# jarcode-foss/glava

Hardware: AMD Instinct MI355X
Metric: stereo 4096-pt FFT+smooth frames/s; % HBM roofline -- `value`: the window+FFT+magnitude pass of BASELINE configs[1]; the FFT+smooth chains (gravity / average on f32 state, GLava's shipped GL_R16 chain, + its pre-smoothing pass) are in roofline.chains (higher is better)
Workload: dtype f32

## Files before the change

### glava_amd/build.py

```python
from __future__ import annotations

import argparse
import os
import subprocess
import sys
from concurrent.futures import ThreadPoolExecutor

HERE = os.path.dirname(os.path.abspath(__file__))
CSRC = os.path.join(HERE, "csrc")
OBJ = os.path.join(CSRC, "build")
TUNE_BIN = os.path.join(os.path.dirname(HERE), "tools", "bin")
ARCH = "gfx950"
HIPFLAGS = ["--offload-arch=" + ARCH, "-O3", "-std=c++17", "-ffp-contract=off", "-fPIC",
            "-fno-fast-math", "-Wall", "-Wno-unused-function"]
SIZES = (7, 8, 9, 10, 11, 12, 13, 14)
SMALL = ("glv_bars", "glv_misc")
HOST = ("glv_api", "glv_wisdom", "glv_device_state", "glv_bar_tables", "glv_chain", "glv_track", "glv_multi")
PARTS = (0, 1, 2, 3, 4, 5, 6)


def _inst_jobs(obj_dir: str, sizes, extra: list[str]):
    return [("glv_inst.hip", os.path.join(obj_dir, f"glv_inst_{k}_{p}.o"), [f"-DGLV_LOG_NN={k}", f"-DGLV_INST_PART={p}", *extra])
            for k in sorted(sizes, reverse=True) for p in PARTS]
HEADERS = ["glv_core.h", "glv_frame.h", "glv_kernel_tmpl.h", "glv_launch.h", "glv_launch_util.h", "glv_tables.h", "glv_winsplit.h", "glv_host.h",
           os.path.join("..", "..", "include", "glv_spectrum.h")]


def _newer(target: str, deps: list[str]) -> bool:
    if not os.path.exists(target):
        return True
    t = os.path.getmtime(target)
    return any(os.path.getmtime(d) > t for d in deps)


def _hipcc() -> str:
    for c in (os.environ.get("HIPCC"), "/opt/rocm/bin/hipcc", "hipcc"):
        if c and (os.path.isabs(c) and os.path.exists(c) or not os.path.isabs(c)):
            return c
    return "hipcc"


def _run(cmd: list[str]) -> None:
    r = subprocess.run(cmd, capture_output=True, text=True)
    if r.returncode != 0:
        sys.stderr.write(" ".join(cmd) + "\n" + r.stdout + r.stderr)
        raise RuntimeError("build step failed: " + os.path.basename(cmd[-1]))


def _compile(src: str, obj: str, extra: list[str]) -> str:
    deps = [os.path.join(CSRC, src)] + [os.path.join(CSRC, h) for h in HEADERS]
    if _newer(obj, deps):
        cmd = [_hipcc(), *HIPFLAGS, *extra, "-c", os.path.join(CSRC, src), "-o", obj]
        _run(cmd)
        open(obj + ".cmd", "w").write(" ".join(cmd) + "\n")
    return obj


def _refuse_experiment_flags(flags: list[str]) -> None:
    env = " ".join(os.environ.get(k, "") for k in ("HIPCC_COMPILE_FLAGS_APPEND", "HIPFLAGS", "CXXFLAGS", "CPPFLAGS"))
    bad = [f for f in flags if f.startswith("-D") and not f.startswith(("-DGLV_LOG_NN=", "-DGLV_INST_PART="))]
    if bad or "-DGLV_" in env:
        raise RuntimeError(f"product build refuses extra macro definitions: {bad or env!r} (use build_variant for A/B libraries)")


def build_tune_variant(name: str, extra_flags: list[str], variants: str | None = None) -> str:
    os.makedirs(OBJ, exist_ok=True)
    os.makedirs(TUNE_BIN, exist_ok=True)
    obj = os.path.join(OBJ, f"glv_tune_{name}.o")
    flags = ["-DGLV_TUNE_BUILD", *[f for f in extra_flags if f != "-DGLV_TUNE_BUILD"]]
    if variants:
        flags.append("-DGLV_TUNE_VARIANTS=" + variants)
    _run([_hipcc(), *HIPFLAGS, *flags, "-c", os.path.join(CSRC, "glv_tune.hip"), "-o", obj])
    lib = os.path.join(TUNE_BIN, f"libglvtune_{name}.so")
    _run([_hipcc(), "--offload-arch=" + ARCH, "-shared", "-fPIC", "-o", lib, obj])
    os.remove(obj)
    return lib


def build_variant(name: str, extra_flags: list[str], sizes=SIZES, kernels_only: bool = False, misc: bool = False) -> str:
    obj_dir = os.path.join(OBJ, name)
    os.makedirs(obj_dir, exist_ok=True)
    extra_flags = ["-DGLV_TUNE_BUILD", *[f for f in extra_flags if f != "-DGLV_TUNE_BUILD"]]
    jobs = _inst_jobs(obj_dir, sizes, extra_flags)
    reused = []
    if kernels_only:
        reused = [os.path.join(OBJ, f"glv_inst_{k}_{p}.o") for k in SIZES if k not in sizes for p in PARTS]
        reused += [os.path.join(OBJ, f"{u}.o") for u in HOST]
        if misc:
            jobs += [(f"{m}.hip", os.path.join(obj_dir, f"{m}.o"), list(extra_flags)) for m in SMALL]
        else:
            reused += [os.path.join(OBJ, f"{m}.o") for m in SMALL]
    else:
        jobs += [(f"{m}.hip", os.path.join(obj_dir, f"{m}.o"), list(extra_flags)) for m in SMALL]
        jobs += [(f"{u}.cpp", os.path.join(obj_dir, f"{u}.o"), ["-x", "hip", *extra_flags]) for u in HOST]
    with ThreadPoolExecutor(max_workers=min(8, os.cpu_count() or 2)) as ex:
        objs = list(ex.map(lambda j: _compile(*j), jobs))
    lib = os.path.join(CSRC, f"libglvspectrum_{name}.so")
    _run([_hipcc(), "--offload-arch=" + ARCH, "-shared", "-fPIC", "-o", lib, *objs, *reused])
    return lib


def build(tune: bool = False, verbose: bool = False) -> str:
    lib = os.path.join(CSRC, "libglvspectrum.so")
    srcs = [os.path.join(CSRC, f) for f in ("glv_inst.hip", *(f"{m}.hip" for m in SMALL), *(f"{u}.cpp" for u in HOST))] + [os.path.join(CSRC, h) for h in HEADERS]
    stamp_path = lib + ".stamp"
    stamp = repr(max(os.path.getmtime(f) for f in srcs))
    if not tune and os.path.exists(lib) and os.path.exists(stamp_path) and open(stamp_path).read() == stamp:
        if verbose:
            print("up to date", lib)
        return lib
    os.makedirs(OBJ, exist_ok=True)
    jobs = _inst_jobs(OBJ, SIZES, [])
    jobs += [(f"{m}.hip", os.path.join(OBJ, f"{m}.o"), []) for m in SMALL]
    jobs += [(f"{u}.cpp", os.path.join(OBJ, f"{u}.o"), ["-x", "hip"]) for u in HOST]
    for _, _, extra in jobs:
        _refuse_experiment_flags(extra)
    if tune:
        jobs.append(("glv_tune.hip", os.path.join(OBJ, "glv_tune.o"), ["-DGLV_TUNE_BUILD"]))
    with ThreadPoolExecutor(max_workers=min(8, os.cpu_count() or 2)) as ex:
        objs = list(ex.map(lambda j: _compile(*j), jobs))
    prod = [o for o in objs if not o.endswith("glv_tune.o")]
    if _newer(lib, prod) or not os.path.exists(stamp_path) or open(stamp_path).read() != stamp:
        _run([_hipcc(), "--offload-arch=" + ARCH, "-shared", "-fPIC", "-o", lib, *prod])
    if repr(max(os.path.getmtime(f) for f in srcs)) == stamp:
        open(stamp_path, "w").write(stamp)
    else:
        for o in prod:
            os.remove(o)
        if os.path.exists(stamp_path): os.remove(stamp_path)
    if tune:
        tlib = os.path.join(CSRC, "libglvtune.so")
        tobj = os.path.join(OBJ, "glv_tune.o")
        if _newer(tlib, [tobj]):
            _run([_hipcc(), "--offload-arch=" + ARCH, "-shared", "-fPIC", "-o", tlib, tobj])
    if verbose:
        print("built", lib)
    return lib


if __name__ == "__main__":
    ap = argparse.ArgumentParser()
    ap.add_argument("--tune", action="store_true")
    ap.add_argument("--variant", nargs="+", metavar=("NAME", "FLAG"), help="build libglvspectrum_NAME.so with extra flags; write them without the leading dash (DGLV_X=1)")
    a = ap.parse_args()
    if a.variant:
        print("built", build_variant(a.variant[0], ["-" + f.lstrip("-") for f in a.variant[1:]]))
    else:
        build(tune=a.tune, verbose=True)
```

### glava_amd/csrc/glv_api.cpp

```cpp
#include <cstdarg>
#include <cstdio>
#include <cstdlib>
#include <new>

#include "glv_host.h"
#include "glv_tables.h"

namespace glvh __attribute__((visibility("hidden"))) {
thread_local std::string g_err = "";
int fail(int code, const char* fmt, ...) {
    char buf[512];
    va_list ap;
    va_start(ap, fmt);
    vsnprintf(buf, sizeof(buf), fmt, ap);
    va_end(ap);
    g_err = buf;
    return code;
}
}
namespace {
int validate(const glv_params* p) {
    if (!p) return fail(GLV_ERR_INVALID, "params is NULL");
    const int l = log2_exact(p->n);
    if (l < 8 || l > 15) return fail(GLV_ERR_INVALID, "n=%u: must be a power of two in [256, 32768]", p->n);
    if (p->channels != 1 && p->channels != 2) return fail(GLV_ERR_INVALID, "channels=%u: must be 1 or 2", p->channels);
    if (p->avg_frames < 1 || p->avg_frames > GLV_MAX_AVG_FRAMES)
        return fail(GLV_ERR_INVALID, "avg_frames=%u: must be in [1, %d]", p->avg_frames, GLV_MAX_AVG_FRAMES);
    if (p->avg_window_kind > 1) return fail(GLV_ERR_INVALID, "avg_window_kind=%u: must be 0 or 1", p->avg_window_kind);
    if (p->log_mode > 2) return fail(GLV_ERR_INVALID, "log_mode=%u: must be 0, 1 or 2", p->log_mode);
    if (p->gl_storage > 2) return fail(GLV_ERR_INVALID, "gl_storage=%u: must be 0, 1 (GL_R16 state, one launch) or 2 (pass by pass, f32 state)", p->gl_storage);
    if (p->ur != p->ur) return fail(GLV_ERR_INVALID, "ur is NaN");
    if (p->round_formula > GLV_ROUND_LINEAR) return fail(GLV_ERR_INVALID, "round_formula=%u: 0 sinusoidal, 1 circular, 2 linear", p->round_formula);
    if (p->sample_mode > GLV_SAMPLE_HYBRID) return fail(GLV_ERR_INVALID, "sample_mode=%u: 0 average, 1 maximum, 2 hybrid", p->sample_mode);
    return GLV_OK;
}

int ensure_device(int device) {
    int count = 0;
    hipError_t e = hipGetDeviceCount(&count);
    if (e != hipSuccess || count <= 0)
        return fail(GLV_ERR_NO_DEVICE, "no usable HIP device (%s); this library has no CPU path",
                    e == hipSuccess ? "device count is 0" : hipGetErrorString(e));
    if (device < 0 || device >= count) return fail(GLV_ERR_INVALID, "device %d out of range [0, %d)", device, count);
    HIP_TRY(hipSetDevice(device));
    return GLV_OK;
}

bool same_params(const glv_params& a, const glv_params& b) {
    return a.n == b.n && a.channels == b.channels && same_bits(a.fft_scale, b.fft_scale) && same_bits(a.fft_cutoff, b.fft_cutoff)
           && same_bits(a.gravity_step, b.gravity_step) && same_bits(a.ur, b.ur) && a.avg_frames == b.avg_frames && a.avg_window == b.avg_window
           && a.avg_window_kind == b.avg_window_kind && a.log_mode == b.log_mode && a.bars == b.bars && same_bits(a.smooth_factor, b.smooth_factor)
           && same_bits(a.smooth_distance, b.smooth_distance) && same_bits(a.smooth_ratio, b.smooth_ratio) && a.gl_storage == b.gl_storage
           && same_bits(a.bar_phase, b.bar_phase) && same_shape(a, b);
}

int batch_create_rows(const glv_params* p, uint32_t streams, unsigned ops_mask, int device, bool single_row, glv_batch** out) {
    if (!out) return fail(GLV_ERR_INVALID, "out is NULL");
    *out = nullptr;
    if (int rc = validate(p)) return rc;
    if (streams == 0) return fail(GLV_ERR_INVALID, "streams must be > 0");
    if (streams > (1u << 30)) return fail(GLV_ERR_INVALID, "streams=%u: at most 2^30 (row indices are 32-bit)", streams);
    if (int rc = ensure_device(device)) return rc;
    wisdom_load_env();
    glv_batch* b = new (std::nothrow) glv_batch();
    if (!b) return fail(GLV_ERR_NOMEM, "out of host memory");
    b->p = *p; b->streams = streams; b->ops_mask = ops_mask; b->device = device;
    b->rows = single_row ? 1u : streams * 2u; b->single_row = single_row;
    b->unfused_bars = std::getenv("GLV_UNFUSED_BARS") != nullptr;
    b->unfused_wave = std::getenv("GLV_UNFUSED_WAVE") != nullptr;
    if (const char* o = std::getenv("GLV_TRACK_WAVE_ORDER")) b->track_wave_by_steps = std::strcmp(o, "steps") == 0;
    b->bar_i8_off = std::getenv("GLV_NO_BARS_I8") != nullptr;
    b->log_nn = log2_exact(p->n) - 1;
    hipDeviceProp_t prop;
    if (hipGetDeviceProperties(&prop, device) == hipSuccess) {
        b->num_cus = prop.multiProcessorCount;
        std::snprintf(b->device_name, sizeof(b->device_name), "%s", prop.gcnArchName[0] ? prop.gcnArchName : prop.name);
    }
    int rc = b->tab.create(p->n, device);
    if (rc == GLV_OK) rc = batch_alloc(b);
    if (rc == GLV_OK) rc = batch_prepare(b);
    if (rc != GLV_OK) { glv_batch_destroy(b); return rc; }
    *out = b;
    return GLV_OK;
}

int sync_params(glv_batch* b, const glv_params* p) {
    if (same_params(b->p, *p)) return GLV_OK;
    glv_params rest = *p;
    rest.ur = b->p.ur; rest.gravity_step = b->p.gravity_step;
    if (!same_params(b->p, rest)) return glv_batch_set_params(b, p);
    b->p.ur = p->ur; b->p.gravity_step = p->gravity_step;
    update_gravity_step(b);
    return GLV_OK;
}

int round_trip(glv_state* s, const void* in, size_t in_bytes, void* out, size_t out_bytes, unsigned ops, bool texels) {
    glv_batch* b = s->b;
    HIP_TRY(hipSetDevice(b->device));
    const bool via_seq = s->mapped && (ops & GLV_OP_SMOOTH);
    if (via_seq && !s->seq) HIP_TRY(s->seq.alloc(b->p.n, false));
    if (texels && !s->d_tex) {
        if (s->mapped) {
            HIP_TRY(hipHostMalloc(reinterpret_cast<void**>(&s->h_tex), out_bytes, hipHostMallocMapped));
            HIP_TRY(hipHostGetDevicePointer(reinterpret_cast<void**>(&s->d_tex), s->h_tex, 0));
        } else {
            HIP_TRY(s->tex_copy.alloc(b->p.n, false));
            s->d_tex = s->tex_copy;
        }
    }
    float* d_in = via_seq ? s->seq.get() : s->d_io;
    float* d_out = texels ? reinterpret_cast<float*>(s->d_tex) : d_in;
    if (s->mapped && !via_seq) {
        std::memcpy(s->h_io, in, in_bytes);
        const int rc = process(b, d_in, glv::IN_F32_PLANAR, d_out, ops, 1, 0, nullptr);
        HIP_TRY(hipStreamSynchronize(nullptr));
        if (rc) return rc;
        std::memcpy(out, texels ? static_cast<const void*>(s->h_tex) : s->h_io, out_bytes);
        return GLV_OK;
    }
    HIP_TRY(hipMemcpyAsync(d_in, in, in_bytes, hipMemcpyHostToDevice, nullptr));
    if (int rc = process(b, d_in, glv::IN_F32_PLANAR, d_out, ops, 1, 0, nullptr)) return rc;
    HIP_TRY(hipMemcpyAsync(out, d_out, out_bytes, hipMemcpyDeviceToHost, nullptr));
    HIP_TRY(hipStreamSynchronize(nullptr));
    return GLV_OK;
}
}

extern "C" {
void glv_params_default(glv_params* p) {
    if (!p) return;
    std::memset(p, 0, sizeof(*p));
    p->n = 4096;
    p->channels = 2;
    p->fft_scale = 10.2F;
    p->fft_cutoff = 0.3F;
    p->gravity_step = 4.2F;
    p->ur = 22050.0F / 256.0F;
    p->avg_frames = 5;
    p->avg_window = 1;
    p->avg_window_kind = 0;
    p->log_mode = 1;
    p->bars = 80;
    p->smooth_factor = 0.025F;
    p->smooth_distance = 0.01F;
    p->smooth_ratio = 4.0F;
    p->gl_storage = 0;
    p->bar_phase = 0.0F;
}

int glv_set_last_error(int code, const char* msg) { g_err = msg ? msg : ""; return code; }
int glv_abi_version(void) { return GLV_ABI_VERSION; }
const char* glv_last_error(void) { return g_err.c_str(); }
int glv_device_count(void) {
    int count = 0;
    if (hipGetDeviceCount(&count) != hipSuccess) return 0;
    return count;
}

int glv_batch_create(const glv_params* p, uint32_t streams, unsigned ops_mask, int device, glv_batch** out) {
    return batch_create_rows(p, streams, ops_mask, device, false, out);
}

int glv_batch_set_params(glv_batch* b, const glv_params* p) {
    if (!b) return fail(GLV_ERR_INVALID, "batch is NULL");
    if (int rc = validate(p)) return rc;
    if (p->n != b->p.n || p->avg_frames != b->p.avg_frames)
        return fail(GLV_ERR_STATE, "params (n=%u, F=%u) do not match the batch (n=%u, F=%u): fixed at creation", p->n, p->avg_frames, b->p.n, b->p.avg_frames);
    if ((p->gl_storage == 1) != b->state16)
        return fail(GLV_ERR_STATE, "gl_storage=%u: the state of this batch was created as %s", p->gl_storage, b->state16 ? "GL_R16 texels (gl_storage 1)" : "floats (gl_storage 0 / 2)");
    if (b->snapped() && (p->bars != b->p.bars || p->gl_storage == 0))
        return fail(GLV_ERR_STATE, "bar texels are set (glv_batch_set_bar_texels): bars (%u -> %u) must keep the table's length and gl_storage must stay non-zero "
                                   "(a float chain has no pre-smoothed texture); clear the table first", b->p.bars, p->bars);
    HIP_TRY(hipSetDevice(b->device));
    HIP_TRY(hipDeviceSynchronize());
    const glv_params old = b->p;
    b->p = *p;
    int rc = batch_prepare(b);
    if (rc == GLV_OK && b->ran_live && b->live_bins() == 0)
        rc = fail(GLV_ERR_STATE, "this GLV_OP_BARS_ONLY batch has run its live kernel class: the state beyond the live bins was not kept, and these parameters "
                                 "(smooth_factor=%g bars=%u log_mode=%u) need the full chain -- glv_batch_reset first, or a new batch", (double) p->smooth_factor, p->bars, p->log_mode);
    if (rc != GLV_OK) { const std::string said = g_err; b->p = old; (void) batch_prepare(b); g_err = said; }
    for (auto& row : b->plan_cache) for (auto& pc : row) pc.gen = 0;
    return rc;
}

int glv_batch_reset(glv_batch* b) {
    if (!b) return fail(GLV_ERR_INVALID, "batch is NULL");
    HIP_TRY(hipSetDevice(b->device));
    const size_t n = b->p.n;
    if (b->d_hist) HIP_TRY(hipMemset(b->d_hist, 0, b->hist_bytes()));
    if (b->d_grav) HIP_TRY(hipMemset(b->d_grav, 0, b->grav_bytes()));
    if (b->d_ring) HIP_TRY(hipMemset(b->d_ring, 0, sizeof(int16_t) * 2 * n * b->streams));
    if (b->d_ring_f32) HIP_TRY(hipMemset(b->d_ring_f32, 0, sizeof(float) * 2 * n * b->streams));
    b->ring_pos = 0; b->ring_pos_f32 = 0; b->rewind_state();
    return GLV_OK;
}

int glv_batch_destroy(glv_batch* b) {
    if (!b) return GLV_OK;
    (void) hipSetDevice(b->device);
    b->tab.destroy();
    state_free(b->d_grav);
    state_free(b->d_hist);
    for (hipEvent_t e : b->ev) (void) hipEventDestroy(e);
    delete b;
    return GLV_OK;
}

int glv_batch_process_s16(glv_batch* b, const int16_t* d_pcm, float* d_out, unsigned ops, void* hip_stream) {
    if (!b) return fail(GLV_ERR_INVALID, "batch is NULL");
    if (!(ops & (GLV_OP_FFT | GLV_OP_WAVE))) return fail(GLV_ERR_INVALID, "s16 input requires GLV_OP_FFT or GLV_OP_WAVE");
    return process(b, d_pcm, glv::IN_S16_STEREO, d_out, ops, b->streams * 2, 0, (hipStream_t) hip_stream);
}

int glv_batch_process_f32(glv_batch* b, const float* d_f32, float* d_out, unsigned ops, void* hip_stream) {
    if (!b) return fail(GLV_ERR_INVALID, "batch is NULL");
    return process(b, d_f32, glv::IN_F32_PLANAR, d_out, ops, b->streams * 2, 0, (hipStream_t) hip_stream);
}

int glv_batch_process_f32_stereo(glv_batch* b, const float* d_pcm, float* d_out, unsigned ops, void* hip_stream) {
    if (!b) return fail(GLV_ERR_INVALID, "batch is NULL");
    if (!(ops & (GLV_OP_FFT | GLV_OP_WAVE))) return fail(GLV_ERR_INVALID, "interleaved input requires GLV_OP_FFT or GLV_OP_WAVE");
    return process(b, d_pcm, glv::IN_F32_STEREO, d_out, ops, b->streams * 2, 0, (hipStream_t) hip_stream);
}
// ... 339 lines not shown
```

### glava_amd/csrc/glv_chain.cpp

```cpp
#include <cstring>

#include "glv_host.h"
#include "glv_tables.h"

namespace glvh __attribute__((visibility("hidden"))) {
bool gl_fused_chain(const glv_batch* b, unsigned ops) {
    return b->p.gl_storage == 1 && (ops & GLV_OP_FFT) && (ops & (GLV_OP_GRAVITY | GLV_OP_AVERAGE)) && !(ops & (GLV_OP_RAW | GLV_OP_SMOOTH)) && b->p.log_mode != 2;
}
}
namespace {
bool gl_passes_chain(const glv_batch* b, unsigned ops) {
    return b->p.gl_storage != 0 && (ops & (GLV_OP_GRAVITY | GLV_OP_AVERAGE)) && !gl_fused_chain(b, ops);
}
}
namespace glvh __attribute__((visibility("hidden"))) {
unsigned frame_ops(const glv_batch* b, unsigned ops) { return gl_passes_chain(b, ops) ? GLV_OP_FFT | (ops & GLV_OP_RAW) : ops; }

void fill_common(glv::FrameArgs& a, const glv_params& p, const Tables& t) {
    std::memset(&a, 0, sizeof(a));
    a.tw = t.d_tw; a.win = t.d_win; a.win_split = t.d_win_split; a.logtab = t.d_log; a.tilt = t.d_tilt;
    a.F = p.avg_frames; a.mono = p.channels == 1; a.avg_window = p.avg_window != 0;
    a.inv_n = 1.0f / (float) p.n;
    a.fft_scale = p.fft_scale;
    a.one_minus_cutoff = 1.0F - p.fft_cutoff;
// ... 8 lines not shown
    if (!b->timing) return GLV_OK;
    if (b->ev_used + 2 > b->ev.size()) {
        hipEvent_t e0, e1;
        HIP_TRY(hipEventCreate(&e0));
        HIP_TRY(hipEventCreate(&e1));
        b->ev.push_back(e0); b->ev.push_back(e1);
    }
    HIP_TRY(hipEventRecord(b->ev[b->ev_used], st));
    return GLV_OK;
}
int timed_launch_end(glv_batch* b, hipStream_t st) {
    if (!b->timing) return GLV_OK;
    HIP_TRY(hipEventRecord(b->ev[b->ev_used + 1], st));
    b->ev_used += 2;
    b->launches += 1;
    return GLV_OK;
}

void update_gravity_step(glv_batch* b) {
    const float g = b->p.gravity_step * (1.0F / b->p.ur);
    if (b->state16 && (!b->grav_known || std::memcmp(&g, &b->grav_g, sizeof(g)) != 0)) {
        b->grav_int = glv::gravity_r16_integer_step(g, &b->grav_sub);
        b->grav_g = g; b->grav_known = true;
    }
}

int batch_prepare(glv_batch* b) {
    if (int rc = b->tab.set_tilt(b->p.fft_scale, b->p.fft_cutoff, b->p.log_mode == 1)) return rc;
    update_gravity_step(b);
    {
        const std::string said = g_err;
        const int rc = ensure_smooth_tables(b);
        if (rc != GLV_OK) { if (b->ops_mask & GLV_OP_SMOOTH) return rc; g_err = said; }
    }
    {
        const std::string said = g_err;
        const int rc = ensure_bar_tables(b);
        if (rc != GLV_OK) { if (b->ops_mask & GLV_OP_BARS) return rc; g_err = said; }
    }
    if (b->ops_mask & GLV_OP_BARS) {
        if (bars_need_rows(b, b->bar) || (b->ops_mask & GLV_OP_WAVE)) if (int rc = ensure_scratch(b)) return rc;
        if (int rc = ensure_snap_tables(b)) return rc;
        b->update_live_bins();
    }
    if (b->attr_log_mode != (int) b->p.log_mode) {
        b->attr_log_mode = (int) b->p.log_mode;
        glv::FrameArgs a;
        std::memset(&a, 0, sizeof(a));
        for (int in_mode = 0; in_mode < glv::kFrameKinds; ++in_mode)
            for (int v = 0; v < glv::frame_variants(b->log_nn); ++v)
                for (int c = 0; c < glv::kFrameClasses; ++c)
                    (void) glv::launch_frame(b->log_nn, in_mode, (int) b->p.log_mode, v, (glv::FrameClass) c, a, 0, nullptr);
        (void) hipGetLastError();
    }
    if (b->p.gl_storage == 2 && (b->ops_mask & (GLV_OP_GRAVITY | GLV_OP_AVERAGE)) && !b->single_row) return ensure_scratch(b);
    return GLV_OK;
}

int check_ops(const glv_batch* b, unsigned ops, const float* d_out) {
    const bool state_is_output = (ops & GLV_OP_GRAVITY) && !(ops & (GLV_OP_AVERAGE | GLV_OP_SMOOTH | GLV_OP_RAW));
    if (!d_out && !(state_is_output && !(ops & GLV_OP_BARS) && !b->state16))
        return fail(GLV_ERR_INVALID, "NULL output pointer (allowed only for f32-state chains ending in gravity, see glv_batch_gravity_state)");
    if (ops & GLV_OP_WAVE) {
        if (ops & (GLV_OP_FFT | GLV_OP_GRAVITY | GLV_OP_AVERAGE | GLV_OP_RAW | GLV_OP_WRANGE | GLV_OP_MAGNITUDE | GLV_OP_SMOOTH | GLV_OP_OUTPUT_IS_STATE))
            return fail(GLV_ERR_INVALID, "GLV_OP_WAVE combines with GLV_OP_BARS and GLV_OP_R16 only (it includes wrange and is stateless; ops 0x%x)", ops);
        if (ops & GLV_OP_BARS) {
            if (b->p.gl_storage == 0)
                return fail(GLV_ERR_STATE, "GLV_OP_WAVE | GLV_OP_BARS: gl_storage 0 -- a float chain has no texel rows for the pre-smoothing pass to sample");
            if ((b->ops_mask & (GLV_OP_WAVE | GLV_OP_BARS)) != (unsigned) (GLV_OP_WAVE | GLV_OP_BARS))
                return fail(GLV_ERR_STATE, "GLV_OP_WAVE | GLV_OP_BARS needs both bits in glv_batch_create's ops_mask (0x%x): the rows between its two launches are made at creation", b->ops_mask);
        }
        if (b->columns())
            return fail(GLV_ERR_STATE, "GLV_OP_WAVE with column texels set (glv_batch_set_column_texels): the wave shader does not average three texels (wave/1.frag:17-23)");
    }
    const unsigned stateful = ops & (GLV_OP_GRAVITY | GLV_OP_AVERAGE);
    if (stateful & ~b->ops_mask)
        return fail(GLV_ERR_STATE, "ops 0x%x need state the batch was not created with (ops_mask 0x%x)", ops, b->ops_mask);
    if (stateful && b->state16 != (b->p.gl_storage == 1))
        return fail(GLV_ERR_STATE, "gl_storage=%u: the state of this batch was created as %s", b->p.gl_storage, b->state16 ? "GL_R16 texels (gl_storage 1)" : "floats (gl_storage 0 / 2)");
    if ((b->ops_mask & GLV_OP_BARS_ONLY) && stateful && !(ops & GLV_OP_BARS))
        return fail(GLV_ERR_STATE, "the batch was created with GLV_OP_BARS_ONLY: its state lives only below the bins the bars sample, a stateful call must ask for GLV_OP_BARS (ops 0x%x)", ops);
    if ((ops & GLV_OP_WRANGE) && (ops & GLV_OP_FFT)) return fail(GLV_ERR_INVALID, "GLV_OP_WRANGE excludes GLV_OP_FFT");
    if ((ops & GLV_OP_RAW) && !(ops & GLV_OP_FFT)) return fail(GLV_ERR_INVALID, "GLV_OP_RAW needs GLV_OP_FFT");
    if ((ops & GLV_OP_MAGNITUDE) && (ops & (GLV_OP_FFT | GLV_OP_WRANGE))) return fail(GLV_ERR_INVALID, "GLV_OP_MAGNITUDE excludes GLV_OP_FFT and GLV_OP_WRANGE");
    if (!(ops & (GLV_OP_FFT | GLV_OP_GRAVITY | GLV_OP_AVERAGE | GLV_OP_WRANGE | GLV_OP_SMOOTH | GLV_OP_MAGNITUDE | GLV_OP_R16 | GLV_OP_WAVE))) return fail(GLV_ERR_INVALID, "empty ops");
    if ((ops & GLV_OP_R16) && (ops & (GLV_OP_RAW | GLV_OP_SMOOTH))) return fail(GLV_ERR_INVALID, "GLV_OP_R16 excludes GLV_OP_RAW and GLV_OP_SMOOTH");
    if ((ops & GLV_OP_R16) && !d_out) return fail(GLV_ERR_INVALID, "GLV_OP_R16 needs an output buffer");
    if ((ops & GLV_OP_OUTPUT_IS_STATE) && (!state_is_output || !d_out || (ops & (GLV_OP_BARS | GLV_OP_R16)) || b->p.gl_storage))
        return fail(GLV_ERR_INVALID, "GLV_OP_OUTPUT_IS_STATE needs a chain that ends in gravity with f32 rows out (no AVERAGE / SMOOTH / RAW / BARS / R16, gl_storage 0)");
    if ((ops & GLV_OP_BARS) && !b->bar.desc)
        return fail(GLV_ERR_STATE, "GLV_OP_BARS: the batch has no bar tables (bars / smooth_factor / bar_phase were unusable when it was created; tables are built at creation and by glv_batch_set_params, process calls never allocate)");
    if ((ops & GLV_OP_BARS) && (b->bar_x.count != b->p.bars || b->bar_x.factor != b->p.smooth_factor || b->bar_x.phase != b->p.bar_phase || !same_shape(b->bar_x.shape_of, b->p)))
        return fail(GLV_ERR_STATE, "GLV_OP_BARS: bar parameters changed without glv_batch_set_params");
    if ((ops & GLV_OP_BARS) && b->snapped()) {
        if (!(ops & GLV_OP_WAVE) && (!(ops & GLV_OP_FFT) || !(gl_fused_chain(b, ops) || gl_passes_chain(b, ops)) || (ops & GLV_OP_SMOOTH)))
            return fail(GLV_ERR_STATE, "GLV_OP_BARS with bar texels set (glv_batch_set_bar_texels) needs a GL chain's texel rows: GLV_OP_FFT with gravity / average on "
                                       "gl_storage 1 or 2, without GLV_OP_SMOOTH (ops 0x%x)", ops);
        if (!snap_current(b)) return fail(GLV_ERR_STATE, "GLV_OP_BARS: bar parameters changed without glv_batch_set_params");
        if (b->columns() && (ops & GLV_OP_R16))
            return fail(GLV_ERR_STATE, "GLV_OP_R16 with column texels set (glv_batch_set_column_texels): a mean of three texels is not a texel, the columns are floats");
    }
    if ((ops & GLV_OP_SMOOTH) && (!b->d_smin || b->smooth_d != b->p.smooth_distance || b->smooth_r != b->p.smooth_ratio))
        return fail(GLV_ERR_STATE, "GLV_OP_SMOOTH: the batch has no window bounds for these parameters (unusable smooth_ratio at creation, or changed without glv_batch_set_params)");
    return GLV_OK;
}

int plan_wave(const glv_batch* b, int in_mode, unsigned ops, uint32_t rot, float* d_out, ChainPlan& pl, bool whole_groups = true) {
    pl.route = ChainPlan::WAVE; pl.ops = ops; pl.out = d_out; pl.bars = ChainPlan::NO_BARS;
    pl.wave_r16 = (ops & GLV_OP_R16) != 0; pl.wave_limit = b->p.n;
    if (!(ops & GLV_OP_BARS)) return GLV_OK;
    const bool averaging = b->p.sample_mode == GLV_SAMPLE_AVERAGE;
    if (b->snapped()) pl.bars = averaging ? ChainPlan::BARS_SNAP : ChainPlan::BARS_SNAP_MODE;
    else if (averaging && b->p.bars >= glv::kBarSeqMin && b->bar_x.i8()) pl.bars = ChainPlan::BARS_I8;
    else pl.bars = ChainPlan::BARS_F32;
    pl.wave_fused = pl.bars == ChainPlan::BARS_I8 && (in_mode == glv::IN_S16_STEREO || in_mode == glv::IN_S16_RING) && (rot & 7u) == 0u && whole_groups && !b->unfused_wave && !b->single_row;
    if (pl.wave_fused) return GLV_OK;
    if (!b->d_scratch) return fail(GLV_ERR_STATE, "GLV_OP_WAVE | GLV_OP_BARS needs the internal rows: announce both bits in glv_batch_create's ops_mask");
    pl.out = pl.rows = b->d_scratch;
    pl.wave_r16 = pl.bars == ChainPlan::BARS_I8 || pl.bars == ChainPlan::BARS_SNAP;
    const uint32_t bins = b->snapped() ? b->snap.bins : b->bar_x.bins_needed;
    if ((pl.bars != ChainPlan::BARS_F32 || !averaging) && bins != 0 && bins < b->p.n) pl.wave_limit = bins;
    return GLV_OK;
}

int launch_bars_pass(glv_batch* b, const ChainPlan& pl, float* d_bars, size_t units, bool r16, hipStream_t st) {
    hipError_t e;
    if (pl.bars == ChainPlan::NO_BARS) return GLV_OK;
    if (pl.bars == ChainPlan::BARS_F32) {
        const glv::BarRowsTables rt = rows_tables(b->p, b->bar_x, b->bar);
        e = glv::launch_bars(pl.rows, d_bars, units, b->p.n, b->p.bars, b->bar_x.nsteps, b->bar_x.items, b->bar.desc, b->bar.w, st, r16, &rt);
    } else if (pl.bars == ChainPlan::BARS_SNAP || pl.bars == ChainPlan::BARS_SNAP_FLOATS) {
        e = glv::launch_bars_snap(pl.rows, pl.bars == ChainPlan::BARS_SNAP_FLOATS, d_bars, units, b->p.n, b->p.bars, b->snap.desc, reinterpret_cast<const uint32_t*>(b->snap.w.get()), st, r16);
    } else if (pl.bars == ChainPlan::BARS_COLUMNS) {
        e = glv::launch_columns(pl.rows, d_bars, units, b->p.n, (uint32_t) b->snap_x.tex.size(), b->p.bars, b->snap_x.col_nsteps, b->snap_x.col_items, b->snap.desc,
                                b->snap.w, b->snap_x.col_map, b->p.sample_mode, shape_hybrid(b->p), st);
    } else if (pl.bars == ChainPlan::BARS_SNAP_MODE) {
        const glv::BarRowsTables rt = rows_tables(b->p, b->bar_x, b->snap);
        e = glv::launch_bars(pl.rows, d_bars, units, b->p.n, b->p.bars, 0, nullptr, b->snap.desc, nullptr, st, r16, &rt);
    } else {
        const glv::BarIRowsTables irt = b->bar_x.irows_tables();
        e = glv::launch_bars_i8(pl.rows, pl.bars == ChainPlan::BARS_I8_FLOATS, d_bars, units, b->p.n, b->p.bars, &irt, st, r16);
    }
    ++b->last_launches;
    return e == hipSuccess ? GLV_OK : fail(GLV_ERR_HIP, "bars launch failed: %s", hipGetErrorString(e));
}
}
namespace {
int plan_chain(glv_batch* b, int in_mode, unsigned ops, uint32_t units, uint32_t rot, float* d_out, ChainPlan& pl) {
    if (ops & GLV_OP_WAVE) return plan_wave(b, in_mode, ops, rot, d_out, pl);
    const bool gl_passes = gl_passes_chain(b, ops);
    if (gl_fused_chain(b, ops)) pl.route = ChainPlan::GL_FUSED;
    else if (ops & GLV_OP_FFT) pl.route = gl_passes ? ChainPlan::GL_PASSES : ChainPlan::FRAME;
    else pl.route = (ops & (GLV_OP_GRAVITY | GLV_OP_AVERAGE | GLV_OP_WRANGE | GLV_OP_MAGNITUDE | GLV_OP_R16)) ? ChainPlan::POST : ChainPlan::COPY;
    if (ops & GLV_OP_FFT) launch_plan(b, units, in_mode, ops, &pl.variant, &pl.grid);
    const bool snap = (ops & GLV_OP_BARS) && b->snapped();
    pl.fused_bars = (ops & GLV_OP_BARS) && (ops & GLV_OP_FFT) && !gl_passes && bars_fusable(b, ops) && pl.variant < kMaxVariants
                    && (snap ? b->snap : b->bar).fusable[pl.variant];
    pl.out = d_out;
    if (ops & GLV_OP_BARS) {
        const bool state_is_output = (ops & GLV_OP_GRAVITY) && !(ops & (GLV_OP_AVERAGE | GLV_OP_SMOOTH | GLV_OP_RAW));
        if (pl.fused_bars || (state_is_output && !b->p.gl_storage)) pl.out = nullptr;
        else {
            if (!b->d_scratch) return fail(GLV_ERR_STATE, "this GLV_OP_BARS chain needs the internal spectra rows: announce it in glv_batch_create's ops_mask (GLV_OP_BARS together with the chain's other operators; GLV_OP_R16 too when a float chain's bars are wanted as texels)");
            pl.out = b->d_scratch;
        }
    }
    if (pl.route == ChainPlan::GL_PASSES) {
        pl.out = d_out && !(ops & (GLV_OP_BARS | GLV_OP_R16)) ? d_out : b->d_scratch;
        pl.rows = (ops & GLV_OP_BARS) ? pl.out : d_out;
    } else pl.rows = pl.out ? pl.out : b->d_grav;
    if (!(ops & GLV_OP_BARS) || pl.fused_bars) pl.bars = ChainPlan::NO_BARS;
    else if (snap && b->columns()) pl.bars = ChainPlan::BARS_COLUMNS;
    else if (snap) pl.bars = b->p.sample_mode != GLV_SAMPLE_AVERAGE ? ChainPlan::BARS_SNAP_MODE : pl.route == ChainPlan::GL_FUSED ? ChainPlan::BARS_SNAP : ChainPlan::BARS_SNAP_FLOATS;
    else if (b->p.bars >= glv::kBarSeqMin && b->bar_x.i8() && (pl.route == ChainPlan::GL_FUSED || (gl_passes && !(ops & GLV_OP_SMOOTH))))
        pl.bars = pl.route == ChainPlan::GL_FUSED ? ChainPlan::BARS_I8 : ChainPlan::BARS_I8_FLOATS;
    else pl.bars = ChainPlan::BARS_F32;
    if (pl.route == ChainPlan::GL_PASSES) pl.ops = frame_ops(b, ops);
    else {
        pl.ops = ops & ~(unsigned) (GLV_OP_PRIVATE_STATE | GLV_OP_OUTPUT_IS_STATE);
        if (ops & GLV_OP_BARS) pl.ops &= ~(unsigned) GLV_OP_R16;
        if (pl.bars == ChainPlan::BARS_I8 || pl.bars == ChainPlan::BARS_SNAP) pl.ops |= glv::OP_R16;
    }
    const uint32_t bins_needed = snap ? b->snap.bins : b->bar_x.bins_needed;
    if (pl.route == ChainPlan::GL_FUSED && pl.bars != ChainPlan::NO_BARS && bins_needed != 0 && bins_needed < b->p.n)
        pl.out_limit = bins_needed * 4u;
    if (b->live_bins() != 0 && (pl.route == ChainPlan::GL_FUSED || pl.fused_bars)) pl.live_points = b->live_bins() / 2u;
    pl.cls = glv::frame_class(pl.route == ChainPlan::GL_FUSED, pl.fused_bars, pl.live_points != 0, pl.ops, snap, snap && b->columns());
    return GLV_OK;
}

int run_wave(glv_batch* b, const ChainPlan& pl, const void* d_in, int in_mode, float* d_out, unsigned ops, uint32_t units, uint32_t rot, hipStream_t st) {
    const bool mono = b->p.channels == 1;
    if (int rc = timed_launch_begin(b, st)) return rc;
    hipError_t e;
    if (pl.wave_fused) {
        const glv::BarIRowsTables irt = b->bar_x.irows_tables();
        e = glv::launch_bars_i8_pcm(d_in, rot, mono, d_out, units, b->p.n, b->p.bars, &irt, st, (ops & GLV_OP_R16) != 0);
        b->kernel_name = "glv_bars_rows_i8_kernel";
    } else {
        e = glv::launch_wave(d_in, in_mode, mono, b->p.n, rot, units, pl.out, pl.wave_r16, pl.wave_limit, st);
        b->kernel_name = "glv_wave_kernel";
    }
    ++b->last_launches;
    if (e != hipSuccess) return fail(GLV_ERR_HIP, "kernel launch failed: %s", hipGetErrorString(e));
    if (!pl.wave_fused) if (int rc = launch_bars_pass(b, pl, d_out, units, (ops & GLV_OP_R16) != 0, st)) return rc;
    return timed_launch_end(b, st);
}

int run_chain(glv_batch* b, const ChainPlan& pl, const void* d_in, int in_mode, float* d_out, unsigned ops, uint32_t units, uint32_t rot,
              hipStream_t st) {
    glv::FrameArgs a;
    fill_common(a, b->p, b->tab);
    a.in = d_in; a.out = pl.out; a.grav = b->grav_cur; a.grav_w = b->d_grav; a.hist = b->d_hist;
    a.units = units; a.ops = pl.ops; a.head = b->head; a.rot = rot; a.log_mode = b->p.log_mode;
    a.grav_sub = b->grav_sub; a.grav_int = b->grav_int ? 1u : 0u;
    a.bars_r16 = (ops & GLV_OP_BARS) && (ops & GLV_OP_R16) ? 1u : 0u;
    a.out_limit = pl.out_limit;
    const bool gravity_only = (ops & GLV_OP_GRAVITY) && !(ops & GLV_OP_AVERAGE);
    const bool out_is_state = (ops & GLV_OP_OUTPUT_IS_STATE) != 0;
    if (out_is_state) {
        if ((const void*) d_out == d_in) return fail(GLV_ERR_INVALID, "GLV_OP_OUTPUT_IS_STATE: the output buffer must not be the input");
        a.grav_w = d_out; a.out = nullptr;
    }
    const float* grav_next = gravity_only ? (out_is_state ? d_out : b->d_grav) : b->grav_cur;
    if (pl.fused_bars) {
        const BarTableSet& t = b->snapped() ? b->snap : b->bar;
        a.bar_desc = t.desc; a.bar_items = t.fitems[pl.variant]; a.bar_nsteps = t.fnsteps[pl.variant]; a.bar_w = t.w;
        a.bars = b->p.bars; a.bars_out = d_out; a.col_map = b->snap_x.col_map;
    }
    if (pl.route == ChainPlan::GL_FUSED) a.gl_storage = 1;
    if (pl.route == ChainPlan::POST && (ops & (GLV_OP_GRAVITY | GLV_OP_AVERAGE))) a.gl_storage = b->p.gl_storage;
    if (pl.route == ChainPlan::GL_PASSES && !pl.out)
        return fail(GLV_ERR_STATE, "this gl_storage chain needs the internal spectra rows (created for gl_storage 2 batches with state, and with GLV_OP_BARS in the ops_mask)");
    if (pl.live_points != 0) { a.live_points = pl.live_points; b->ran_live = true; }

    if (int rc = timed_launch_begin(b, st)) return rc;
    hipError_t e = hipSuccess;
    if (pl.route == ChainPlan::POST || pl.route == ChainPlan::COPY) {
        if (in_mode != glv::IN_F32_PLANAR) return fail(GLV_ERR_INVALID, "operators without GLV_OP_FFT take planar f32 input");
        if (pl.route == ChainPlan::POST) { e = glv::launch_post(a, b->p.n, st); ++b->last_launches; }
        else if ((const void*) pl.out != d_in) e = hipMemcpyAsync(pl.out, d_in, sizeof(float) * (size_t) units * b->p.n, hipMemcpyDeviceToDevice, st);
        b->kernel_name = pl.route == ChainPlan::POST ? "glv_post_kernel" : "glv_smooth_kernel";
    } else {
        b->last_grid = pl.grid; b->last_variant = pl.variant;
        e = glv::launch_frame(b->log_nn, in_mode, (int) b->p.log_mode, pl.variant, pl.cls, a, pl.grid, st); ++b->last_launches;
        if (pl.route == ChainPlan::FRAME) b->kernel_name = "glv_frame_kernel";
    }
    if (e != hipSuccess) return fail(GLV_ERR_HIP, "kernel launch failed: %s", hipGetErrorString(e));
    if (pl.route == ChainPlan::GL_PASSES) {
        glv::FrameArgs a2 = a;
        a2.in = pl.out; a2.ops = ops & (GLV_OP_GRAVITY | GLV_OP_AVERAGE | ((ops & GLV_OP_BARS) ? 0u : (unsigned) GLV_OP_R16)); a2.gl_storage = b->p.gl_storage;
        a2.out = pl.rows;
        e = glv::launch_post(a2, b->p.n, st); ++b->last_launches;
        if (e != hipSuccess) return fail(GLV_ERR_HIP, "GL-storage pass launch failed: %s", hipGetErrorString(e));
    }
    if (pl.route == ChainPlan::GL_FUSED || pl.route == ChainPlan::GL_PASSES) b->kernel_name = "glv_frame_kernel";
    if (ops & GLV_OP_AVERAGE) b->head = (b->head + 1) % b->p.avg_frames;
    b->grav_cur = grav_next;
    if (ops & GLV_OP_SMOOTH) {
        e = glv::launch_smooth(pl.rows, units, b->p.n, b->d_smin, b->d_smax, b->smooth_asz, b->smooth_reach, b->smooth_window, st); ++b->last_launches;
        if (e != hipSuccess) return fail(GLV_ERR_HIP, "smooth launch failed: %s", hipGetErrorString(e));
    }
    if (int rc = launch_bars_pass(b, pl, d_out, units, (ops & GLV_OP_R16) != 0, st)) return rc;
    return timed_launch_end(b, st);
}

int gravity_form(unsigned ops) { return !(ops & GLV_OP_GRAVITY) ? 0 : (ops & GLV_OP_AVERAGE) ? 2 : 1; }
}
namespace glvh __attribute__((visibility("hidden"))) {
int refuse_gravity_mix(const glv_batch* b, unsigned ops) {
    const int mode = gravity_form(ops);
    if (mode == 0 || b->grav_mode == 0 || b->grav_mode == mode) return GLV_OK;
    return fail(GLV_ERR_STATE, "gravity was last applied %s average on this batch and is now requested %s it: the two forms keep "
                               "their state in different buffers (glv_batch_reset, or one batch per chain)",
                b->grav_mode == 2 ? "fused with" : "without", mode == 2 ? "fused with" : "without");
}
void commit_gravity_form(glv_batch* b, unsigned ops) {
    if (ops & GLV_OP_GRAVITY) b->grav_mode = gravity_form(ops);
}
int refuse_stale_tilt(const glv_batch* b) {
    if (b->tab.tilt_scale == b->p.fft_scale && b->tab.tilt_cutoff == b->p.fft_cutoff && b->tab.tilt_fold == (b->p.log_mode == 1)) return GLV_OK;
    return fail(GLV_ERR_STATE, "fft_scale / fft_cutoff / log_mode changed without glv_batch_set_params");
}

int process(glv_batch* b, const void* d_in, int in_mode, float* d_out, unsigned ops, uint32_t units,
            uint32_t rot, hipStream_t st) {
    if (!d_in) return fail(GLV_ERR_INVALID, "NULL device pointer");
    if (int rc = check_ops(b, ops, d_out)) return rc;
    if (int rc = refuse_gravity_mix(b, ops)) return rc;
    b->last_launches = 0;
    HIP_TRY(hipSetDevice(b->device));
    ChainPlan pl;
    if (int rc = plan_chain(b, in_mode, ops, units, rot, d_out, pl)) return rc;
    if (int rc = refuse_stale_tilt(b)) return rc;
    commit_gravity_form(b, ops);
    if (pl.route == ChainPlan::WAVE) return run_wave(b, pl, d_in, in_mode, d_out, ops, units, rot, st);
    return run_chain(b, pl, d_in, in_mode, d_out, ops, units, rot, st);
}
}
```

### glava_amd/csrc/glv_core.h

```cpp
#pragma once

#include <math.h>
#include <stdint.h>

#if !defined(GLV_TUNE_BUILD)
#if defined(GLV_ROWS_RB) || defined(GLV_BAR_BATCH_BIG) || defined(GLV_STATE_PAIR_MAX)
#error "tuning macros are for tools/tune.py A/B builds: compile with -DGLV_TUNE_BUILD (glava_amd.build.build_variant does); the product never defines them"
#endif
#endif

#if defined(__HIPCC__)
#define GLV_HD __host__ __device__ __forceinline__
#else
#define GLV_HD inline
#endif

#if defined(__HIP_DEVICE_COMPILE__)
#define GLV_SCHED_FENCE() __builtin_amdgcn_sched_barrier(0)
#else
#define GLV_SCHED_FENCE() ((void) 0)
#endif

namespace glv {

struct alignas(8) cf { float x, y; };
struct alignas(8) u32x2 { uint32_t x, y; };
struct alignas(16) d2 { double x, y; };
struct alignas(16) cf2 { cf a, b; };

GLV_HD constexpr int tw_offset(int L) { return L; }

#if defined(__HIP_DEVICE_COMPILE__)
typedef float glv_f2 __attribute__((ext_vector_type(2)));
template <bool SCALAR_W>
__device__ __forceinline__ void bf_mul(glv_f2& p02, glv_f2& p13, const cf& b, const cf& w) {
    const glv_f2 B = { b.x, b.y }, W = { w.x, w.y };
    if constexpr (SCALAR_W) {
        asm("v_pk_mul_f32 %0, %1, %2 op_sel:[0,0] op_sel_hi:[0,1]" : "=v"(p02) : "s"(W), "v"(B));
        asm("v_pk_mul_f32 %0, %1, %2 op_sel:[1,1] op_sel_hi:[1,0]" : "=v"(p13) : "s"(W), "v"(B));
    } else {
        asm("v_pk_mul_f32 %0, %1, %2 op_sel:[0,0] op_sel_hi:[0,1]" : "=v"(p02) : "v"(W), "v"(B));
        asm("v_pk_mul_f32 %0, %1, %2 op_sel:[1,1] op_sel_hi:[1,0]" : "=v"(p13) : "v"(W), "v"(B));
    }
}
__device__ __forceinline__ void bf_t(glv_f2& t, const glv_f2& p02, const glv_f2& p13) {
    asm("v_pk_add_f32 %0, %1, %2 neg_lo:[0,1]" : "=v"(t) : "v"(p02), "v"(p13));
}
__device__ __forceinline__ void bf_out(cf& a, cf& b, const glv_f2& t) {
    const glv_f2 A = { a.x, a.y };
    glv_f2 hi, lo;
    asm("v_pk_add_f32 %0, %1, %2 neg_lo:[0,1] neg_hi:[0,1]" : "=v"(hi) : "v"(A), "v"(t));
    asm("v_pk_add_f32 %0, %1, %2" : "=v"(lo) : "v"(A), "v"(t));
    a.x = lo.x; a.y = lo.y; b.x = hi.x; b.y = hi.y;
}
#endif
template <bool SCALAR_W = false>
GLV_HD void butterfly(cf& a, cf& b, const cf w) {
#if defined(__HIP_DEVICE_COMPILE__)
    glv_f2 p02, p13, t;
    bf_mul<SCALAR_W>(p02, p13, b, w);
    bf_t(t, p02, p13);
    bf_out(a, b, t);
#else
    const float p0 = w.x * b.x, p1 = w.y * b.y;
    const float p2 = w.x * b.y, p3 = w.y * b.x;
    const float tr = p0 - p1;
    const float ti = p2 + p3;
    const cf hi = { a.x - tr, a.y - ti };
    const cf lo = { a.x + tr, a.y + ti };
    a = lo; b = hi;
#endif
}

GLV_HD void butterfly_unit(cf& a, cf& b) {
#if defined(__HIP_DEVICE_COMPILE__)
    const glv_f2 A = { a.x, a.y }, B = { b.x, b.y };
    glv_f2 hi, lo;
    asm("v_pk_add_f32 %0, %1, %2 neg_lo:[0,1] neg_hi:[0,1]" : "=v"(hi) : "v"(A), "v"(B));
    asm("v_pk_add_f32 %0, %1, %2" : "=v"(lo) : "v"(A), "v"(B));
    a.x = lo.x; a.y = lo.y; b.x = hi.x; b.y = hi.y;
#else
    const cf hi = { a.x - b.x, a.y - b.y };
    const cf lo = { a.x + b.x, a.y + b.y };
    a = lo; b = hi;
#endif
}

GLV_HD constexpr int bitrev(int v, int bits) {
    int r = 0;
    for (int i = 0; i < bits; ++i) r |= ((v >> i) & 1) << (bits - 1 - i);
    return r;
}

template <int RB>
struct SubPass {
    static constexpr int R = 1 << RB;

    GLV_HD static constexpr int ksub_of(int r0, int s) {
        int k = 0;
        for (int t = 0; t < s; ++t) k |= ((r0 >> (RB - 1 - t)) & 1) << t;
        return k;
    }

    template <bool FIRST, bool UNIT_SHORTCUT = true>
    GLV_HD static void run(cf (&v)[R], const cf (&tw)[R > 1 ? R - 1 : 1]) {
        constexpr bool SC = FIRST && UNIT_SHORTCUT;
#pragma unroll
        for (int s = 0; s < RB; ++s) {
            const int bit = 1 << (RB - 1 - s);
#if defined(__HIP_DEVICE_COMPILE__)
            constexpr int NB = R / 2, GRP = NB < 4 ? NB : 4;
#pragma unroll
            for (int g0 = 0; g0 < NB; g0 += GRP) {
                glv_f2 p02[GRP], p13[GRP], t[GRP];
#pragma unroll
                for (int j = 0; j < GRP; ++j) {
                    const int r0 = lo_slot(g0 + j, bit);
                    if (!(SC && ksub_of(r0, s) == 0)) bf_mul<FIRST>(p02[j], p13[j], v[r0 | bit], tw[(1 << s) - 1 + ksub_of(r0, s)]);
                }
#pragma unroll
                for (int j = 0; j < GRP; ++j) {
                    const int r0 = lo_slot(g0 + j, bit);
                    if (!(SC && ksub_of(r0, s) == 0)) bf_t(t[j], p02[j], p13[j]);
                }
#pragma unroll
                for (int j = 0; j < GRP; ++j) {
                    const int r0 = lo_slot(g0 + j, bit);
                    if (SC && ksub_of(r0, s) == 0) butterfly_unit(v[r0], v[r0 | bit]);
                    else bf_out(v[r0], v[r0 | bit], t[j]);
                }
            }
#else
#pragma unroll
            for (int r0 = 0; r0 < R; ++r0) {
                if (r0 & bit) continue;
                if (SC && ksub_of(r0, s) == 0) butterfly_unit(v[r0], v[r0 | bit]);
                else butterfly<FIRST>(v[r0], v[r0 | bit], tw[(1 << s) - 1 + ksub_of(r0, s)]);
            }
#endif
        }
    }
    GLV_HD static constexpr int lo_slot(int idx, int bit) { return ((idx & ~(bit - 1)) << 1) | (idx & (bit - 1)); }

    GLV_HD static constexpr int tw_index(int L0, int k0, int s, int ksub) {
        return tw_offset(L0 << s) + k0 + L0 * ksub;
    }
};

template <int LOG_NN, int LOG_E = 4>
struct Plan {
    static constexpr int NN = 1 << LOG_NN;
    static constexpr int E = 1 << LOG_E;
    static constexpr int T = NN / E;
    static constexpr int P = (LOG_NN + LOG_E - 1) / LOG_E;
    GLV_HD static constexpr int rb(int pass) { return pass < P - 1 ? LOG_E : LOG_NN - LOG_E * (P - 1); }
    GLV_HD static constexpr int log_l0(int pass) { return LOG_E * pass; }
};

GLV_HD constexpr int lds_index(int pass, int q, int log_e = 4) { return pass == 0 ? q + (q >> log_e) : q; }
// ... 174 lines not shown
```

### glava_amd/csrc/glv_frame.h

```cpp
#pragma once

#include "glv_core.h"

namespace glv {

enum InMode { IN_S16_STEREO = 0, IN_F32_PLANAR = 1, IN_S16_RING = 2, IN_F32_STEREO = 3, IN_F32_RING = 4,
              IN_S16_TRACK = 5,
              IN_F32_TRACK = 6 };
constexpr int IN_S16_TRACK_AT = 7, IN_F32_TRACK_AT = 8;
constexpr int kFrameKinds = 9;
GLV_HD constexpr bool in_track_table(int in_mode) { return in_mode == IN_S16_TRACK_AT || in_mode == IN_F32_TRACK_AT; }
enum Epi { EPI_RAW = 0, EPI_MAG = 1, EPI_MAG_STATE = 2, EPI_RAW_STATE = 3 };

enum : uint32_t { OP_FFT = 1u, OP_GRAVITY = 2u, OP_AVERAGE = 4u, OP_RAW = 8u, OP_WRANGE = 16u, OP_BARS = 32u, OP_SMOOTH = 64u, OP_MAGNITUDE = 128u, OP_R16 = 256u, OP_PRIVATE_STATE = 512u, OP_WAVE = 16384u };

struct BarDesc { uint32_t first_bin, count, tap_offset; float weight_sum; };
struct BarModeBlock { uint32_t w_off, maxcount; };
constexpr uint32_t kBarModeUnroll = 4;
struct alignas(16) BarItem { uint32_t w_byte, tex_byte, res; float keep; };
struct alignas(8) ColumnMap { uint16_t l, m, r, pad; };
struct alignas(16) BarTile { uint32_t k0, k1, origin, end; };
struct alignas(16) BarMTile { uint32_t k0, origin, steps, w_off; };
struct alignas(8) BarIFin { uint32_t c, s; };
constexpr uint32_t kBarIFinNone = 16;
constexpr uint32_t kBarILookAhead = 4;

enum FrameClass : int {
    FC_PLAIN = 0,
    FC_STATE = 1,
    FC_STATE_BARS = 2,
    FC_R16 = 3,
    FC_STATE_R16 = 4,
    FC_GL16 = 5,
    FC_GL16_BARS = 6,
    FC_GL16_LIVE = 7,
    FC_STATE_BARS_LIVE = 8,
    FC_GL16_BARS_LIVE = 9,
    FC_GL16_SNAP = 10,
    FC_GL16_SNAP_LIVE = 11,
    FC_GL16_COLS = 12,
    FC_GL16_COLS_LIVE = 13,
};
constexpr int kFrameClasses = 14;
GLV_HD constexpr bool fc_cols(int c) { return c == FC_GL16_COLS || c == FC_GL16_COLS_LIVE; }
GLV_HD constexpr bool fc_snap(int c) { return c == FC_GL16_SNAP || c == FC_GL16_SNAP_LIVE || fc_cols(c); }
GLV_HD constexpr bool fc_fused_bars(int c) { return c == FC_STATE_BARS || c == FC_GL16_BARS || c == FC_STATE_BARS_LIVE || c == FC_GL16_BARS_LIVE || fc_snap(c); }
GLV_HD constexpr bool fc_gl16(int c) { return c == FC_GL16 || c == FC_GL16_BARS || c == FC_GL16_LIVE || c == FC_GL16_BARS_LIVE || fc_snap(c); }
GLV_HD constexpr bool fc_live(int c) { return c == FC_GL16_LIVE || c == FC_STATE_BARS_LIVE || c == FC_GL16_BARS_LIVE || c == FC_GL16_SNAP_LIVE || c == FC_GL16_COLS_LIVE; }
GLV_HD constexpr bool fc_has_state(int c) { return c != FC_PLAIN && c != FC_R16; }
GLV_HD constexpr bool fc_texel_out(int c) { return c == FC_R16 || c == FC_STATE_R16; }
GLV_HD constexpr FrameClass frame_class(bool gl16, bool fused_bars, bool live, uint32_t ops, bool snap = false, bool cols = false) {
    if (gl16 && fused_bars && snap && cols) return live ? FC_GL16_COLS_LIVE : FC_GL16_COLS;
    if (gl16 && fused_bars && snap) return live ? FC_GL16_SNAP_LIVE : FC_GL16_SNAP;
    if (gl16) return fused_bars ? (live ? FC_GL16_BARS_LIVE : FC_GL16_BARS) : (live ? FC_GL16_LIVE : FC_GL16);
    if (fused_bars) return live ? FC_STATE_BARS_LIVE : FC_STATE_BARS;
    if (ops & (OP_GRAVITY | OP_AVERAGE)) return (ops & OP_R16) ? FC_STATE_R16 : FC_STATE;
    return (ops & OP_R16) ? FC_R16 : FC_PLAIN;
}

struct TrackWindows {
    uint64_t pitch_frames, hop;
    uint32_t steps, streams;
    uint32_t step_major, pad;
    const uint32_t* starts;
    uint32_t start_max, pad2;
};
GLV_HD constexpr uint64_t track_window_start(const TrackWindows& w, uint32_t s, uint32_t t, uint32_t entry = 0) {
    return (uint64_t) s * w.pitch_frames + (w.starts ? (uint64_t) (entry < w.start_max ? entry : w.start_max) : (uint64_t) t * w.hop);
}
GLV_HD constexpr uint64_t track_window_row(const TrackWindows& w, uint32_t s, uint32_t t) {
    return w.step_major ? ((uint64_t) t * w.streams + s) * 2u : ((uint64_t) s * w.steps + t) * 2u;
}

struct FrameArgs {
    const void* in;
    float* out;
    const float* grav;
    float* grav_w;
    float* hist;
    const cf* tw;
    const double* win;
    const void* win_split;
    const LogEntry* logtab;
    const float* tilt;
    uint32_t units;
    uint32_t ops;
    uint32_t F, head;
    uint32_t mono;
    uint32_t avg_window;
    uint32_t gl_storage;
    uint32_t grav_sub;
    uint32_t grav_int;
    uint32_t bars_r16;
    uint32_t log_mode;
    uint32_t rot;
    float inv_n, fft_scale, one_minus_cutoff, g, F_as_float;
    float F_rcp;
    uint32_t out_limit;
    uint32_t live_points;
    double wts[64];
    float wts32[64];
    const BarDesc* bar_desc;
    const BarItem* bar_items;
    const float* bar_w;
    float* bars_out;
    uint32_t bars;
    uint32_t bar_nsteps;
    const ColumnMap* col_map;
    TrackWindows trk;
};

constexpr int kBarTaps = 8;
GLV_HD constexpr int bar_lanes_of(uint32_t n) { return n <= 1024u ? 2 : (n == 2048u ? 4 : 8); }
GLV_HD constexpr uint32_t bar_chunk_of(uint32_t n) { return (uint32_t) (bar_lanes_of(n) * kBarTaps); }
GLV_HD constexpr bool win_split_of(int log_nn, int cls) { return !(log_nn == 13 && cls == FC_PLAIN); }
constexpr int kBarBatch = 2;
#if !defined(GLV_BAR_BATCH_BIG)
#define GLV_BAR_BATCH_BIG 6
#endif
GLV_HD constexpr int bar_batch_of(int log_nn) { return log_nn >= 13 ? GLV_BAR_BATCH_BIG : kBarBatch; }
struct BarTaps { float t[kBarTaps], w[kBarTaps]; };
struct alignas(16) BarW4 { float w[4]; };
struct __attribute__((packed, aligned(4))) BarT4 { float t[4]; };
template <bool VEC = true>
GLV_HD BarTaps bar_item_load(const float* tex_row, const float* tap_w, const BarItem& it, int sub) {
    BarTaps s;
    const uint32_t lane_byte = 4u * (uint32_t) kBarTaps * (uint32_t) sub;
#pragma unroll
    for (int h = 0; h < kBarTaps / 4; ++h) {
        const BarW4 w4 = ld<BarW4>(tap_w, it.w_byte + lane_byte + 16u * (uint32_t) h);
#pragma unroll
        for (int i = 0; i < 4; ++i) s.w[4 * h + i] = w4.w[i];
    }
    const uint32_t base = it.tex_byte + lane_byte;
    if constexpr (VEC) {
#pragma unroll
        for (int h = 0; h < kBarTaps / 4; ++h) {
            const BarT4 t4 = *reinterpret_cast<const BarT4*>(reinterpret_cast<const char*>(tex_row) + base + 16u * (uint32_t) h);
#pragma unroll
            for (int i = 0; i < 4; ++i) s.t[4 * h + i] = t4.t[i];
        }
    } else {
#pragma unroll
        for (int i = 0; i < kBarTaps; ++i) s.t[i] = ld<float>(tex_row, base + 4u * (uint32_t) i);
    }
    return s;
}
GLV_HD float bar_item_lane_sum(const BarTaps& s) {
#if defined(__HIP_DEVICE_COMPILE__)
    const glv_f2 ones = {1.0f, 1.0f};
    glv_f2 acc = {0.0f, 0.0f};
#pragma unroll
    for (int i = 0; i < kBarTaps; i += 2) {
        glv_f2 t = {s.t[i], s.t[i + 1]};
        const glv_f2 w = {s.w[i], s.w[i + 1]};
        asm("v_pk_mul_f32 %0, %1, %2 clamp" : "=v"(t) : "v"(t), "s"(ones));
        asm("v_pk_fma_f32 %0, %1, %2, %3" : "=v"(acc) : "v"(t), "v"(w), "v"(acc));
    }
    return acc.x + acc.y;
#else
    float e = 0.0f, o = 0.0f;
    auto clamp01 = [](float x) { return x > 0.0f ? (x < 1.0f ? x : 1.0f) : 0.0f; };
    for (int i = 0; i < kBarTaps; i += 2) {
        e = __builtin_fmaf(clamp01(s.t[i]), s.w[i], e);
        o = __builtin_fmaf(clamp01(s.t[i + 1]), s.w[i + 1], o);
    }
    return e + o;
#endif
}
GLV_HD uint64_t bar_snap_lane_sum(const BarTaps& s) {
    uint64_t acc = 0;
#pragma unroll
    for (int i = 0; i < kBarTaps; i += 2) {
        const uint32_t c2 = pack_unorm16(s.t[i], s.t[i + 1]);
        acc += (uint64_t) __builtin_bit_cast(uint32_t, s.w[i]) * (c2 & 0xffffu);
        acc += (uint64_t) __builtin_bit_cast(uint32_t, s.w[i + 1]) * (c2 >> 16);
    }
    return acc;
}
GLV_HD uint64_t bar_item_texel_sum(const uint16_t* tex_row, const float* tap_w, const BarItem& it, int sub) {
    const uint32_t lane_byte = 4u * (uint32_t) kBarTaps * (uint32_t) sub;
    const uint32_t first = it.tex_byte / 4u + (uint32_t) kBarTaps * (uint32_t) sub;
    uint32_t c[kBarTaps];
#pragma unroll
    for (int i = 0; i < kBarTaps; ++i) c[i] = (uint32_t) tex_row[first + (uint32_t) i];
    uint64_t acc = 0;
#pragma unroll
    for (int h = 0; h < kBarTaps / 4; ++h) {
        const BarW4 w4 = ld<BarW4>(tap_w, it.w_byte + lane_byte + 16u * (uint32_t) h);
#pragma unroll
        for (int i = 0; i < 4; ++i) acc += (uint64_t) __builtin_bit_cast(uint32_t, w4.w[i]) * c[4 * h + i];
    }
    return acc;
}
GLV_HD uint32_t bar_snap_texel(uint64_t total) { return (uint32_t) ((total + (1ull << 30)) >> 31); }
GLV_HD float bar_snap_float(uint64_t total) { return (float) (__builtin_ldexp((double) total, -31) / 65535.0); }
GLV_HD float column_mean(uint32_t cl, uint32_t cm, uint32_t cr) {
    const float lm = unorm16_to_float(cl) + unorm16_to_float(cm);
    const float lmr = lm + unorm16_to_float(cr);
    return lmr / 3.0f;
}

#if defined(__HIPCC__)
template <int CTRL> __device__ __forceinline__ float dpp_move(float v) {
    return __builtin_bit_cast(float, __builtin_amdgcn_update_dpp(0, __builtin_bit_cast(int, v), CTRL, 0xF, 0xF, false));
}
template <int GL> __device__ __forceinline__ float group_sum(float v) {
    static_assert(GL == 2 || GL == 4 || GL == 8, "lanes per group");
    v = v + dpp_move<0xB1>(v);
    if constexpr (GL >= 4) v = v + dpp_move<0x4E>(v);
    if constexpr (GL >= 8) v = v + dpp_move<0x141>(v);
    return v;
}
template <int CTRL> __device__ __forceinline__ uint64_t dpp_move64(uint64_t v) {
    const uint32_t lo = (uint32_t) __builtin_amdgcn_update_dpp(0, (int) (uint32_t) v, CTRL, 0xF, 0xF, false);
    const uint32_t hi = (uint32_t) __builtin_amdgcn_update_dpp(0, (int) (uint32_t) (v >> 32), CTRL, 0xF, 0xF, false);
    return ((uint64_t) hi << 32) | lo;
}
template <int GL> __device__ __forceinline__ uint64_t group_sum64(uint64_t v) {
    static_assert(GL == 2 || GL == 4 || GL == 8, "lanes per group");
    v = v + dpp_move64<0xB1>(v);
    if constexpr (GL >= 4) v = v + dpp_move64<0x4E>(v);
    if constexpr (GL >= 8) v = v + dpp_move64<0x141>(v);
    return v;
}
#endif


GLV_HD uint32_t ring_slot(uint32_t head, uint32_t f, uint32_t F) {
    uint32_t s = head + 1 + f;
    return s >= F ? s - F : s;
}

GLV_HD void weighted_add(cf& acc, cf f, float w, bool windowed) {
#if defined(__HIP_DEVICE_COMPILE__)
    const glv_f2 T = {f.x, f.y}, A = {acc.x, acc.y};
    glv_f2 s;
    if (windowed) {
        const glv_f2 W = {w, w};
        glv_f2 p;
        asm("v_pk_mul_f32 %0, %1, %2" : "=v"(p) : "v"(T), "s"(W));
        asm("v_pk_add_f32 %0, %1, %2" : "=v"(s) : "v"(A), "v"(p));
    } else asm("v_pk_add_f32 %0, %1, %2" : "=v"(s) : "v"(A), "v"(T));
    acc.x = s.x; acc.y = s.y;
#else
    if (windowed) { const float p0 = w * f.x, p1 = w * f.y; acc.x = acc.x + p0; acc.y = acc.y + p1; }
    else { acc.x = acc.x + f.x; acc.y = acc.y + f.y; }
#endif
}
GLV_HD void weighted_texels(cf& acc, uint32_t p, float w, bool windowed) { weighted_add(acc, texels_to_float(p), w, windowed); }
GLV_HD uint32_t apply_state_r16(uint32_t tex, uint32_t off, size_t row, uint32_t n, const FrameArgs& a) {
    const uint32_t F = a.F, o = off / 2u;
    const bool ring = (a.ops & OP_AVERAGE) != 0;
    uint16_t* h = ring ? reinterpret_cast<uint16_t*>(a.hist) + row * (size_t) F * n : nullptr;
    if (a.ops & OP_GRAVITY) {
        const uint16_t* gs = ring ? h + (size_t) (F == 1 ? a.head : ring_slot(a.head, F - 2, F)) * n
                                  : reinterpret_cast<const uint16_t*>(a.grav) + row * (size_t) n;
        tex = gravity_r16(tex, ld<uint32_t>(gs, o), a.g, a.grav_sub, a.grav_int);
        if (!ring) st<uint32_t>(reinterpret_cast<uint16_t*>(a.grav_w) + row * (size_t) n, o, tex);
    }
    if (ring) {
        cf acc = { 0.0f, 0.0f };
// ... 851 lines not shown
```

### glava_amd/csrc/glv_host.h

```cpp
#pragma once

#include <hip/hip_runtime.h>

#include <cstring>
#include <string>
#include <vector>

#include "../../include/glv_spectrum.h"
#include "glv_launch.h"

namespace glvh __attribute__((visibility("hidden"))) {
extern thread_local std::string g_err;
int fail(int code, const char* fmt, ...) __attribute__((format(printf, 2, 3)));

#define HIP_TRY(expr)                                                                              \
    do {                                                                                           \
        hipError_t e_ = (expr);                                                                    \
        if (e_ != hipSuccess) return fail(GLV_ERR_HIP, "%s failed: %s", #expr, hipGetErrorString(e_)); \
    } while (0)

inline int log2_exact(uint32_t v) {
    int l = 0;
    while ((1u << l) < v) ++l;
    return (1u << l) == v ? l : -1;
}

inline float shape_scale(const glv_params& p) { return p.sample_scale != 0.0f ? p.sample_scale : 8.0f; }
inline float shape_range(const glv_params& p) { return p.sample_range != 0.0f ? p.sample_range : 0.9f; }
inline float shape_hybrid(const glv_params& p) { return p.sample_hybrid_weight != 0.0f ? p.sample_hybrid_weight : 0.65f; }
inline bool same_bits(float a, float b) { return std::memcmp(&a, &b, sizeof(a)) == 0; }
inline bool same_shape(const glv_params& a, const glv_params& b) {
    return a.round_formula == b.round_formula && a.sample_mode == b.sample_mode && same_bits(a.sample_hybrid_weight, b.sample_hybrid_weight)
           && same_bits(a.sample_scale, b.sample_scale) && same_bits(a.sample_range, b.sample_range);
}

constexpr int kOpsClasses = 7, kInKinds = 7;
constexpr int kMaxVariants = 4;
constexpr bool kTrackWaveBySteps = false;

template <class T> class DeviceArray {
    T* p_ = nullptr;
    hipError_t renew(const T* src, size_t count, bool zeroed) {
        T* q = nullptr;
        hipError_t e = hipMalloc(&q, sizeof(T) * count);
        if (e == hipSuccess && src) e = hipMemcpy(q, src, sizeof(T) * count, hipMemcpyHostToDevice);
        if (e == hipSuccess && zeroed) e = hipMemset(q, 0, sizeof(T) * count);
        if (e != hipSuccess) { if (q) (void) hipFree(q); return e; }
        reset();
        p_ = q;
        return hipSuccess;
    }
public:
    DeviceArray() = default;
    DeviceArray(DeviceArray&& o) noexcept : p_(o.p_) { o.p_ = nullptr; }
    DeviceArray& operator=(DeviceArray&& o) noexcept { if (this != &o) { reset(); p_ = o.p_; o.p_ = nullptr; } return *this; }
    ~DeviceArray() { reset(); }
    hipError_t upload(const T* src, size_t count) { return renew(src, count, false); }
    hipError_t upload(const std::vector<T>& v) { return renew(v.data(), v.size(), false); }
    hipError_t alloc(size_t count, bool zeroed) { return renew(nullptr, count, zeroed); }
    void reset() { if (p_) (void) hipFree(p_); p_ = nullptr; }
    T* get() const { return p_; }
    operator T*() const { return p_; }
};

struct SharedTables;
struct Tables {
    SharedTables* shared = nullptr;
    glv::cf* d_tw = nullptr;
    double* d_win = nullptr;
    float* d_win_split = nullptr;
    int win_shifted = 0;
    glv::LogEntry* d_log = nullptr;
    DeviceArray<float> d_tilt;
    float tilt_scale = 0.f, tilt_cutoff = 0.f;
    bool tilt_fold = false;
    uint32_t n_ = 0;
    int set_tilt(float fft_scale, float fft_cutoff, bool fold);
    static int make_shared(SharedTables* t);
    int create(uint32_t n, int device);
    void destroy();
};

struct BarTableSet {
    DeviceArray<glv::BarDesc> desc;
    DeviceArray<float> w;
    DeviceArray<glv::BarItem> fitems[kMaxVariants];
    uint32_t fnsteps[kMaxVariants] = {}; bool fusable[kMaxVariants] = {};
    DeviceArray<glv::BarModeBlock> mblocks; DeviceArray<float> mw; uint32_t nmblocks = 0;
    uint32_t bins = 0;
};
struct BarExtras {
    DeviceArray<glv::BarItem> items; uint32_t nsteps = 0;
    DeviceArray<glv::BarMTile> mtiles; DeviceArray<float> wt, wsum; DeviceArray<glv::BarTile> rounds;
    uint32_t ntiles = 0, nrounds = 0, ring_bins = 0, bins_needed = 0;
    uint32_t chunk_reach = 0;
    DeviceArray<glv::BarMTile> itiles; DeviceArray<int8_t> wq; DeviceArray<glv::BarIFin> fin; DeviceArray<glv::BarTile> irounds;
    uint32_t intiles = 0, inrounds = 0, iring_bins = 0;
    bool i8_none = false;
    uint32_t count = 0; float factor = -1.f, phase = 0.f;
    glv_params shape_of{};
    glv::BarIRowsTables irows_tables() const { return glv::BarIRowsTables{itiles, intiles, wq, fin, irounds, inrounds, iring_bins}; }
    bool i8() const { return irounds.get() != nullptr && inrounds != 0; }
};
struct SnapExtras {
    std::vector<uint32_t> tex;
    std::vector<uint32_t> col_tex;
    DeviceArray<glv::ColumnMap> col_map;
    DeviceArray<glv::BarItem> col_items; uint32_t col_nsteps = 0;
    glv_params of{};
};

struct EventPair {
    hipEvent_t e0 = nullptr, e1 = nullptr;
    EventPair() = default; EventPair(const EventPair&) = delete; EventPair& operator=(const EventPair&) = delete;
    ~EventPair() { if (e0) (void) hipEventDestroy(e0); if (e1) (void) hipEventDestroy(e1); }
    hipError_t create() { const hipError_t e = hipEventCreate(&e0); return e != hipSuccess ? e : hipEventCreate(&e1); }
};
}
using namespace glvh;

struct glv_batch {
    glv_params p;
    uint32_t streams = 0;
    unsigned ops_mask = 0;
    int device = 0;
    int log_nn = 0;
    int num_cus = 256;
    Tables tab;
    float* d_grav = nullptr;
    const float* grav_cur = nullptr;
    float* d_hist = nullptr;
    DeviceArray<int16_t> d_ring;
    int grav_mode = 0;
    uint32_t head = 0;
    uint32_t ring_pos = 0;
    int grid_override = 0;
    int variant_override = -1;
    int attr_log_mode = -1;
    int last_launches = 0;
    int last_grid = 0;
    int last_variant = 0;
    char device_name[48] = "unknown";
    struct PlanCache { uint64_t gen = 0; int variant = 0, grid = 0; bool hit = false; } plan_cache[kInKinds][kOpsClasses];
    uint32_t rows = 0;
    bool single_row = false;
    bool unfused_bars = false;
    bool unfused_wave = false;
    bool track_wave_by_steps = kTrackWaveBySteps;
    bool state16 = false;
    float grav_g = 0.f; uint32_t grav_sub = 0; bool grav_int = false, grav_known = false;
    DeviceArray<float> d_scratch;
    DeviceArray<float> d_ring_f32;
    uint32_t ring_pos_f32 = 0;
    DeviceArray<int> d_smin, d_smax;
    uint32_t smooth_asz = 0;
    uint32_t smooth_reach = 0;
    uint32_t smooth_window = 0;
    float smooth_d = -1.f, smooth_r = -1.f;
    BarTableSet bar; BarExtras bar_x;
    BarTableSet snap; SnapExtras snap_x;
    bool bar_i8_off = false;
    size_t grav_bytes() const { return (state16 ? sizeof(uint16_t) : sizeof(float)) * rows * p.n; }
    size_t hist_bytes() const { return grav_bytes() * p.avg_frames; }
    void rewind_state() { head = 0; grav_mode = 0; grav_cur = d_grav; ran_live = false; }
    bool snapped() const { return !snap_x.tex.empty(); }
    bool columns() const { return !snap_x.col_tex.empty(); }
    uint32_t live_bins_now = 0;
    uint32_t live_bins() const { return live_bins_now; }
    bool ran_live = false;
    uint32_t live_bins_with(uint32_t snap_bins) const {
        const uint32_t sampled = snap_bins > bar.bins ? snap_bins : bar.bins;
        if (!(ops_mask & GLV_OP_BARS_ONLY) || sampled == 0 || sampled >= p.n || p.gl_storage > 1u || p.log_mode == 2u) return 0u;
        for (int v = 0; v < glv::frame_variants(log_nn); ++v)
            if ((uint32_t) glv::frame_geometry(log_nn, v).live_points * 2u < sampled) return 0u;
        if (p.gl_storage == 0u && (!bar.fusable[0] || unfused_bars)) return 0u;
        return sampled;
    }
    void update_live_bins() { live_bins_now = live_bins_with(snapped() ? snap.bins : 0u); }
    bool timing = false;
    std::vector<hipEvent_t> ev;
    size_t ev_used = 0;
    uint64_t launches = 0;
    const char* kernel_name = "glv_frame_kernel";
};

struct glv_state {
    glv_batch* b = nullptr;
    float* h_io = nullptr;
    float* d_io = nullptr;
    uint16_t* h_tex = nullptr;
    uint16_t* d_tex = nullptr;
    DeviceArray<uint16_t> tex_copy;
    DeviceArray<float> seq;
    bool mapped = true;
};

namespace glvh __attribute__((visibility("hidden"))) {
struct ChainPlan {
    enum Route {
        GL_FUSED,
        GL_PASSES,
        FRAME,
        POST,
        COPY,
        WAVE,
    } route = FRAME;
    enum Bars { NO_BARS, BARS_F32, BARS_I8, BARS_I8_FLOATS,
                BARS_SNAP, BARS_SNAP_FLOATS, BARS_SNAP_MODE,
                BARS_COLUMNS,
                BARS_COLUMNS_TEXELS } bars = NO_BARS;
    int variant = 0, grid = 0;
    glv::FrameClass cls = glv::FC_PLAIN;
    unsigned ops = 0;
    bool fused_bars = false;
    float* out = nullptr;
    float* rows = nullptr;
    uint32_t out_limit = 0, live_points = 0;
    bool wave_fused = false;
    bool wave_r16 = false;
    uint32_t wave_limit = 0;
};

    void launch_plan(glv_batch* b, uint32_t units, int in_mode, unsigned ops, int* variant, int* grid);
    void wisdom_load_env();
    void state_free(void* p);
    int batch_alloc(glv_batch* b);
    glv::BarRowsTables rows_tables(const glv_params& p, const BarExtras& x, const BarTableSet& s);
    int ensure_smooth_tables(glv_batch* b); int ensure_bar_tables(glv_batch* b); int ensure_scratch(glv_batch* b); int ensure_snap_tables(glv_batch* b);
    bool snap_current(const glv_batch* b);
    bool bars_fusable(const glv_batch* b, unsigned ops);
    bool bars_need_rows(const glv_batch* b, const BarTableSet& s);
    bool gl_fused_chain(const glv_batch* b, unsigned ops);
    unsigned frame_ops(const glv_batch* b, unsigned ops);
    void fill_common(glv::FrameArgs& a, const glv_params& p, const Tables& t);
    int timed_launch_begin(glv_batch* b, hipStream_t st); int timed_launch_end(glv_batch* b, hipStream_t st);
    void update_gravity_step(glv_batch* b);
    int batch_prepare(glv_batch* b);
    int check_ops(const glv_batch* b, unsigned ops, const float* d_out);
    int plan_wave(const glv_batch* b, int in_mode, unsigned ops, uint32_t rot, float* d_out, ChainPlan& pl, bool whole_groups);
    int launch_bars_pass(glv_batch* b, const ChainPlan& pl, float* d_bars, size_t units, bool r16, hipStream_t st);
    int refuse_gravity_mix(const glv_batch* b, unsigned ops); void commit_gravity_form(glv_batch* b, unsigned ops); int refuse_stale_tilt(const glv_batch* b);
    int process(glv_batch* b, const void* d_in, int in_mode, float* d_out, unsigned ops, uint32_t units, uint32_t rot, hipStream_t st);
}
```

### glava_amd/csrc/glv_kernel_tmpl.h

```cpp
#pragma once

#include <hip/hip_runtime.h>

#include <atomic>
#include <type_traits>

#include "glv_frame.h"

namespace glv {

template <int T, int SLOTS>
struct SlotSync {
    static constexpr bool WAVE_LOCAL = T <= 64 && (64 % T) == 0;
    static constexpr bool WORKGROUP = !WAVE_LOCAL && SLOTS == 1;
    static constexpr bool COUNTER = !WAVE_LOCAL && !WORKGROUP;
    static constexpr uint32_t WAVES = T / 64 > 0 ? T / 64 : 1;
    uint32_t* counter = nullptr;
    uint32_t expected = 0;
    __device__ __forceinline__ void sync() {
        if constexpr (WAVE_LOCAL) {
            __builtin_amdgcn_fence(__ATOMIC_ACQ_REL, "wavefront");
            __builtin_amdgcn_wave_barrier();
        } else if constexpr (WORKGROUP) {
            __syncthreads();
        } else {
            expected += WAVES;
            __builtin_amdgcn_fence(__ATOMIC_RELEASE, "workgroup");
            if ((threadIdx.x & 63) == 0) __hip_atomic_fetch_add(counter, 1u, __ATOMIC_RELAXED, __HIP_MEMORY_SCOPE_WORKGROUP);
            while (__hip_atomic_load(counter, __ATOMIC_RELAXED, __HIP_MEMORY_SCOPE_WORKGROUP) < expected) __builtin_amdgcn_s_sleep(1);
            __builtin_amdgcn_fence(__ATOMIC_ACQUIRE, "workgroup");
        }
    }
};

template <int LOG_NN, int LOG_E, int NBUF, int TWREG, bool UNIT_SHORTCUT = true>
struct Body {
    using FR = Frame<LOG_NN, LOG_E>;
    static constexpr int P = FR::P, NN = FR::NN, N = FR::N, T = FR::T;

    static constexpr bool TW_LDS_MODE = (TWREG == 4 && P >= 2) || (TWREG >= 2 && P >= 3);
    static constexpr bool is_mid(int q) { return q >= 1 && q < P - 1; }
    static constexpr bool from_lds(int q) { return TW_LDS_MODE && (is_mid(q) || (TWREG == 4 && q >= 1)); }
    static constexpr bool resident(int q) { return q >= 1 && (TWREG == 1 || (TWREG >= 2 && !TW_LDS_MODE) || (TWREG == 3 && q == P - 1)); }
    static constexpr int LDS_BIAS = tw_offset(FR::E);
    static constexpr int LDS_ENTRIES = !TW_LDS_MODE ? 0 : TWREG == 4 ? NN - FR::E : (1 << FR::PL::log_l0(P - 1)) - FR::E;

    template <int PASS>
    static constexpr int tw_off() {
        if constexpr (PASS == 0) return 0;
        else return tw_off<PASS - 1>() + FR::template PassInfo<PASS - 1>::NTW;
    }
    static constexpr int TW_TOTAL = tw_off<P>();

    template <int PASS>
    static __device__ __forceinline__ cf (&tw_ref(cf* all))[FR::template PassInfo<PASS>::NTW] {
        return *reinterpret_cast<cf(*)[FR::template PassInfo<PASS>::NTW]>(all + tw_off<PASS>());
    }

    static __device__ __forceinline__ void gather_uniform_tw0(cf* all, const cf* __restrict__ table) {
        cf (&t0)[FR::template PassInfo<0>::NTW] = tw_ref<0>(all);
        FR::template gather_tw<0>(t0, table, 0);
#pragma unroll
        for (int i = 0; i < FR::template PassInfo<0>::NTW; ++i) {
            t0[i].x = __builtin_bit_cast(float, __builtin_amdgcn_readfirstlane(__builtin_bit_cast(int, t0[i].x)));
            t0[i].y = __builtin_bit_cast(float, __builtin_amdgcn_readfirstlane(__builtin_bit_cast(int, t0[i].y)));
        }
    }

    template <int PASS>
    static __device__ __forceinline__ void gather_resident(cf* all, const cf* __restrict__ table, int tid) {
        if constexpr (resident(PASS)) FR::template gather_tw<PASS>(tw_ref<PASS>(all), table, tid);
        if constexpr (PASS + 1 < P) gather_resident<PASS + 1>(all, table, tid);
    }
    template <int PASS>
    static __device__ __forceinline__ void gather_transient(cf* all, const cf* __restrict__ table, const cf* lds_tw, int tid) {
        if constexpr (from_lds(PASS)) FR::template gather_tw<PASS, LDS_BIAS>(tw_ref<PASS>(all), lds_tw, tid);
        else if constexpr (!resident(PASS)) FR::template gather_tw<PASS>(tw_ref<PASS>(all), table, tid);
    }

    template <int PASS, typename SYNC>
    static __device__ __forceinline__ void run(cf (&v)[FR::E], cf* tw_all, const cf* __restrict__ table,
                                               char* xslot, int tid, unsigned& xcount, const cf* lds_tw, SYNC& sy) {
        FR::template compute<PASS, UNIT_SHORTCUT>(v, tw_ref<PASS>(tw_all));
        if constexpr (PASS + 1 < P) {
            char* xb = xslot + (NBUF == 2 ? (size_t) (xcount & 1u) * FR::XREGION * sizeof(cf) : 0);
            GLV_SCHED_FENCE();
            if constexpr (NBUF == 0) {
                sy.sync();
                FR::template exchange_write_half<PASS, 0>(xb, v, tid);
                gather_transient<PASS + 1>(tw_all, table, lds_tw, tid);
                sy.sync();
                FR::template exchange_read_half<PASS + 1, 0>(v, xb, tid);
                GLV_SCHED_FENCE();
                sy.sync();
                FR::template exchange_write_half<PASS, 1>(xb, v, tid);
                sy.sync();
                FR::template exchange_read_half<PASS + 1, 1>(v, xb, tid);
            } else {
            if constexpr (NBUF == 1) sy.sync();
            FR::template exchange_write<PASS>(xb, v, tid);
            gather_transient<PASS + 1>(tw_all, table, lds_tw, tid);
            sy.sync();
            FR::template exchange_read<PASS + 1>(v, xb, tid);
            }
            GLV_SCHED_FENCE();
            ++xcount;
            run<PASS + 1>(v, tw_all, table, xslot, tid, xcount, lds_tw, sy);
        }
    }
};

template <int LOG_NN, int LOG_E, int SLOTS, int NBUF, bool WINLDS, int TWREG = 0>
constexpr size_t frame_lds_bytes() {
    return (size_t) SLOTS * (NBUF == 0 ? sizeof(float) : NBUF * sizeof(cf)) * Frame<LOG_NN, LOG_E>::XREGION + (WINLDS ? (size_t) Frame<LOG_NN, LOG_E>::N * sizeof(double) : 0)
           + ((size_t) sizeof(LogEntry) << log_tab_bits_of(LOG_NN)) + (size_t) Body<LOG_NN, LOG_E, NBUF, TWREG>::LDS_ENTRIES * sizeof(cf) + (size_t) 16 * SLOTS;
}

template <bool UNIFORM>
static __device__ __forceinline__ uint32_t maybe_scalar(uint32_t v) {
    if constexpr (UNIFORM) return (uint32_t) __builtin_amdgcn_readfirstlane((int) v);
    else return v;
}

template <int LOG_NN, int IN_MODE, int LOG_MODE, int SLOTS, int NBUF, int TWREG, bool WINLDS, int OCC, int PREFETCH, int TILTREG,
          int LOG_E, int STATEFUL, int WPRE = 0>
__global__ void __launch_bounds__((Frame<LOG_NN, LOG_E>::T * SLOTS), OCC)
glv_frame_kernel(const FrameArgs a) {
    using FR = Frame<LOG_NN, LOG_E>;
    constexpr int E = FR::E;
    constexpr int T = FR::T, N = FR::N;
    constexpr bool RING = IN_MODE == IN_S16_RING;
    constexpr bool TRACK_TABLE = in_track_table(IN_MODE);
    constexpr bool TRACK = IN_MODE == IN_S16_TRACK || IN_MODE == IN_S16_TRACK_AT;
    constexpr bool TRACKF = IN_MODE == IN_F32_TRACK || IN_MODE == IN_F32_TRACK_AT;
    constexpr bool S16 = IN_MODE == IN_S16_STEREO || RING || TRACK;
    constexpr bool WSPLIT = S16 && win_split_of(LOG_NN, STATEFUL);
    constexpr bool NF = !S16;
    using BD = Body<LOG_NN, LOG_E, NBUF, TWREG, S16>;
    constexpr bool WAVE_SLOT = (T % 64) == 0;
    constexpr size_t XBYTES = (size_t) FR::XREGION * (NBUF == 0 ? sizeof(float) : sizeof(cf));
    constexpr int NREG = NBUF == 0 ? 1 : NBUF;

    extern __shared__ __attribute__((aligned(16))) char smem[];
    constexpr int NTHREADS = T * SLOTS;
    const uint32_t slot = maybe_scalar<WAVE_SLOT>(threadIdx.x / T);
    const int tid = (int) (threadIdx.x % T);
    char* xslot = smem + (size_t) slot * NREG * XBYTES;

    const void* gwin = WSPLIT ? a.win_split : static_cast<const void*>(a.win);
    const void* win = gwin;
    if constexpr (WINLDS) {
        char* lwin = smem + (size_t) SLOTS * NREG * XBYTES;
        for (int i = threadIdx.x; i < N / 2; i += NTHREADS) st<d2>(lwin, (uint32_t) i * 16u, ld<d2>(gwin, (uint32_t) i * 16u));
        __syncthreads();
        win = lwin;
    }

    const LogEntry* logtab = a.logtab;
    if constexpr (LOG_MODE == 0) {
        char* llog = smem + (size_t) SLOTS * NREG * XBYTES + (WINLDS ? (size_t) N * sizeof(double) : 0);
        constexpr int LB = log_tab_bits_of(LOG_NN);
        for (int i = threadIdx.x; i < (1 << LB); i += NTHREADS) st<d2>(llog, (uint32_t) i * 16u, ld<d2>(a.logtab, (uint32_t) (i << (kLogTabMaxBits - LB)) * 16u));
        __syncthreads();
        logtab = reinterpret_cast<const LogEntry*>(llog);
    }

    const cf* lds_tw = nullptr;
    if constexpr (BD::TW_LDS_MODE) {
        char* ltw = smem + (size_t) SLOTS * NREG * XBYTES + (WINLDS ? (size_t) N * sizeof(double) : 0) + ((size_t) sizeof(LogEntry) << log_tab_bits_of(LOG_NN));
        for (int i = threadIdx.x; i < BD::LDS_ENTRIES; i += NTHREADS) st<cf>(ltw, (uint32_t) i * 8u, ld<cf>(a.tw, (uint32_t) (BD::LDS_BIAS + i) * 8u));
        __syncthreads();
        lds_tw = reinterpret_cast<const cf*>(ltw);
    }

    SlotSync<T, SLOTS> sy;
    if constexpr (SlotSync<T, SLOTS>::COUNTER) {
        uint32_t* ctr = reinterpret_cast<uint32_t*>(smem + frame_lds_bytes<LOG_NN, LOG_E, SLOTS, NBUF, WINLDS, TWREG>() - 16 * SLOTS) + 4 * slot;
        if (tid == 0) { ctr[0] = 0; ctr[1] = 0; ctr[2] = 0; }
        __syncthreads();
        sy.counter = ctr;
    }

    cf tw_all[BD::TW_TOTAL];
    BD::gather_uniform_tw0(tw_all, a.tw);
    if constexpr (FR::P > 1) BD::template gather_resident<1>(tw_all, a.tw, tid);
    cf tilt_reg[TILTREG == 1 ? E : 1];
    if constexpr (TILTREG == 1) FR::gather_tilt(tilt_reg, a.tilt, tid);
    if constexpr (TILTREG == 3) {
        const int lane_q = FR::template out_index<FR::P - 1>(tid, 0, 0) - FR::template out_index<FR::P - 1>(0, 0, 0);
        tilt_reg[0].x = tilt_lin_base(tilt_lin(a.inv_n, a.fft_scale, a.one_minus_cutoff), 2 * lane_q);
        tilt_reg[0].y = 0.0f;
    }

    const bool raw_out = (a.ops & OP_RAW) != 0;
    constexpr bool FUSED_BARS = fc_fused_bars(STATEFUL);
    constexpr bool GL16 = fc_gl16(STATEFUL);
    constexpr bool GL16_LIVE = GL16 && fc_live(STATEFUL);
    constexpr bool F32_LIVE = !GL16 && fc_live(STATEFUL);
    constexpr bool HAS_STATE = fc_has_state(STATEFUL);
    constexpr bool TEXELS = fc_texel_out(STATEFUL);
    static_assert(!FUSED_BARS || WAVE_SLOT, "fused bars need whole waves per row");
    static_assert(!GL16 || LOG_MODE != 2, "the GL_R16 chain is built for log modes 0 and 1");
    static_assert(!FUSED_BARS || NBUF == 1, "fused bars park the finished row in exchange region 0: needs the full-size, two-barrier region");
    constexpr bool LIVE_PRE = GL16_LIVE && FR::LIVE_PREFETCH && S16 && PREFETCH == 1;
    typename FR::LivePre live_pre;
    const typename FR::LivePre* live_pre_ptr = nullptr;
    auto finish = [&](const cf (&v)[E], size_t row, int tid) {
        float* out_row = FUSED_BARS ? reinterpret_cast<float*>(xslot)
                                               : (HAS_STATE && a.out == nullptr ? nullptr : a.out + row * N);
        if constexpr (GL16) {
            float* o = FUSED_BARS ? reinterpret_cast<float*>(xslot)
                                  : ((a.ops & OP_R16) ? reinterpret_cast<float*>(reinterpret_cast<uint16_t*>(a.out) + row * N) : a.out + row * N);
            FR::template epilogue_gl16<LOG_MODE, TILTREG, NF, FUSED_BARS, GL16_LIVE>(v, o, row, tid, a, logtab, tilt_reg, live_pre_ptr);
        } else if constexpr (TEXELS && HAS_STATE) {
            float* out16 = reinterpret_cast<float*>(reinterpret_cast<uint16_t*>(a.out) + row * N);
            if (raw_out) FR::template epilogue<LOG_MODE, EPI_RAW_STATE, 0, true, NF>(v, out16, row, tid, a, logtab);
            else FR::template epilogue<LOG_MODE, EPI_MAG_STATE, TILTREG, true, NF>(v, out16, row, tid, a, logtab, tilt_reg);
        } else if constexpr (F32_LIVE) {
            FR::template epilogue<LOG_MODE, EPI_MAG_STATE, TILTREG, false, NF, true>(v, out_row, row, tid, a, logtab, tilt_reg);
        } else if constexpr (HAS_STATE) {
            if (raw_out) FR::template epilogue<LOG_MODE, EPI_RAW_STATE, 0, false, NF>(v, out_row, row, tid, a, logtab);
            else FR::template epilogue<LOG_MODE, EPI_MAG_STATE, TILTREG, false, NF>(v, out_row, row, tid, a, logtab, tilt_reg);
        } else if constexpr (TEXELS) {
            float* out16 = reinterpret_cast<float*>(reinterpret_cast<uint16_t*>(a.out) + row * N);
            if (raw_out) FR::template epilogue<LOG_MODE, EPI_RAW, 0, true, NF>(v, out16, row, tid, a, logtab);
            else FR::template epilogue<LOG_MODE, EPI_MAG, TILTREG, true, NF>(v, out16, row, tid, a, logtab, tilt_reg);
        } else {
            if (raw_out) FR::template epilogue<LOG_MODE, EPI_RAW, 0, false, NF>(v, out_row, row, tid, a, logtab);
            else FR::template epilogue<LOG_MODE, EPI_MAG, TILTREG, false, NF>(v, out_row, row, tid, a, logtab, tilt_reg);
        }
    };
    float bar_wsum = 1.0f;
    if constexpr (FUSED_BARS && !fc_cols(STATEFUL)) { if ((uint32_t) tid < a.bars) bar_wsum = a.bar_desc[tid].weight_sum; }
    auto finish_row = [&](const cf (&v)[E], size_t row, int tid, bool active) {
        if constexpr (FUSED_BARS) {
            sy.sync();
            if (active) finish(v, row, tid);
            sy.sync();
            constexpr int GL = bar_lanes_of((uint32_t) N);
            constexpr uint32_t G = T / GL;
            constexpr int BB = bar_batch_of(LOG_NN);
            float* lrow = reinterpret_cast<float*>(xslot);
            float* lres = lrow + N;
            static_assert(2 * T >= 64, "the chunk reads of bar_item_load stay inside the slot's region");
            constexpr bool snap = fc_snap(STATEFUL);
            constexpr bool cols = fc_cols(STATEFUL);
            if (active && snap) {
                const int sub = tid & (GL - 1);
                const uint32_t g = (uint32_t) tid / GL;
                const BarItem* items = a.bar_items + g;
                uint32_t* lout = reinterpret_cast<uint32_t*>(lres);
                const bool r16 = a.bars_r16 != 0;
                BarItem it[BB];
#pragma unroll
                for (int b = 0; b < BB; ++b) it[b] = items[(size_t) b * G];
                uint64_t total = 0;
                for (uint32_t s0 = 0; s0 < a.bar_nsteps; s0 += BB) {
                    BarTaps tp[BB];
                    BarItem nx[BB];
#pragma unroll
                    for (int b = 0; b < BB; ++b) tp[b] = bar_item_load<false>(lrow, a.bar_w, it[b], sub);
#pragma unroll
                    for (int b = 0; b < BB; ++b) nx[b] = items[(size_t) (s0 + BB + b) * G];
                    if constexpr (BB <= kBarBatch) GLV_SCHED_FENCE();
#pragma unroll
                    for (int b = 0; b < BB; ++b) {
                        const uint64_t chunk_sum = group_sum64<GL>(bar_snap_lane_sum(tp[b]));
                        total = it[b].keep != 0.0f ? total + chunk_sum : chunk_sum;
                        if constexpr (cols) { if (sub == 0) reinterpret_cast<uint16_t*>(lres)[it[b].res] = (uint16_t) bar_snap_texel(total); }
                        else if (sub == 0) lout[it[b].res] = r16 ? bar_snap_texel(total) : __builtin_bit_cast(uint32_t, bar_snap_float(total));
                    }
#pragma unroll
                    for (int b = 0; b < BB; ++b) it[b] = nx[b];
                }
            } else if (active) {
                const int sub = tid & (GL - 1);
                const uint32_t g = (uint32_t) tid / GL;
                const BarItem* items = a.bar_items + g;
                BarItem it[BB];
#pragma unroll
                for (int b = 0; b < BB; ++b) it[b] = items[(size_t) b * G];
                float total = 0.0f;
                for (uint32_t s0 = 0; s0 < a.bar_nsteps; s0 += BB) {
                    BarTaps tp[BB];
                    BarItem nx[BB];
#pragma unroll
                    for (int b = 0; b < BB; ++b) tp[b] = bar_item_load<false>(lrow, a.bar_w, it[b], sub);
#pragma unroll
                    for (int b = 0; b < BB; ++b) nx[b] = items[(size_t) (s0 + BB + b) * G];
                    if constexpr (BB <= kBarBatch) GLV_SCHED_FENCE();
#pragma unroll
                    for (int b = 0; b < BB; ++b) {
                        total = __builtin_fmaf(total, it[b].keep, group_sum<GL>(bar_item_lane_sum(tp[b])));
                        if (sub == 0) lres[it[b].res] = total;
                    }
#pragma unroll
                    for (int b = 0; b < BB; ++b) it[b] = nx[b];
                }
            }
            sy.sync();
            if constexpr (cols) {
                if (active) {
                    const uint16_t* ltex = reinterpret_cast<const uint16_t*>(lres);
                    float* co = a.bars_out + row * a.bars;
                    for (uint32_t x = (uint32_t) tid; x < a.bars; x += T) {
                        const ColumnMap m = a.col_map[x];
                        co[x] = column_mean(ltex[m.l], ltex[m.m], ltex[m.r]);
                    }
                }
            } else
            if (active) {
                if (GL16 && a.bars_r16 && snap) {
                    uint16_t* bo = reinterpret_cast<uint16_t*>(a.bars_out) + row * a.bars;
                    const uint32_t* lout = reinterpret_cast<const uint32_t*>(lres);
                    for (uint32_t k = (uint32_t) tid; k < a.bars; k += T) bo[k] = (uint16_t) lout[k];
                } else if (GL16 && a.bars_r16) {
                    uint16_t* bo = reinterpret_cast<uint16_t*>(a.bars_out) + row * a.bars;
                    if ((uint32_t) tid < a.bars) bo[tid] = (uint16_t) unorm16(lres[tid] / bar_wsum);
                    for (uint32_t k = (uint32_t) tid + T; k < a.bars; k += T) bo[k] = (uint16_t) unorm16(lres[k] / a.bar_desc[k].weight_sum);
                } else {
                if ((uint32_t) tid < a.bars) a.bars_out[row * a.bars + (uint32_t) tid] = lres[tid] / bar_wsum;
                for (uint32_t k = (uint32_t) tid + T; k < a.bars; k += T) a.bars_out[row * a.bars + k] = lres[k] / a.bar_desc[k].weight_sum;
                }
            }
        } else {
            if (active) finish(v, row, tid);
        }
    };
    auto row_of = [&](uint32_t base) -> uint32_t {
        const uint32_t r = base + slot;
        return r < a.units ? r : a.units - 1;
    };

    struct TrackAt { const void* win; size_t row0; };
    auto track_entry = [&](uint32_t f) -> uint32_t { if constexpr (TRACK_TABLE) return a.trk.starts[f % a.trk.steps]; else return 0u; };
    auto track_at = [&](uint32_t f, uint32_t entry) -> TrackAt {
        const uint32_t s = f / a.trk.steps, t = f - s * a.trk.steps;
        uint64_t start;
        if constexpr (TRACK_TABLE) start = (uint64_t) s * a.trk.pitch_frames + (entry < a.trk.start_max ? entry : a.trk.start_max);
        else start = (uint64_t) s * a.trk.pitch_frames + (uint64_t) t * a.trk.hop;
        return { static_cast<const char*>(a.in) + start * (TRACKF ? 8u : 4u), a.trk.step_major ? ((size_t) t * a.trk.streams + s) * 2u : (size_t) f * 2u };
    };
    (void) track_at; (void) track_entry;

    unsigned xcount = 0;
    constexpr uint32_t SEQ = SLOTS == 1 ? 2 : 1, RPI = SLOTS * SEQ;
    const uint32_t stride = gridDim.x * RPI;
    const uint32_t nsteps = a.units == 0 ? 0 : ((a.units - 1) / RPI / gridDim.x + 1) * SEQ;
    auto step_base = [&](uint32_t step) -> uint32_t {
        return blockIdx.x * RPI + (step / SEQ) * stride + (step % SEQ) * SLOTS;
    };
    const int tid_outer = tid;
    if constexpr (S16 && PREFETCH == 1) {
        const uint32_t nframes = a.units / 2;
        const uint32_t fstride = gridDim.x * SLOTS;
        const uint32_t nfs = nframes == 0 ? 0 : (nframes - 1) / fstride + 1;
        auto frame_of = [&](uint32_t m) -> uint32_t {
            const uint32_t f = blockIdx.x * SLOTS + m * fstride + slot;
            return f < nframes ? f : nframes - 1;
        };
        auto frame_ptr = [&](uint32_t f) -> const void* { return static_cast<const char*>(a.in) + (size_t) f * ((size_t) N * 4); };
        cf v[E];
        typename FR::Raw raw;
        size_t trow = 0, trow_next = 0;
        uint32_t tent = 0;
        (void) trow; (void) trow_next; (void) frame_ptr; (void) tent;
        if (blockIdx.x * SLOTS < nframes) {
            int tid = tid_outer;
            asm volatile("" : "+v"(tid));
            if constexpr (TRACK) {
                const TrackAt w = track_at(frame_of(0), track_entry(frame_of(0))); FR::load_pcm_at(raw, w.win, tid); trow = w.row0;
                if constexpr (TRACK_TABLE) tent = track_entry(frame_of(1));
            } else
            FR::template load_pcm<RING>(raw, frame_ptr(frame_of(0)), tid, a.rot);
            FR::template unpack_window<0, WSPLIT>(v, raw, win, tid, 0u, a.mono != 0);
        }
        __builtin_amdgcn_s_waitcnt(0x0F70);
        for (uint32_t r = 0; r < 2 * nfs; ++r) {
            const uint32_t m = r >> 1, ch = r & 1u;
            if (blockIdx.x * SLOTS + m * fstride >= nframes) break;
            int tid = tid_outer;
            asm volatile("" : "+v"(tid));
            const uint32_t fraw = blockIdx.x * SLOTS + m * fstride + slot;
            const bool active = fraw < nframes;
            const uint32_t f = frame_of(m);
            if constexpr (TRACK) {
                if (ch) { const TrackAt w = track_at(frame_of(m + 1), tent); FR::load_pcm_at(raw, w.win, tid); trow_next = w.row0; if constexpr (TRACK_TABLE) tent = track_entry(frame_of(m + 2)); }
            } else
            if (ch) FR::template load_pcm<RING>(raw, frame_ptr(frame_of(m + 1)), tid, a.rot);
            if constexpr (LIVE_PRE) { FR::live_prefetch(live_pre, (size_t) f * 2 + ch, tid, a); live_pre_ptr = &live_pre; }
            GLV_SCHED_FENCE();
            BD::template run<0>(v, tw_all, a.tw, xslot, tid, xcount, lds_tw, sy);
            GLV_SCHED_FENCE();
            __builtin_amdgcn_s_waitcnt(0x0F70);
            typename FR::template WinPre<WPRE> wp;
            if constexpr (WPRE > 0) { FR::template window_prefetch<WPRE>(wp, win, tid); GLV_SCHED_FENCE(); }
            if constexpr (TRACK) { finish_row(v, trow + ch, tid, active); if (ch) trow = trow_next; }
            else
            finish_row(v, (size_t) f * 2 + ch, tid, active);
            GLV_SCHED_FENCE();
            FR::template unpack_window<WPRE, WSPLIT>(v, raw, win, tid, ch ^ 1u, a.mono != 0, wp.w);
        }
        return;
    }
    if constexpr (IN_MODE == IN_F32_PLANAR && PREFETCH == 1 && LOG_E <= 4) {
        auto row_ptr = [&](uint32_t row) -> const void* { return static_cast<const char*>(a.in) + (size_t) row * ((size_t) N * 4); };
        cf v[E];
        typename FR::RawF raw;
        if (step_base(0) < a.units) {
            int tid = tid_outer;
            asm volatile("" : "+v"(tid));
            FR::load_f32_raw(raw, row_ptr(row_of(step_base(0))), tid);
            FR::window_f32_raw(v, raw, win, tid);
        }
        __builtin_amdgcn_s_waitcnt(0x0F70);
        for (uint32_t step = 0; step < nsteps; ++step) {
            const uint32_t base = step_base(step);
            if (base >= a.units) break;
            int tid = tid_outer;
            asm volatile("" : "+v"(tid));
            const bool active = base + slot < a.units;
            const uint32_t row = row_of(base);
            const uint32_t nb = step_base(step + 1);
            const bool has_next = step + 1 < nsteps && nb < a.units;
            FR::load_f32_raw(raw, row_ptr(row_of(has_next ? nb : base)), tid);
            GLV_SCHED_FENCE();
            BD::template run<0>(v, tw_all, a.tw, xslot, tid, xcount, lds_tw, sy);
            GLV_SCHED_FENCE();
            __builtin_amdgcn_s_waitcnt(0x0F70);
            finish_row(v, (size_t) row, tid, active);
            GLV_SCHED_FENCE();
            FR::window_f32_raw(v, raw, win, tid);
        }
        return;
    }
    constexpr bool F32S = IN_MODE == IN_F32_STEREO || IN_MODE == IN_F32_RING || TRACKF;
    constexpr bool RINGF = IN_MODE == IN_F32_RING;
    if constexpr (F32S && PREFETCH == 1 && LOG_E <= 4) {
        if (a.mono == 0) {
            const uint32_t nframes = a.units / 2;
            const uint32_t fstride = gridDim.x * SLOTS;
            const uint32_t nfs = nframes == 0 ? 0 : (nframes - 1) / fstride + 1;
            auto frame_of = [&](uint32_t m) -> uint32_t {
                const uint32_t f = blockIdx.x * SLOTS + m * fstride + slot;
                return f < nframes ? f : nframes - 1;
            };
            auto frame_ptr = [&](uint32_t f) -> const void* { return static_cast<const char*>(a.in) + (size_t) f * ((size_t) N * 8); };
            cf v[E];
            typename FR::RawF raw;
            size_t trow = 0, trow_next = 0;
            uint32_t tent = 0, tent_next = 0;
            (void) trow; (void) trow_next; (void) frame_ptr; (void) tent; (void) tent_next;
            if (blockIdx.x * SLOTS < nframes) {
                int tid = tid_outer;
                asm volatile("" : "+v"(tid));
                if constexpr (TRACKF) {
                    if constexpr (TRACK_TABLE) tent = track_entry(frame_of(0));
                    const TrackAt w = track_at(frame_of(0), tent); FR::template load_f32s_raw<false>(raw, w.win, tid, 0u); trow = w.row0;
                    if constexpr (TRACK_TABLE) tent_next = track_entry(frame_of(1));
                } else
                FR::template load_f32s_raw<RINGF>(raw, frame_ptr(frame_of(0)), tid, 0u, a.rot);
                FR::window_f32_raw(v, raw, win, tid);
            }
            __builtin_amdgcn_s_waitcnt(0x0F70);
            for (uint32_t r = 0; r < 2 * nfs; ++r) {
                const uint32_t m = r >> 1, ch = r & 1u;
                if (blockIdx.x * SLOTS + m * fstride >= nframes) break;
                int tid = tid_outer;
                asm volatile("" : "+v"(tid));
                const bool active = blockIdx.x * SLOTS + m * fstride + slot < nframes;
                const uint32_t f = frame_of(m);
                if constexpr (TRACKF) {
                    const TrackAt w = track_at(frame_of(m + ch), ch ? tent_next : tent);
                    FR::template load_f32s_raw<false>(raw, w.win, tid, ch ^ 1u);
                    if (ch) { trow_next = w.row0; if constexpr (TRACK_TABLE) { tent = tent_next; tent_next = track_entry(frame_of(m + 2)); } }
                } else
                FR::template load_f32s_raw<RINGF>(raw, frame_ptr(frame_of(m + ch)), tid, ch ^ 1u, a.rot);
                GLV_SCHED_FENCE();
                BD::template run<0>(v, tw_all, a.tw, xslot, tid, xcount, lds_tw, sy);
                GLV_SCHED_FENCE();
                __builtin_amdgcn_s_waitcnt(0x0F70);
                if constexpr (TRACKF) { finish_row(v, trow + ch, tid, active); if (ch) trow = trow_next; }
                else
                finish_row(v, (size_t) f * 2 + ch, tid, active);
                GLV_SCHED_FENCE();
                FR::window_f32_raw(v, raw, win, tid);
            }
            return;
        }
    }
    for (uint32_t step = 0; step < nsteps; ++step) {
        const uint32_t base = step_base(step);
        if (base >= a.units) break;
        int tid = tid_outer;
        asm volatile("" : "+v"(tid));
        const bool active = base + slot < a.units;
        const uint32_t row = row_of(base);
        cf v[E];
        if constexpr (TRACK) {
            typename FR::Raw raw;
            const TrackAt w = track_at(row >> 1, track_entry(row >> 1));
            FR::load_pcm_at(raw, w.win, tid);
            GLV_SCHED_FENCE();
            FR::template unpack_window<0, WSPLIT>(v, raw, win, tid, row & 1u, a.mono != 0);
            BD::template run<0>(v, tw_all, a.tw, xslot, tid, xcount, lds_tw, sy);
            finish_row(v, w.row0 + (row & 1u), tid, active);
            continue;
        } else
        if constexpr (TRACKF) {
            const TrackAt w = track_at(row >> 1, track_entry(row >> 1));
            FR::load_f32_stereo_window_at(v, w.win, win, tid, row & 1u, a.mono != 0);
            BD::template run<0>(v, tw_all, a.tw, xslot, tid, xcount, lds_tw, sy);
            finish_row(v, w.row0 + (row & 1u), tid, active);
            continue;
        } else
        if constexpr (S16) {
            typename FR::Raw raw;
            FR::template load_pcm<RING>(raw, static_cast<const char*>(a.in) + (size_t) (row >> 1) * ((size_t) N * 4), tid, a.rot);
            GLV_SCHED_FENCE();
            FR::template unpack_window<0, WSPLIT>(v, raw, win, tid, row & 1u, a.mono != 0);
        } else if constexpr (F32S) {
            FR::template load_f32_stereo_window<RINGF>(v, static_cast<const char*>(a.in) + (size_t) (row >> 1) * ((size_t) N * 8), win, tid,
                                                       row & 1u, a.mono != 0, a.rot);
        } else {
            FR::load_f32_window(v, static_cast<const char*>(a.in) + (size_t) row * ((size_t) N * 4), win, tid);
        }
        BD::template run<0>(v, tw_all, a.tw, xslot, tid, xcount, lds_tw, sy);
        finish_row(v, (size_t) row, tid, active);
    }
}



template <int LOG_NN, int IN_MODE, int LOG_MODE, int SLOTS, int NBUF, int TWREG, bool WINLDS, int OCC, int PREFETCH, int TILTREG,
          int LOG_E = 4, int WPRE = 0, int WPRE_S = 0>
hipError_t launch_variant(FrameClass cls, const FrameArgs& a, int grid, hipStream_t st) {
    using FR = Frame<LOG_NN, LOG_E>;
    constexpr size_t lds = frame_lds_bytes<LOG_NN, LOG_E, SLOTS, NBUF, WINLDS, TWREG>();
    static_assert(lds <= 160 * 1024, "exchange regions + window exceed the 160 KiB LDS of a gfx950 CU");
    struct AttrDone { std::atomic<bool> dev[64] = {}; };
    auto launch = [&](auto k, AttrDone& done, int threads = FR::T * SLOTS) -> hipError_t {
        if (lds > 64 * 1024) {
            int dev = 0;
            (void) hipGetDevice(&dev);
            if (dev < 0 || dev >= 64 || !done.dev[dev].load(std::memory_order_acquire)) {
                hipError_t e = hipFuncSetAttribute(reinterpret_cast<const void*>(k),
                                                   hipFuncAttributeMaxDynamicSharedMemorySize, (int) lds);
                if (e != hipSuccess) return e;
                if (dev >= 0 && dev < 64) done.dev[dev].store(true, std::memory_order_release);
            }
        }
        if (grid <= 0) return hipSuccess;
        hipLaunchKernelGGL(k, dim3(grid), dim3(threads), lds, st, a);
        return hipGetLastError();
    };
    static AttrDone done[kFrameClasses];
    constexpr int TW_STATEFUL = TWREG == 3 ? 2 : TWREG;
    auto launch_class = [&](auto c) -> hipError_t {
        constexpr int C = decltype(c)::value;
        if constexpr ((fc_fused_bars(C) && !(FR::T % 64 == 0 && NBUF == 1)) || (fc_gl16(C) && LOG_MODE == 2) || ((IN_MODE == IN_S16_TRACK || IN_MODE == IN_F32_TRACK || in_track_table(IN_MODE)) && fc_has_state(C))) return hipErrorInvalidValue;
        else if constexpr (fc_has_state(C))
            return launch(glv_frame_kernel<LOG_NN, IN_MODE, LOG_MODE, SLOTS, NBUF, TW_STATEFUL, WINLDS, OCC, PREFETCH, TILTREG, LOG_E, C, WPRE_S>, done[C]);
        else return launch(glv_frame_kernel<LOG_NN, IN_MODE, LOG_MODE, SLOTS, NBUF, TWREG, WINLDS, OCC, PREFETCH, TILTREG, LOG_E, C, WPRE>, done[C]);
    };
    switch (cls) {
        case FC_GL16_LIVE:       return launch_class(std::integral_constant<int, FC_GL16_LIVE>{});
        case FC_GL16_COLS_LIVE:  return launch_class(std::integral_constant<int, FC_GL16_COLS_LIVE>{});
        case FC_GL16_COLS:       return launch_class(std::integral_constant<int, FC_GL16_COLS>{});
        case FC_GL16_SNAP_LIVE:  return launch_class(std::integral_constant<int, FC_GL16_SNAP_LIVE>{});
        case FC_GL16_SNAP:       return launch_class(std::integral_constant<int, FC_GL16_SNAP>{});
        case FC_GL16_BARS_LIVE:  return launch_class(std::integral_constant<int, FC_GL16_BARS_LIVE>{});
        case FC_GL16_BARS:       return launch_class(std::integral_constant<int, FC_GL16_BARS>{});
        case FC_GL16:            return launch_class(std::integral_constant<int, FC_GL16>{});
        case FC_STATE_BARS_LIVE: return launch_class(std::integral_constant<int, FC_STATE_BARS_LIVE>{});
        case FC_STATE_BARS:      return launch_class(std::integral_constant<int, FC_STATE_BARS>{});
        case FC_STATE_R16:       return launch_class(std::integral_constant<int, FC_STATE_R16>{});
        case FC_STATE:           return launch_class(std::integral_constant<int, FC_STATE>{});
        case FC_R16:             return launch_class(std::integral_constant<int, FC_R16>{});
        case FC_PLAIN:           return launch_class(std::integral_constant<int, FC_PLAIN>{});
    }
    return hipErrorInvalidValue;
}

}
```

### glava_amd/csrc/glv_track.cpp

```cpp
#include "glv_host.h"
#include "glv_tables.h"

namespace {
struct TrackPlan {
    uint32_t q = 0, log_q = 0;
    uint64_t frames = 0;
    uint64_t k0 = 0;
    bool windows = false;
    bool f32 = false;
    bool to_out = false;
    bool scan = false;
    uint32_t hops_per_pitch = 0, residue_rows = 0;
    bool state = false;
    bool in16 = false;
    bool out16 = false;
    ChainPlan::Bars bars = ChainPlan::NO_BARS;
    uint64_t rows_bytes = 0, work_bytes = 0;
    uint64_t out_rows = 0;
    bool at = false;
    const uint32_t* starts = nullptr;
    bool live = false;
    uint32_t kept = 0;
};
int track_args(unsigned ops, uint32_t steps, bool live = false) {
    if (!(ops & GLV_OP_FFT)) return fail(GLV_ERR_INVALID, "a track call transforms: GLV_OP_FFT is required (ops 0x%x)", ops);
    if (live && (!(ops & GLV_OP_BARS) || !(ops & (GLV_OP_GRAVITY | GLV_OP_AVERAGE))))
        return fail(GLV_ERR_INVALID, "a live track call takes GLV_OP_FFT | GLV_OP_BARS with GLV_OP_GRAVITY and / or GLV_OP_AVERAGE (ops 0x%x)", ops);
    const unsigned allowed = GLV_OP_FFT | GLV_OP_GRAVITY | GLV_OP_AVERAGE | GLV_OP_BARS | GLV_OP_R16 | GLV_OP_PRIVATE_STATE;
    if (ops & ~allowed)
        return fail(GLV_ERR_INVALID, "a track call takes GLV_OP_FFT with GLV_OP_GRAVITY / AVERAGE / BARS / R16 only (no RAW, SMOOTH, WAVE, WRANGE, MAGNITUDE, OUTPUT_IS_STATE; ops 0x%x)", ops);
    if (steps == 0) return fail(GLV_ERR_INVALID, "steps must be > 0");
    return GLV_OK;
}
uint32_t kept_bins(const glv_batch* b, const TrackPlan& tp) {
    const uint32_t L = b->live_bins();
    if (L == 0) return 0;
    uint32_t reach = L;
    if (!tp.out16) {
        if (tp.bars != ChainPlan::BARS_F32 || b->p.sample_mode != GLV_SAMPLE_AVERAGE || b->p.bars >= glv::kBarSeqMin) return 0;
        reach = b->bar_x.chunk_reach;
    }
    const uint32_t K = glv::track_kept_bins(L, reach);
    if (K >= b->p.n) return 0;
    for (int v = 0; v < glv::frame_variants(b->log_nn); ++v)
        if (K > 2u * (uint32_t) glv::frame_geometry(b->log_nn, v).live_points) return 0;
    return K;
}
int track_chain(const glv_batch* b, uint32_t pitch_frames, uint32_t steps, unsigned ops, TrackPlan& tp, bool columns = false, bool live = false) {
    static const float some_output = 0.0f;
    if (b->p.gl_storage == 2) return fail(GLV_ERR_STATE, "gl_storage 2 is the pass-by-pass checker form: a track call runs on gl_storage 0 and 1");
    if (live) {
        if (!(b->ops_mask & GLV_OP_BARS_ONLY))
            return fail(GLV_ERR_STATE, "the batch was not created with GLV_OP_BARS_ONLY: its track entries are glv_batch_track_windows_* / glv_batch_track_columns_*");
        columns = b->columns();
    } else if (b->ops_mask & GLV_OP_BARS_ONLY)
        return fail(GLV_ERR_STATE, "the batch was created with GLV_OP_BARS_ONLY: its state beyond the live bins does not exist, which the scan over time would read");
    if (b->columns() && !columns) return fail(GLV_ERR_STATE, "column texels are set (glv_batch_set_column_texels): a track call has no columns form");
    if (columns && !b->columns())
        return fail(GLV_ERR_STATE, "no column texels are set (glv_batch_set_column_texels): bars and bar texels are tracked by glv_batch_track_windows_s16 / _f32");
    if (b->single_row) return fail(GLV_ERR_STATE, "a track call needs a batch of stereo streams");
    if (int rc = check_ops(b, ops, &some_output)) return rc;
    tp.out_rows = (uint64_t) steps * b->streams * 2u;
    if (tp.out_rows > 0xffffffffull)
        return fail(GLV_ERR_INVALID, "steps=%u of %u streams at pitch_frames=%u: more than 2^32 rows in one call, cut the track into chunks", steps, b->streams, pitch_frames);
    tp.state = (ops & (GLV_OP_GRAVITY | GLV_OP_AVERAGE)) != 0;
    tp.live = live;
    if (columns) {
        tp.bars = ChainPlan::BARS_COLUMNS_TEXELS; tp.in16 = tp.out16 = true;
        if (live) tp.kept = kept_bins(b, tp);
        return GLV_OK;
    }
    const bool gl = tp.state && b->state16;
    const bool snap = (ops & GLV_OP_BARS) && b->snapped();
    if (!(ops & GLV_OP_BARS)) tp.bars = ChainPlan::NO_BARS;
    else if (snap) tp.bars = b->p.sample_mode != GLV_SAMPLE_AVERAGE ? ChainPlan::BARS_SNAP_MODE : b->p.log_mode != 2 ? ChainPlan::BARS_SNAP : ChainPlan::BARS_SNAP_FLOATS;
    else if (gl && b->p.bars >= glv::kBarSeqMin && b->bar_x.i8()) tp.bars = b->p.log_mode != 2 ? ChainPlan::BARS_I8 : ChainPlan::BARS_I8_FLOATS;
    else tp.bars = ChainPlan::BARS_F32;
    tp.in16 = tp.state ? gl : ((ops & GLV_OP_R16) && !(ops & GLV_OP_BARS));
    tp.out16 = (ops & GLV_OP_BARS) ? (tp.bars == ChainPlan::BARS_I8 || tp.bars == ChainPlan::BARS_SNAP) : (ops & GLV_OP_R16) != 0;
    if (live) tp.kept = kept_bins(b, tp);
    return GLV_OK;
}
uint64_t up256(uint64_t v) { return (v + 255u) & ~(uint64_t) 255u; }
bool pitch_too_short(uint32_t n, uint32_t pitch_frames, uint32_t hop, uint32_t steps) {
    if ((uint64_t) pitch_frames >= (uint64_t) n + (uint64_t) (steps - 1) * hop) return false;
    (void) fail(GLV_ERR_INVALID, "pitch_frames=%u holds fewer than steps=%u windows of n=%u frames every hop=%u", pitch_frames, steps, n, hop);
    return true;
}
int plan_track(const glv_batch* b, uint32_t pitch_frames, uint32_t hop, uint32_t steps, unsigned ops, TrackPlan& tp) {
    const uint32_t n = b->p.n;
    if (int rc = track_args(ops, steps)) return rc;
    const int lh = log2_exact(hop);
    if (lh < 2 || hop > n) return fail(GLV_ERR_INVALID, "hop=%u: must be a power of two in [4, n=%u]", hop, n);
    if (pitch_frames % hop != 0) return fail(GLV_ERR_INVALID, "pitch_frames=%u is not a multiple of hop=%u", pitch_frames, hop);
    if (pitch_too_short(n, pitch_frames, hop, steps)) return GLV_ERR_INVALID;
    if (int rc = track_chain(b, pitch_frames, steps, ops, tp)) return rc;
    tp.q = n / hop; tp.log_q = (uint32_t) log2_exact(tp.q);
    tp.frames = (uint64_t) (b->streams - 1) * pitch_frames + (uint64_t) (steps - 1) * hop + n;
    tp.k0 = tp.frames / n;
    if (2u * tp.k0 > 0xffffffffull || (uint64_t) b->streams * (pitch_frames / hop) + steps > 0xffffffffull)
        return fail(GLV_ERR_INVALID, "steps=%u of %u streams at pitch_frames=%u: more than 2^32 rows in one call, cut the track into chunks", steps, b->streams, pitch_frames);
    tp.scan = true; tp.hops_per_pitch = pitch_frames / hop; tp.residue_rows = (uint32_t) (2u * tp.k0);
    tp.rows_bytes = up256((uint64_t) tp.q * 2u * tp.k0 * n * (tp.in16 ? 2u : 4u));
    tp.work_bytes = tp.rows_bytes + ((ops & GLV_OP_BARS) ? up256(tp.out_rows * n * (tp.out16 ? 2u : 4u)) : 0u);
    return GLV_OK;
}
int windows_args(uint32_t n, uint32_t pitch_frames, uint32_t hop, uint32_t steps, bool at) {
    if (at) return pitch_frames >= n ? GLV_OK : fail(GLV_ERR_INVALID, "pitch_frames=%u holds no window of n=%u frames", pitch_frames, n);
    if (hop == 0) return fail(GLV_ERR_INVALID, "hop must be > 0");
    return pitch_too_short(n, pitch_frames, hop, steps) ? GLV_ERR_INVALID : GLV_OK;
}
void windows_geometry(const glv_batch* b, uint32_t steps, unsigned ops, TrackPlan& tp) {
    const uint32_t n = b->p.n;
    tp.windows = true; tp.scan = tp.state; tp.hops_per_pitch = steps;
    tp.to_out = !tp.state && !(ops & GLV_OP_BARS);
    if (tp.to_out) { tp.rows_bytes = 0; tp.work_bytes = 256; return; }
    tp.rows_bytes = up256(tp.out_rows * n * (tp.in16 ? 2u : 4u));
    tp.work_bytes = tp.rows_bytes + (tp.state && (ops & GLV_OP_BARS) ? up256(tp.out_rows * n * (tp.out16 ? 2u : 4u)) : 0u);
}
int plan_track_windows(const glv_batch* b, uint32_t pitch_frames, uint32_t hop, uint32_t steps, unsigned ops, TrackPlan& tp) {
    if (int rc = track_args(ops, steps)) return rc;
    if (int rc = windows_args(b->p.n, pitch_frames, hop, steps, tp.at)) return rc;
    if (int rc = track_chain(b, pitch_frames, steps, ops, tp)) return rc;
    windows_geometry(b, steps, ops, tp);
    return GLV_OK;
}
int plan_track_columns(const glv_batch* b, uint32_t pitch_frames, uint32_t hop, uint32_t steps, unsigned ops, TrackPlan& tp) {
    if (int rc = track_args(ops, steps)) return rc;
    if (!(ops & GLV_OP_BARS)) return fail(GLV_ERR_INVALID, "a columns track call samples: GLV_OP_BARS is required (ops 0x%x)", ops);
    if (int rc = windows_args(b->p.n, pitch_frames, hop, steps, tp.at)) return rc;
    if (int rc = track_chain(b, pitch_frames, steps, ops, tp, true)) return rc;
    windows_geometry(b, steps, ops, tp);
    return GLV_OK;
}
int plan_track_live(const glv_batch* b, uint32_t pitch_frames, uint32_t hop, uint32_t steps, unsigned ops, TrackPlan& tp) {
    if (int rc = track_args(ops, steps, true)) return rc;
    if (int rc = windows_args(b->p.n, pitch_frames, hop, steps, tp.at)) return rc;
    if (int rc = track_chain(b, pitch_frames, steps, ops, tp, false, true)) return rc;
    windows_geometry(b, steps, ops, tp);
    return GLV_OK;
}
int plan_track_at(const glv_batch* b, uint32_t pitch_frames, uint32_t hop, uint32_t steps, unsigned ops, TrackPlan& tp) {
    tp.at = true;
    if (b->ops_mask & GLV_OP_BARS_ONLY) return plan_track_live(b, pitch_frames, hop, steps, ops, tp);
    if (b->columns()) return plan_track_columns(b, pitch_frames, hop, steps, ops, tp);
    return plan_track_windows(b, pitch_frames, hop, steps, ops, tp);
}

int refuse_track_pointers(const void* d_pcm, bool f32, const void* d_out, const void* d_work) {
    if (!d_pcm || !d_out || !d_work) return fail(GLV_ERR_INVALID, "NULL device pointer");
    if (f32 && (reinterpret_cast<uintptr_t>(d_pcm) & 7u)) return fail(GLV_ERR_INVALID, "d_pcm must be aligned like a float frame: 8 bytes");
    if (reinterpret_cast<uintptr_t>(d_work) & 255u) return fail(GLV_ERR_INVALID, "d_work must be 256-byte aligned");
    return GLV_OK;
}
int track_residues(glv_batch* b, const TrackPlan& tp, glv::FrameArgs& a, glv::FrameClass cls, const int16_t* d_pcm, uint32_t hop, char* work, hipStream_t st) {
    const uint32_t n = b->p.n;
    for (uint32_t r = 0; r < tp.q; ++r) {
        const uint64_t k_r = (tp.frames - (uint64_t) r * hop) / n;
        if (k_r == 0) continue;
        a.in = d_pcm + (size_t) r * hop * 2u;
        a.out = reinterpret_cast<float*>(work + (size_t) r * 2u * tp.k0 * n * (tp.in16 ? 2u : 4u));
        a.units = (uint32_t) (2u * k_r);
        int variant = 0, grid = 0;
        launch_plan(b, a.units, glv::IN_S16_STEREO, a.ops, &variant, &grid);
        b->last_grid = grid; b->last_variant = variant;
        const hipError_t e = glv::launch_frame(b->log_nn, glv::IN_S16_STEREO, (int) b->p.log_mode, variant, cls, a, grid, st);
        if (e != hipSuccess) return fail(GLV_ERR_HIP, "kernel launch failed: %s", hipGetErrorString(e));
    }
    b->last_launches += (int) tp.q;
    return GLV_OK;
}
int track_windows(glv_batch* b, const TrackPlan& tp, glv::FrameArgs& a, glv::FrameClass cls, const void* d_pcm, uint32_t pitch_frames, uint32_t hop, uint32_t steps,
                        float* rows, hipStream_t st) {
    a.in = d_pcm; a.out = rows; a.units = (uint32_t) tp.out_rows;
    a.trk.pitch_frames = pitch_frames; a.trk.hop = hop; a.trk.steps = steps; a.trk.streams = b->streams; a.trk.step_major = tp.state ? 0u : 1u;
    a.trk.pad = 0; a.trk.starts = tp.starts; a.trk.start_max = pitch_frames - b->p.n; a.trk.pad2 = 0;
    const int hop_mode = tp.f32 ? glv::IN_F32_TRACK : glv::IN_S16_TRACK;
    const int mode = !tp.starts ? hop_mode : tp.f32 ? glv::IN_F32_TRACK_AT : glv::IN_S16_TRACK_AT;
    int variant = 0, grid = 0;
    launch_plan(b, a.units, hop_mode, a.ops, &variant, &grid);
    b->last_grid = grid; b->last_variant = variant;
    const hipError_t e = glv::launch_frame(b->log_nn, mode, (int) b->p.log_mode, variant, cls, a, grid, st); ++b->last_launches;
    if (e != hipSuccess) return fail(GLV_ERR_HIP, "kernel launch failed: %s", hipGetErrorString(e));
    b->kernel_name = "glv_frame_kernel";
    return GLV_OK;
}
int track_scan(glv_batch* b, const TrackPlan& tp, glv::FrameArgs& a, uint32_t steps, const char* work, float* out, unsigned ops, hipStream_t st) {
    a.in = work; a.out = out;
    a.units = b->streams * 2u; a.ops = ops & (GLV_OP_GRAVITY | GLV_OP_AVERAGE);
    a.grav = b->grav_cur; a.grav_w = b->d_grav; a.hist = b->d_hist; a.head = b->head;
    a.grav_sub = b->grav_sub; a.grav_int = b->grav_int ? 1u : 0u; a.gl_storage = tp.in16 && tp.state ? 1u : 0u;
    glv::TrackGeometry g;
    g.n = b->p.n; g.steps = steps; g.hops_per_pitch = tp.hops_per_pitch; g.log_q = tp.log_q; g.residue_rows = tp.residue_rows; g.out_texels = tp.out16 ? 1u : 0u;
    g.kept = tp.kept != 0 ? tp.kept : b->p.n;
    const hipError_t e = glv::launch_track_scan(a, g, tp.in16, st); ++b->last_launches;
    if (e != hipSuccess) return fail(GLV_ERR_HIP, "scan launch failed: %s", hipGetErrorString(e));
    b->kernel_name = "glv_track_scan_kernel";
    if (ops & GLV_OP_AVERAGE) b->head = (uint32_t) (((uint64_t) b->head + steps) % b->p.avg_frames);
    if ((ops & GLV_OP_GRAVITY) && !(ops & GLV_OP_AVERAGE)) b->grav_cur = b->d_grav;
    return GLV_OK;
}
int track_columns(glv_batch* b, const TrackPlan& tp, const float* rows, float* out, hipStream_t st) {
    const hipError_t e = glv::launch_columns_texels(reinterpret_cast<const uint16_t*>(rows), out, (size_t) tp.out_rows, b->p.n,
                                                    (uint32_t) b->snap_x.tex.size(), b->p.bars, b->snap_x.col_nsteps, b->snap_x.col_items, b->snap.desc, b->snap.w,
                                                    b->snap_x.col_map, b->p.sample_mode, shape_hybrid(b->p), st);
    ++b->last_launches;
    if (e != hipSuccess) return fail(GLV_ERR_HIP, "columns launch failed: %s", hipGetErrorString(e));
    b->kernel_name = "glv_columns_kernel";
    return GLV_OK;
}
const char* bars_kernel_name(const glv_batch* b, ChainPlan::Bars bars) {
    switch (bars) {
        case ChainPlan::BARS_I8: case ChainPlan::BARS_I8_FLOATS: return "glv_bars_rows_i8_kernel";
        case ChainPlan::BARS_SNAP: case ChainPlan::BARS_SNAP_FLOATS: return "glv_bars_snap_kernel";
        case ChainPlan::BARS_SNAP_MODE: return "glv_bars_mode_kernel";
        default: return b->p.sample_mode != GLV_SAMPLE_AVERAGE ? "glv_bars_mode_kernel" : b->p.bars >= glv::kBarSeqMin ? "glv_bars_rows_kernel" : "glv_bars_kernel";
    }
}
int track(glv_batch* b, const TrackPlan& tp, const void* d_pcm, uint32_t pitch_frames, uint32_t hop, uint32_t steps, void* d_out, void* d_work, unsigned ops, hipStream_t st) {
    if (int rc = refuse_track_pointers(d_pcm, tp.f32, d_out, d_work)) return rc;
    if (int rc = refuse_gravity_mix(b, ops)) return rc;
    if (int rc = refuse_stale_tilt(b)) return rc;
    b->last_launches = 0;
    HIP_TRY(hipSetDevice(b->device));
    commit_gravity_form(b, ops);
    char* const work = static_cast<char*>(d_work);
    float* const out = static_cast<float*>(d_out);
    if (int rc = timed_launch_begin(b, st)) return rc;
    glv::FrameArgs a;
    fill_common(a, b->p, b->tab);
    a.ops = GLV_OP_FFT | (tp.in16 ? (unsigned) GLV_OP_R16 : 0u); a.log_mode = b->p.log_mode;
    const glv::FrameClass cls = glv::frame_class(false, false, false, a.ops);
    if (tp.kept != 0) b->ran_live = true;
    if (int rc = tp.windows ? track_windows(b, tp, a, cls, d_pcm, pitch_frames, hop, steps, tp.to_out ? out : reinterpret_cast<float*>(work), st)
                            : track_residues(b, tp, a, cls, static_cast<const int16_t*>(d_pcm), hop, work, st)) return rc;
    ChainPlan pl;
    pl.bars = tp.bars;
    pl.rows = reinterpret_cast<float*>(work + (tp.scan ? tp.rows_bytes : 0u));
    if (tp.scan) if (int rc = track_scan(b, tp, a, steps, work, (ops & GLV_OP_BARS) ? pl.rows : out, ops, st)) return rc;
    if (tp.bars == ChainPlan::BARS_COLUMNS_TEXELS) { if (int rc = track_columns(b, tp, pl.rows, out, st)) return rc; }
    else if (int rc = launch_bars_pass(b, pl, out, (size_t) steps * b->streams * 2u, (ops & GLV_OP_R16) != 0, st)) return rc;
    else if (tp.live) b->kernel_name = bars_kernel_name(b, tp.bars);
    return timed_launch_end(b, st);
}

struct TrackWavePlan {
    bool f32 = false;
    bool at = false;
    ChainPlan pl;
    bool one_launch = false;
    uint64_t rows = 0;
    uint64_t work_bytes = 256;
};
int plan_track_wave(const glv_batch* b, uint32_t pitch_frames, uint32_t hop, uint32_t steps, unsigned ops, TrackWavePlan& tp) {
    static const float some_output = 0.0f;
    const uint32_t n = b->p.n;
    if (!(ops & GLV_OP_WAVE)) return fail(GLV_ERR_INVALID, "a wave track call needs GLV_OP_WAVE (ops 0x%x; GLV_OP_FFT chains: glv_batch_track_s16)", ops);
    if (ops & ~(unsigned) (GLV_OP_WAVE | GLV_OP_BARS | GLV_OP_R16))
        return fail(GLV_ERR_INVALID, "a wave track call takes GLV_OP_WAVE with GLV_OP_BARS / GLV_OP_R16 only (ops 0x%x)", ops);
    if (steps == 0) return fail(GLV_ERR_INVALID, "steps must be > 0");
    if (int rc = windows_args(n, pitch_frames, hop, steps, tp.at)) return rc;
    if (b->single_row) return fail(GLV_ERR_STATE, "a track call needs a batch of stereo streams");
    tp.rows = (uint64_t) steps * b->streams * 2u;
    if (tp.rows > 0x100000000ull)
        return fail(GLV_ERR_INVALID, "steps=%u of %u streams: more than 2^32 rows in one call, cut the track into chunks", steps, b->streams);
    if (int rc = check_ops(b, ops, &some_output)) return rc;
    const int in_mode = tp.f32 ? glv::IN_F32_STEREO : glv::IN_S16_STEREO;
    if (int rc = plan_wave(b, in_mode, ops, 0, nullptr, tp.pl, false)) return rc;
    if (ops & GLV_OP_BARS) {
        ChainPlan grouped;
        if (int rc = plan_wave(b, in_mode, ops, 0, nullptr, grouped, !tp.at && hop % 8u == 0u && pitch_frames % 8u == 0u)) return rc;
        tp.one_launch = grouped.wave_fused;
        tp.work_bytes = up256(tp.rows * n * (tp.pl.wave_r16 ? 2u : 4u));
    }
    return GLV_OK;
}

int track_wave(glv_batch* b, const void* d_pcm, bool f32, uint32_t pitch_frames, uint32_t hop, uint32_t steps, void* d_out, void* d_work, unsigned ops, hipStream_t st,
               const uint32_t* d_starts = nullptr) {
    if (int rc = refuse_track_pointers(d_pcm, f32, d_out, d_work)) return rc;
    TrackWavePlan tp;
    tp.f32 = f32; tp.at = d_starts != nullptr;
    if (int rc = plan_track_wave(b, pitch_frames, hop, steps, ops, tp)) return rc;
    ChainPlan& pl = tp.pl;
    const bool fused = tp.one_launch && (reinterpret_cast<uintptr_t>(d_pcm) & 31u) == 0u;
    b->last_launches = 0;
    HIP_TRY(hipSetDevice(b->device));
    const bool mono = b->p.channels == 1, r16 = (ops & GLV_OP_R16) != 0;
    glv::WaveWindows w;
    w.units = b->streams * 2u; w.steps = steps; w.hop = hop; w.pitch_frames = pitch_frames;
    w.starts = d_starts; w.start_max = pitch_frames - b->p.n;
    w.by_steps = b->track_wave_by_steps && (4ull * w.units + 2u) * b->p.bars * 4u <= 0xffffffffull ? 1u : 0u;
    if (int rc = timed_launch_begin(b, st)) return rc;
    hipError_t e;
    if (fused) {
        const glv::BarIRowsTables irt = b->bar_x.irows_tables();
        e = glv::launch_bars_i8_pcm_track(d_pcm, w, mono, d_out, b->p.n, b->p.bars, &irt, st, r16);
        b->kernel_name = "glv_bars_rows_i8_kernel";
    } else {
        if (ops & GLV_OP_BARS) pl.out = pl.rows = static_cast<float*>(d_work);
        else pl.out = static_cast<float*>(d_out);
        e = glv::launch_wave_track(d_pcm, f32, w, mono, b->p.n, pl.out, pl.wave_r16, pl.wave_limit, st);
        b->kernel_name = "glv_wave_kernel";
    }
    ++b->last_launches;
    if (e != hipSuccess) return fail(GLV_ERR_HIP, "kernel launch failed: %s", hipGetErrorString(e));
    if (!fused) if (int rc = launch_bars_pass(b, pl, static_cast<float*>(d_out), (size_t) tp.rows, r16, st)) return rc;
    return timed_launch_end(b, st);
}

template <class Plan>
uint64_t planned_work_bytes(const glv_batch* b, int (*plan)(const glv_batch*, uint32_t, uint32_t, uint32_t, unsigned, Plan&), uint32_t pitch_frames, uint32_t hop, uint32_t steps,
                            unsigned ops, bool at = false) {
    if (!b) { (void) fail(GLV_ERR_INVALID, "batch is NULL"); return 0; }
    Plan tp;
    tp.at = at;
    if (const int rc = plan(b, pitch_frames, hop, steps, ops, tp)) {
        g_err = std::string(rc == GLV_ERR_STATE ? "GLV_ERR_STATE: " : "GLV_ERR_INVALID: ") + g_err;
        return 0;
    }
    return tp.work_bytes;
}
int track_at(glv_batch* b, const void* d_pcm, bool f32, uint32_t pitch_frames, const uint32_t* d_starts, uint32_t steps, void* d_out, void* d_work, unsigned ops, hipStream_t st) {
    if (!b) return fail(GLV_ERR_INVALID, "batch is NULL");
    if (!d_starts) return fail(GLV_ERR_INVALID, "NULL device pointer");
    if (reinterpret_cast<uintptr_t>(d_starts) & 3u) return fail(GLV_ERR_INVALID, "d_starts must be 4-byte aligned");
    if (ops & GLV_OP_WAVE) return track_wave(b, d_pcm, f32, pitch_frames, 0u, steps, d_out, d_work, ops, st, d_starts);
    TrackPlan tp;
    if (int rc = plan_track_at(b, pitch_frames, 0u, steps, ops, tp)) return rc;
    tp.f32 = f32; tp.starts = d_starts;
    return track(b, tp, d_pcm, pitch_frames, 0u, steps, d_out, d_work, ops, st);
}
}
// ... 110 lines not shown
```

### glava_amd/csrc/glv_tune.hip

```cpp
#include <cstring>
#include <vector>

#include "glv_kernel_tmpl.h"
#include "glv_winsplit.h"
#include "glv_tables.h"

#ifndef GLV_TUNE_LOG_NN
#define GLV_TUNE_LOG_NN 11
#endif
#ifndef GLV_TUNE_IN_MODE
#define GLV_TUNE_IN_MODE IN_S16_STEREO
#endif

namespace glv {
namespace {

struct Variant {
    const char* desc;
    hipError_t (*launch)(int in_mode, int log_mode, const FrameArgs& a, int grid, hipStream_t st);
    int slots;
};

template <int SLOTS, int NBUF, int TWREG, bool WINLDS, int OCC, int PF = 0, int TL = 0, int LE = 4, int WP = 0, int WPS = 0>
hipError_t launch_v(int in_mode, int log_mode, const FrameArgs& a, int grid, hipStream_t st) {
    constexpr int K = GLV_TUNE_LOG_NN;
    if (in_mode != IN_S16_STEREO) return hipErrorInvalidValue;
    const FrameClass cls = frame_class(false, false, false, a.ops);
#if !defined(GLV_TUNE_NO_LOG0)
    if (log_mode == 0) return launch_variant<K, GLV_TUNE_IN_MODE, 0, SLOTS, NBUF, TWREG, WINLDS, OCC, PF, TL, LE, WP, WPS>(cls, a, grid, st);
#endif
    return launch_variant<K, GLV_TUNE_IN_MODE, 1, SLOTS, NBUF, TWREG, WINLDS, OCC, PF, TL, LE, WP, WPS>(cls, a, grid, st);
}

#define V(S, NB, TR, WL, OC) { "slots=" #S " nbuf=" #NB " twreg=" #TR " winlds=" #WL " occ=" #OC, launch_v<S, NB, TR, WL, OC>, S }
#define VX(S, NB, TR, WL, OC, PF, TL) { "slots=" #S " nbuf=" #NB " twreg=" #TR " winlds=" #WL " occ=" #OC " pf=" #PF " tiltreg=" #TL, launch_v<S, NB, TR, WL, OC, PF, TL>, S }
#define VE(S, NB, TR, WL, OC, PF, TL, LE) { "slots=" #S " nbuf=" #NB " twreg=" #TR " winlds=" #WL " occ=" #OC " pf=" #PF " tiltreg=" #TL " log_e=" #LE, launch_v<S, NB, TR, WL, OC, PF, TL, LE>, S }
#define VW(S, NB, TR, WL, OC, PF, TL, LE, WP, WPS) { "slots=" #S " nbuf=" #NB " twreg=" #TR " winlds=" #WL " occ=" #OC " pf=" #PF " tiltreg=" #TL " log_e=" #LE " wpre=" #WP " wpre_s=" #WPS, launch_v<S, NB, TR, WL, OC, PF, TL, LE, WP, WPS>, S }
#define VP(S, NB, TR, WL, OC) { "slots=" #S " nbuf=" #NB " twreg=" #TR " winlds=" #WL " occ=" #OC " prefetch", launch_v<S, NB, TR, WL, OC, true>, S }
const Variant kVariants[] = {
#ifdef GLV_TUNE_VARIANTS
    GLV_TUNE_VARIANTS
#else
    V(2, 1, false, false, 2), V(2, 1, false, false, 3), V(2, 1, false, false, 4),
    V(2, 1, false, true, 2),  V(2, 1, false, true, 4),
    V(2, 1, true, false, 2),  V(2, 1, true, false, 3),
    V(4, 1, false, false, 3), V(4, 1, false, false, 4), V(4, 1, false, true, 4),
    V(2, 2, false, false, 4), V(4, 2, false, false, 4),
#endif
};
#undef V
#undef VP
#undef VX
#undef VE
#undef VW

}
}

extern "C" {
int glv_tune_count(void) { return (int) (sizeof(glv::kVariants) / sizeof(glv::kVariants[0])); }
const char* glv_tune_describe(int i) { return glv::kVariants[i].desc; }
int glv_tune_slots(int i) { return glv::kVariants[i].slots; }
int glv_tune_log_nn(void) { return GLV_TUNE_LOG_NN; }
int glv_tune_launch(int i, int in_mode, int log_mode, const glv::FrameArgs* a, int grid, void* stream) {
    return (int) glv::kVariants[i].launch(in_mode, log_mode, *a, grid, (hipStream_t) stream);
}

int glv_tune_run2(int i, const void* d_pcm, float* d_out, unsigned units, int log_mode, int grid, int iters,
                  void* stream, float* ms, unsigned extra_ops, float* d_grav);
int glv_tune_run3(int i, const void* d_pcm, float* d_out, unsigned units, int log_mode, int grid, int iters,
                  void* stream, float* ms, unsigned extra_ops, float* d_grav, float* d_hist);
int glv_tune_run(int i, const void* d_pcm, float* d_out, unsigned units, int log_mode, int grid, int iters,
                 void* stream, float* ms) {
    return glv_tune_run2(i, d_pcm, d_out, units, log_mode, grid, iters, stream, ms, 0u, nullptr);
}
int glv_tune_run2(int i, const void* d_pcm, float* d_out, unsigned units, int log_mode, int grid, int iters,
                  void* stream, float* ms, unsigned extra_ops, float* d_grav) {
    return glv_tune_run3(i, d_pcm, d_out, units, log_mode, grid, iters, stream, ms, extra_ops, d_grav, nullptr);
}
int glv_tune_run3(int i, const void* d_pcm, float* d_out, unsigned units, int log_mode, int grid, int iters,
                  void* stream, float* ms, unsigned extra_ops, float* d_grav, float* d_hist) {
    using namespace glv;
    static cf* d_tw = nullptr;
    static double* d_win = nullptr;
    static float* d_win_split = nullptr;
    static LogEntry* d_log = nullptr;
    static float* d_tilt = nullptr;
    static float* d_tilt_fast = nullptr;
    constexpr int NN = 1 << GLV_TUNE_LOG_NN, N = 2 * NN;
    if (!d_tw) {
        std::vector<cf> tw(NN, cf{0.0f, 0.0f});
        std::vector<double> win(N);
        make_twiddles(tw.data(), NN);
        make_window(win.data(), N);
        if (hipMalloc(&d_tw, sizeof(cf) * NN) != hipSuccess) return -1;
        if (hipMalloc(&d_win, sizeof(double) * N) != hipSuccess) return -1;
        (void) hipMemcpy(d_tw, tw.data(), sizeof(cf) * NN, hipMemcpyHostToDevice);
        (void) hipMemcpy(d_win, win.data(), sizeof(double) * N, hipMemcpyHostToDevice);
        if (hipMalloc(&d_win_split, sizeof(float) * 2 * N) != hipSuccess) return -1;
        int* d_fs = nullptr;
        if (hipMalloc(&d_fs, 2 * sizeof(int)) != hipSuccess) return -1;
        (void) hipMemset(d_fs, 0, 2 * sizeof(int));
        (void) launch_window_split_impl(d_win, d_win_split, N, d_fs, nullptr);
        (void) hipDeviceSynchronize();
        (void) hipFree(d_fs);
        LogEntry lt[kLogTabMaxSize];
        make_log_table(lt);
        if (hipMalloc(&d_log, sizeof(lt)) != hipSuccess) return -1;
        (void) hipMemcpy(d_log, lt, sizeof(lt), hipMemcpyHostToDevice);
        std::vector<float> tl(N);
        make_tilt(tl.data(), N, 10.2f, 0.3f);
        if (hipMalloc(&d_tilt, sizeof(float) * N) != hipSuccess) return -1;
        (void) hipMemcpy(d_tilt, tl.data(), sizeof(float) * N, hipMemcpyHostToDevice);
        make_tilt(tl.data(), N, 10.2f, 0.3f, true);
        if (hipMalloc(&d_tilt_fast, sizeof(float) * N) != hipSuccess) return -1;
        (void) hipMemcpy(d_tilt_fast, tl.data(), sizeof(float) * N, hipMemcpyHostToDevice);
    }
    FrameArgs a;
    std::memset(&a, 0, sizeof(a));
    a.in = d_pcm; a.out = d_out; a.tw = d_tw; a.win = d_win; a.win_split = d_win_split; a.logtab = d_log; a.tilt = log_mode == 1 ? d_tilt_fast : d_tilt; a.units = units * 2; a.ops = OP_FFT | extra_ops; a.grav = d_grav; a.grav_w = d_grav;
    a.F = d_hist ? 5 : 1; a.hist = d_hist; a.avg_window = 1;
    make_frame_weights(a.wts, a.F, true, 0);
    a.inv_n = 1.0f / (float) N; a.fft_scale = 10.2f; a.one_minus_cutoff = 1.0f - 0.3f;
    a.g = 4.2f * (1.0f / 86.1328125f); a.F_as_float = (float) a.F;
    hipStream_t st = (hipStream_t) stream;
    if (grid <= 0) {
        const unsigned slots = (unsigned) kVariants[i].slots;
        const unsigned wgs = (units * 2 + slots - 1) / slots;
        grid = (int) (wgs < 2048u ? wgs : 2048u);
    }
    hipEvent_t e0, e1;
    (void) hipEventCreate(&e0); (void) hipEventCreate(&e1);
    hipError_t e = kVariants[i].launch(IN_S16_STEREO, log_mode, a, grid, st);
    if (e != hipSuccess) return (int) e;
    (void) hipEventRecord(e0, st);
    for (int it = 0; it < iters; ++it) {
        e = kVariants[i].launch(IN_S16_STEREO, log_mode, a, grid, st);
        if (e != hipSuccess) return (int) e;
    }
    (void) hipEventRecord(e1, st);
    if (hipEventSynchronize(e1) != hipSuccess) return -2;
    float t = 0;
    (void) hipEventElapsedTime(&t, e0, e1);
    *ms = t / (float) iters;
    (void) hipEventDestroy(e0); (void) hipEventDestroy(e1);
    return 0;
}
}
```

### glava_amd/csrc/glv_wisdom.cpp

```cpp
#include <atomic>
#include <cstdio>
#include <cstdlib>
#include <mutex>

#include "glv_host.h"

namespace {
struct WisdomKey { uint32_t n, in_kind, ops_class, log_mode, streams_log2, avg_frames, cus; char device[48]; };
struct WisdomEntry { WisdomKey k; int variant, grid; float ms; };
std::mutex g_wisdom_mu;
std::vector<WisdomEntry> g_wisdom;
std::atomic<uint64_t> g_wisdom_gen{1};
bool g_wisdom_env_loaded = false;

uint32_t log2_round(uint32_t v) { uint32_t l = 0; while ((2u << l) <= v) ++l; return ((v >> l << l) * 3 / 2 <= v && l < 31) ? l + 1 : l; }
bool same_key(const WisdomKey& a, const WisdomKey& b) {
    return a.n == b.n && a.in_kind == b.in_kind && a.ops_class == b.ops_class && a.log_mode == b.log_mode && a.streams_log2 == b.streams_log2
           && a.avg_frames == b.avg_frames && a.cus == b.cus && std::strncmp(a.device, b.device, sizeof(a.device)) == 0;
}
void key_set_device(WisdomKey& k, const char* name, uint32_t cus) {
    std::memset(k.device, 0, sizeof(k.device));
    size_t j = 0;
    for (const char* c = name; *c && j + 1 < sizeof(k.device); ++c) k.device[j++] = (*c == ' ' || *c == '\t' || *c == '\n') ? '_' : *c;
    if (j == 0) std::strcpy(k.device, "unknown");
    k.cus = cus;
}
bool wisdom_lookup(const WisdomKey& k, int* variant, int* grid) {
    std::lock_guard<std::mutex> lock(g_wisdom_mu);
    for (const WisdomEntry& e : g_wisdom) if (same_key(e.k, k)) { *variant = e.variant; *grid = e.grid; return true; }
    return false;
}
void wisdom_store(const WisdomKey& k, int variant, int grid, float ms) {
    std::lock_guard<std::mutex> lock(g_wisdom_mu);
    g_wisdom_gen.fetch_add(1, std::memory_order_release);
    for (WisdomEntry& e : g_wisdom) if (same_key(e.k, k)) { e.variant = variant; e.grid = grid; e.ms = ms; return; }
    g_wisdom.push_back(WisdomEntry{k, variant, grid, ms});
}
int wisdom_load_file(const char* path, int* skipped = nullptr, int* v1 = nullptr) {
    FILE* f = std::fopen(path, "r");
    if (!f) { (void) fail(GLV_ERR_INVALID, "cannot open wisdom file %s", path); return -1; }
    char line[320];
    int n_loaded = 0, n_skipped = 0, n_v1 = 0;
    while (std::fgets(line, sizeof(line), f)) {
        if (line[0] == '#' || line[0] == '\n') continue;
        WisdomKey k; int variant, grid; float ms; char dev[48];
        std::memset(&k, 0, sizeof(k));
        if (std::sscanf(line, "%47s %u %u %u %u %u %u %u %d %d %f", dev, &k.cus, &k.n, &k.in_kind, &k.ops_class, &k.log_mode, &k.streams_log2,
                        &k.avg_frames, &variant, &grid, &ms) == 11 && grid > 0 && variant >= 0) {
            key_set_device(k, dev, k.cus);
            wisdom_store(k, variant, grid, ms); ++n_loaded;
        } else {
            ++n_skipped;
            unsigned a[5]; int g1; float m1; char tail[8];
            if (std::sscanf(line, "%u %u %u %u %u %d %f %7s", &a[0], &a[1], &a[2], &a[3], &a[4], &g1, &m1, tail) == 7) ++n_v1;
        }
    }
    std::fclose(f);
    if (skipped) *skipped = n_skipped;
    if (v1) *v1 = n_v1;
    return n_loaded;
}

uint32_t wisdom_class(const glv_batch* b, unsigned ops) {
    const unsigned f = frame_ops(b, ops);
    return (uint32_t) glv::frame_class(gl_fused_chain(b, ops), (f & GLV_OP_BARS) != 0, false, f);
}

WisdomKey wisdom_key(const glv_batch* b, int in_mode, unsigned ops) {
    WisdomKey k;
    std::memset(&k, 0, sizeof(k));
    k.n = b->p.n; k.in_kind = (uint32_t) in_mode; k.ops_class = wisdom_class(b, ops); k.log_mode = b->p.log_mode;
    k.streams_log2 = log2_round(b->streams);
    k.avg_frames = (frame_ops(b, ops) & GLV_OP_AVERAGE) ? b->p.avg_frames : 0;
    key_set_device(k, b->device_name, (uint32_t) b->num_cus);
    return k;
}

int default_grid(const glv_batch* b, uint32_t units, int variant) {
    const glv::FrameGeometry g = glv::frame_geometry(b->log_nn, variant);
    const uint32_t wgs = (units + g.rows_per_trip - 1) / g.rows_per_trip;
    const uint32_t round = (uint32_t) b->num_cus * (uint32_t) g.resident;
    if (wgs <= round) return (int) wgs;
    uint32_t grid = wgs / 8u;
    if (grid < round) grid = round;
    if (grid > (uint32_t) g.rounds * round) grid = (uint32_t) g.rounds * round;
    return (int) grid;
}
}
namespace glvh __attribute__((visibility("hidden"))) {
void launch_plan(glv_batch* b, uint32_t units, int in_mode, unsigned ops, int* variant, int* grid) {
    int v = 0, g = 0;
    const uint32_t cls = wisdom_class(b, ops);
    if (b->variant_override < 0 || b->grid_override <= 0) {
        glv_batch::PlanCache& pc = b->plan_cache[in_mode][cls];
        const uint64_t gen = g_wisdom_gen.load(std::memory_order_acquire);
        if (pc.gen != gen) {
            pc.hit = wisdom_lookup(wisdom_key(b, in_mode, ops), &pc.variant, &pc.grid);
            if (!pc.hit && (in_mode == glv::IN_S16_RING || in_mode == glv::IN_S16_TRACK)) pc.hit = wisdom_lookup(wisdom_key(b, glv::IN_S16_STEREO, ops), &pc.variant, &pc.grid);
            if (!pc.hit && in_mode == glv::IN_F32_TRACK) pc.hit = wisdom_lookup(wisdom_key(b, glv::IN_F32_STEREO, ops), &pc.variant, &pc.grid);
            pc.gen = gen;
        }
        if (pc.hit) { v = pc.variant; g = pc.grid; }
    }
    if (b->variant_override >= 0) { if (b->variant_override != v) g = 0; v = b->variant_override; }
    if (!glv::frame_variant_ok(b->log_nn, in_mode, (int) b->p.log_mode, v)) { v = 0; g = 0; }
    if (b->grid_override > 0) g = b->grid_override;
    else if (g > 0) {
        const int rpt = glv::frame_geometry(b->log_nn, v).rows_per_trip;
        const uint32_t wgs_max = (units + rpt - 1) / rpt;
        if ((uint32_t) g > wgs_max) g = (int) wgs_max;
    } else g = default_grid(b, units, v);
    *variant = v; *grid = g;
}

void wisdom_load_env() {
    std::unique_lock<std::mutex> lock(g_wisdom_mu);
    const bool first = !g_wisdom_env_loaded;
    g_wisdom_env_loaded = true;
    lock.unlock();
    if (first) if (const char* w = std::getenv("GLV_WISDOM")) {
        int skipped = 0, v1 = 0;
        const int nl = wisdom_load_file(w, &skipped, &v1);
        if (nl >= 0 && skipped > 0)
            std::fprintf(stderr, "glv: GLV_WISDOM=%s: %d entries loaded, %d line(s) skipped%s\n", w, nl, skipped, v1 ? " (7-field v1 format: re-tune)" : "");
    }
}
}

extern "C" {
int glv_wisdom_clear(void) {
    std::lock_guard<std::mutex> lock(g_wisdom_mu);
    g_wisdom.clear();
    g_wisdom_gen.fetch_add(1, std::memory_order_release);
    return GLV_OK;
}
int glv_wisdom_count(void) { std::lock_guard<std::mutex> lock(g_wisdom_mu); return (int) g_wisdom.size(); }
int glv_wisdom_load(const char* path) {
    if (!path) return fail(GLV_ERR_INVALID, "path is NULL");
    int skipped = 0, v1 = 0;
    const int n = wisdom_load_file(path, &skipped, &v1);
    if (n < 0) return GLV_ERR_INVALID;
    if (skipped > 0) {
        const int code = n == 0 ? GLV_ERR_INVALID : GLV_OK;
        (void) fail(code, "wisdom file %s: %d entr%s loaded, %d line(s) skipped%s", path, n, n == 1 ? "y" : "ies", skipped,
                    v1 ? " (some are in the 7-field v1 format of an older library: re-tune with glv_batch_autotune and save again)" : " (not in the 11-field v2 format)");
        return code;
    }
    g_err = "";
    return GLV_OK;
}
int glv_wisdom_save(const char* path) {
    if (!path) return fail(GLV_ERR_INVALID, "path is NULL");
    FILE* f = std::fopen(path, "w");
    if (!f) return fail(GLV_ERR_INVALID, "cannot write wisdom file %s", path);
    std::fprintf(f, "# glv launch wisdom v2: device compute_units n input_kind ops_class log_mode log2(streams) avg_frames variant workgroups ms_per_launch\n");
    std::lock_guard<std::mutex> lock(g_wisdom_mu);
    for (const WisdomEntry& e : g_wisdom)
        std::fprintf(f, "%s %u %u %u %u %u %u %u %d %d %.6f\n", e.k.device, e.k.cus, e.k.n, e.k.in_kind, e.k.ops_class, e.k.log_mode, e.k.streams_log2,
                     e.k.avg_frames, e.variant, e.grid, (double) e.ms);
    std::fclose(f);
    return GLV_OK;
}

int glv_batch_autotune(glv_batch* b, const int16_t* d_pcm, float* d_out, unsigned ops, void* hip_stream, int* best_grid, float* best_ms) {
    if (!b) return fail(GLV_ERR_INVALID, "batch is NULL");
    if (!(ops & GLV_OP_FFT)) return fail(GLV_ERR_INVALID, "autotune needs GLV_OP_FFT (it tunes the frame kernel)");
    if (int rc = check_ops(b, ops, d_out)) return rc;
    if (!d_pcm) return fail(GLV_ERR_INVALID, "NULL device pointer");
    hipStream_t st = (hipStream_t) hip_stream;
    HIP_TRY(hipSetDevice(b->device));
    const uint32_t units = b->streams * 2;
    struct Cand { int variant, grid; };
    std::vector<Cand> cand;
    for (int v = 0; v < glv::frame_variants(b->log_nn); ++v) {
        if (!glv::frame_variant_ok(b->log_nn, glv::IN_S16_STEREO, (int) b->p.log_mode, v)) continue;
        const glv::FrameGeometry geo = glv::frame_geometry(b->log_nn, v);
        const uint32_t wgs = (units + geo.rows_per_trip - 1) / geo.rows_per_trip;
        const uint32_t round = (uint32_t) b->num_cus * (uint32_t) geo.resident;
        for (uint32_t g : { round / 2, round, round * 3 / 2, round * 2, round * 4 }) {
            const int c = (int) (g < 1 ? 1 : (g > wgs ? wgs : g));
            bool dup = false;
            for (const Cand& x : cand) dup |= x.variant == v && x.grid == c;
            if (!dup) cand.push_back(Cand{v, c});
        }
    }
    EventPair ev; HIP_TRY(ev.create());
    const hipEvent_t e0 = ev.e0, e1 = ev.e1;
    const int saved_grid = b->grid_override, saved_variant = b->variant_override;
    Cand best{0, 0}; float bms = 0.f; int rc = GLV_OK;
    for (int pass = 0; pass < 2 && rc == GLV_OK; ++pass)
        for (const Cand& c : cand) {
            b->grid_override = c.grid; b->variant_override = c.variant;
            const int iters = pass == 0 ? 3 : 8;
            if (hipEventRecord(e0, st) != hipSuccess) { rc = fail(GLV_ERR_HIP, "hipEventRecord failed"); break; }
            for (int i = 0; i < iters && rc == GLV_OK; ++i) rc = process(b, d_pcm, glv::IN_S16_STEREO, d_out, ops, units, 0, st);
            if (rc != GLV_OK) break;
            float ms = 0.f;
            if (hipEventRecord(e1, st) != hipSuccess || hipEventSynchronize(e1) != hipSuccess || hipEventElapsedTime(&ms, e0, e1) != hipSuccess) {
                rc = fail(GLV_ERR_HIP, "event timing failed"); break;
            }
            ms /= (float) iters;
            if (pass == 1 && (best.grid == 0 || ms < bms)) { best = c; bms = ms; }
        }
    b->grid_override = saved_grid; b->variant_override = saved_variant;
    if (rc != GLV_OK) return rc;
    if (ops & (GLV_OP_GRAVITY | GLV_OP_AVERAGE)) { if (int r2 = glv_batch_reset(b)) return r2; }
    wisdom_store(wisdom_key(b, glv::IN_S16_STEREO, ops), best.variant, best.grid, bms);
    if (best_grid) *best_grid = best.grid;
    if (best_ms) *best_ms = bms;
    return GLV_OK;
}

int glv_batch_set_grid(glv_batch* b, int grid) {
    if (!b) return fail(GLV_ERR_INVALID, "batch is NULL");
    b->grid_override = grid;
    return GLV_OK;
}
int glv_batch_set_variant(glv_batch* b, int variant) {
    if (!b) return fail(GLV_ERR_INVALID, "batch is NULL");
    if (variant >= glv::frame_variants(b->log_nn))
        return fail(GLV_ERR_INVALID, "variant %d: n=%u has %d kernel configuration(s)", variant, b->p.n, glv::frame_variants(b->log_nn));
    b->variant_override = variant < 0 ? -1 : variant;
    return GLV_OK;
}
int glv_batch_variants(const glv_batch* b) { return b ? glv::frame_variants(b->log_nn) : 0; }
int glv_batch_last_variant(const glv_batch* b) { return b ? b->last_variant : 0; }

int glv_batch_describe_variant(const glv_batch* b, int variant, char* buf, size_t len) {
    if (!b || !buf || len == 0) return fail(GLV_ERR_INVALID, "NULL argument");
    if (variant < 0 || variant >= glv::frame_variants(b->log_nn)) return fail(GLV_ERR_INVALID, "variant %d out of range", variant);
    const glv::FrameGeometry g = glv::frame_geometry(b->log_nn, variant);
    std::snprintf(buf, len, "n=%u variant %d: %d points per lane, %d lanes per row, %d row(s) per workgroup, %d workgroup(s) per CU, "
                            "%d KiB LDS, twiddles %s, window %s", b->p.n, variant, 1 << g.log_e, g.lanes, g.slots, g.resident, (g.lds_bytes + 1023) / 1024,
                  g.twreg == 1 ? "in VGPRs" : g.twreg == 0 ? "through L2" : g.twreg == 4 ? (g.nbuf == 0 ? "in LDS (split exchange)" : "in LDS") : "middle passes in LDS, last pass through L2",
                  g.winlds ? "in LDS" : "through L2");
    return GLV_OK;
}
}
```

Measured before the change: 104.8 million.

## Add tapered multi-round workgroup plans to balance frame kernel tail

Introduces a RoundPlan that splits frames into several rounds of workgroups with decreasing sizes (two-thirds taper), so the last wave of work is smaller and tail imbalance across CUs shrinks. The kernel now derives its frame range and stride from the round it belongs to instead of a single grid-stride loop. The default plan enables tapering only for log_nn==11 (4096-point) or when GLV_GRID_CUS is set. A timeline probe behind a tune-only macro is also added. This adds per-workgroup plan lookup overhead and changes the memory access order.

Result: faster. 107.3 million (median of 5 runs) (+2.4%).

```diff
diff --git a/glava_amd/build.py b/glava_amd/build.py
--- a/glava_amd/build.py
+++ b/glava_amd/build.py
@@ -22,7 +22,7 @@
 def _inst_jobs(obj_dir: str, sizes, extra: list[str]):
     return [("glv_inst.hip", os.path.join(obj_dir, f"glv_inst_{k}_{p}.o"), [f"-DGLV_LOG_NN={k}", f"-DGLV_INST_PART={p}", *extra])
             for k in sorted(sizes, reverse=True) for p in PARTS]
-HEADERS = ["glv_core.h", "glv_frame.h", "glv_kernel_tmpl.h", "glv_launch.h", "glv_launch_util.h", "glv_tables.h", "glv_winsplit.h", "glv_host.h",
+HEADERS = ["glv_core.h", "glv_frame.h", "glv_round_plan.h", "glv_kernel_tmpl.h", "glv_launch.h", "glv_launch_util.h", "glv_tables.h", "glv_winsplit.h", "glv_host.h",
            os.path.join("..", "..", "include", "glv_spectrum.h")]
 
 
diff --git a/glava_amd/csrc/glv_api.cpp b/glava_amd/csrc/glv_api.cpp
--- a/glava_amd/csrc/glv_api.cpp
+++ b/glava_amd/csrc/glv_api.cpp
@@ -70,6 +70,7 @@
     b->unfused_wave = std::getenv("GLV_UNFUSED_WAVE") != nullptr;
     if (const char* o = std::getenv("GLV_TRACK_WAVE_ORDER")) b->track_wave_by_steps = std::strcmp(o, "steps") == 0;
     b->bar_i8_off = std::getenv("GLV_NO_BARS_I8") != nullptr;
+    if (const char* o = std::getenv("GLV_GRID_CUS")) { const int v = std::atoi(o); b->grid_cus = v > 0 ? v : 0; }
     b->log_nn = log2_exact(p->n) - 1;
     hipDeviceProp_t prop;
     if (hipGetDeviceProperties(&prop, device) == hipSuccess) {
diff --git a/glava_amd/csrc/glv_chain.cpp b/glava_amd/csrc/glv_chain.cpp
--- a/glava_amd/csrc/glv_chain.cpp
+++ b/glava_amd/csrc/glv_chain.cpp
@@ -184,7 +184,7 @@
     if (gl_fused_chain(b, ops)) pl.route = ChainPlan::GL_FUSED;
     else if (ops & GLV_OP_FFT) pl.route = gl_passes ? ChainPlan::GL_PASSES : ChainPlan::FRAME;
     else pl.route = (ops & (GLV_OP_GRAVITY | GLV_OP_AVERAGE | GLV_OP_WRANGE | GLV_OP_MAGNITUDE | GLV_OP_R16)) ? ChainPlan::POST : ChainPlan::COPY;
-    if (ops & GLV_OP_FFT) launch_plan(b, units, in_mode, ops, &pl.variant, &pl.grid);
+    if (ops & GLV_OP_FFT) launch_plan(b, units, in_mode, ops, &pl.variant, &pl.grid, &pl.rounds);
     const bool snap = (ops & GLV_OP_BARS) && b->snapped();
     pl.fused_bars = (ops & GLV_OP_BARS) && (ops & GLV_OP_FFT) && !gl_passes && bars_fusable(b, ops) && pl.variant < kMaxVariants
                     && (snap ? b->snap : b->bar).fusable[pl.variant];
@@ -275,6 +275,7 @@
         b->kernel_name = pl.route == ChainPlan::POST ? "glv_post_kernel" : "glv_smooth_kernel";
     } else {
         b->last_grid = pl.grid; b->last_variant = pl.variant;
+        a.plan = pl.rounds;
         e = glv::launch_frame(b->log_nn, in_mode, (int) b->p.log_mode, pl.variant, pl.cls, a, pl.grid, st); ++b->last_launches;
         if (pl.route == ChainPlan::FRAME) b->kernel_name = "glv_frame_kernel";
     }
diff --git a/glava_amd/csrc/glv_core.h b/glava_amd/csrc/glv_core.h
--- a/glava_amd/csrc/glv_core.h
+++ b/glava_amd/csrc/glv_core.h
@@ -4,7 +4,7 @@
 #include <stdint.h>
 
 #if !defined(GLV_TUNE_BUILD)
-#if defined(GLV_ROWS_RB) || defined(GLV_BAR_BATCH_BIG) || defined(GLV_STATE_PAIR_MAX)
+#if defined(GLV_ROWS_RB) || defined(GLV_BAR_BATCH_BIG) || defined(GLV_STATE_PAIR_MAX) || defined(GLV_WG_TIMELINE)
 #error "tuning macros are for tools/tune.py A/B builds: compile with -DGLV_TUNE_BUILD (glava_amd.build.build_variant does); the product never defines them"
 #endif
 #endif
diff --git a/glava_amd/csrc/glv_frame.h b/glava_amd/csrc/glv_frame.h
--- a/glava_amd/csrc/glv_frame.h
+++ b/glava_amd/csrc/glv_frame.h
@@ -1,6 +1,7 @@
 #pragma once
 
 #include "glv_core.h"
+#include "glv_round_plan.h"
 
 namespace glv {
 
@@ -108,6 +109,10 @@
     uint32_t bar_nsteps;
     const ColumnMap* col_map;
     TrackWindows trk;
+    RoundPlan plan;
+#if defined(GLV_WG_TIMELINE)
+    uint64_t* wg_timeline;
+#endif
 };
 
 constexpr int kBarTaps = 8;
diff --git a/glava_amd/csrc/glv_host.h b/glava_amd/csrc/glv_host.h
--- a/glava_amd/csrc/glv_host.h
+++ b/glava_amd/csrc/glv_host.h
@@ -135,6 +135,7 @@
     uint32_t head = 0;
     uint32_t ring_pos = 0;
     int grid_override = 0;
+    int grid_cus = 0;
     int variant_override = -1;
     int attr_log_mode = -1;
     int last_launches = 0;
@@ -210,6 +211,7 @@
                 BARS_COLUMNS,
                 BARS_COLUMNS_TEXELS } bars = NO_BARS;
     int variant = 0, grid = 0;
+    glv::RoundPlan rounds = {};
     glv::FrameClass cls = glv::FC_PLAIN;
     unsigned ops = 0;
     bool fused_bars = false;
@@ -221,7 +223,7 @@
     uint32_t wave_limit = 0;
 };
 
-    void launch_plan(glv_batch* b, uint32_t units, int in_mode, unsigned ops, int* variant, int* grid);
+    void launch_plan(glv_batch* b, uint32_t units, int in_mode, unsigned ops, int* variant, int* grid, glv::RoundPlan* rounds);
     void wisdom_load_env();
     void state_free(void* p);
     int batch_alloc(glv_batch* b);
diff --git a/glava_amd/csrc/glv_kernel_tmpl.h b/glava_amd/csrc/glv_kernel_tmpl.h
--- a/glava_amd/csrc/glv_kernel_tmpl.h
+++ b/glava_amd/csrc/glv_kernel_tmpl.h
@@ -110,6 +110,27 @@
     }
 };
 
+struct WgTimeline {
+#if defined(GLV_WG_TIMELINE)
+    uint64_t t_entry = 0, t_first = 0;
+    __device__ __forceinline__ void entry() { t_entry = wall_clock64(); }
+    __device__ __forceinline__ void first() { t_first = wall_clock64(); }
+    __device__ __forceinline__ void exit(const FrameArgs& a) {
+        const uint64_t t_exit = wall_clock64();
+        if (threadIdx.x == 0 && a.wg_timeline) {
+            uint64_t* o = a.wg_timeline + (size_t) blockIdx.x * 5;
+            o[0] = (uint64_t) blockIdx.x | (uint64_t) (uint32_t) __builtin_amdgcn_s_getreg(4 | (31 << 11)) << 32;
+            o[1] = (uint64_t) (uint32_t) __builtin_amdgcn_s_getreg(20 | (31 << 11));
+            o[2] = t_entry; o[3] = t_first; o[4] = t_exit;
+        }
+    }
+#else
+    __device__ __forceinline__ void entry() {}
+    __device__ __forceinline__ void first() {}
+    __device__ __forceinline__ void exit(const FrameArgs&) {}
+#endif
+};
+
 template <int LOG_NN, int LOG_E, int SLOTS, int NBUF, bool WINLDS, int TWREG = 0>
 constexpr size_t frame_lds_bytes() {
     return (size_t) SLOTS * (NBUF == 0 ? sizeof(float) : NBUF * sizeof(cf)) * Frame<LOG_NN, LOG_E>::XREGION + (WINLDS ? (size_t) Frame<LOG_NN, LOG_E>::N * sizeof(double) : 0)
@@ -141,6 +162,8 @@
     constexpr size_t XBYTES = (size_t) FR::XREGION * (NBUF == 0 ? sizeof(float) : sizeof(cf));
     constexpr int NREG = NBUF == 0 ? 1 : NBUF;
 
+    WgTimeline tl;
+    tl.entry();
     extern __shared__ __attribute__((aligned(16))) char smem[];
     constexpr int NTHREADS = T * SLOTS;
     const uint32_t slot = maybe_scalar<WAVE_SLOT>(threadIdx.x / T);
@@ -327,10 +350,6 @@
             if (active) finish(v, row, tid);
         }
     };
-    auto row_of = [&](uint32_t base) -> uint32_t {
-        const uint32_t r = base + slot;
-        return r < a.units ? r : a.units - 1;
-    };
 
     struct TrackAt { const void* win; size_t row0; };
     auto track_entry = [&](uint32_t f) -> uint32_t { if constexpr (TRACK_TABLE) return a.trk.starts[f % a.trk.steps]; else return 0u; };
@@ -345,18 +364,26 @@
 
     unsigned xcount = 0;
     constexpr uint32_t SEQ = SLOTS == 1 ? 2 : 1, RPI = SLOTS * SEQ;
-    const uint32_t stride = gridDim.x * RPI;
-    const uint32_t nsteps = a.units == 0 ? 0 : ((a.units - 1) / RPI / gridDim.x + 1) * SEQ;
+    static_assert(SLOTS == 1 || SLOTS % 2 == 0, "a round's frames are whole trips of the row loops");
+    const RoundView rv = plan_round_of(a.plan, blockIdx.x, gridDim.x, (a.units + 1u) / 2u);
+    const uint32_t row0 = 2u * rv.f0, rend = 2u * rv.fend < a.units ? 2u * rv.fend : a.units;
+    const uint32_t stride = rv.wgs * RPI;
+    const uint32_t nsteps = rend <= row0 ? 0 : ((rend - row0 - 1) / RPI / rv.wgs + 1) * SEQ;
     auto step_base = [&](uint32_t step) -> uint32_t {
-        return blockIdx.x * RPI + (step / SEQ) * stride + (step % SEQ) * SLOTS;
+        return row0 + rv.wg * RPI + (step / SEQ) * stride + (step % SEQ) * SLOTS;
+    };
+    auto row_of = [&](uint32_t base) -> uint32_t {
+        const uint32_t r = base + slot;
+        return r < rend ? r : rend - 1;
     };
     const int tid_outer = tid;
     if constexpr (S16 && PREFETCH == 1) {
-        const uint32_t nframes = a.units / 2;
-        const uint32_t fstride = gridDim.x * SLOTS;
-        const uint32_t nfs = nframes == 0 ? 0 : (nframes - 1) / fstride + 1;
+        const uint32_t nframes = rv.fend;
+        const uint32_t fstride = rv.wgs * SLOTS;
+        const uint32_t fwg = rv.f0 + rv.wg * SLOTS;
+        const uint32_t nfs = nframes <= rv.f0 ? 0 : (nframes - rv.f0 - 1) / fstride + 1;
         auto frame_of = [&](uint32_t m) -> uint32_t {
-            const uint32_t f = blockIdx.x * SLOTS + m * fstride + slot;
+            const uint32_t f = fwg + m * fstride + slot;
             return f < nframes ? f : nframes - 1;
         };
         auto frame_ptr = [&](uint32_t f) -> const void* { return static_cast<const char*>(a.in) + (size_t) f * ((size_t) N * 4); };
@@ -365,7 +392,7 @@
         size_t trow = 0, trow_next = 0;
         uint32_t tent = 0;
         (void) trow; (void) trow_next; (void) frame_ptr; (void) tent;
-        if (blockIdx.x * SLOTS < nframes) {
+        if (fwg < nframes) {
             int tid = tid_outer;
             asm volatile("" : "+v"(tid));
             if constexpr (TRACK) {
@@ -376,12 +403,13 @@
             FR::template unpack_window<0, WSPLIT>(v, raw, win, tid, 0u, a.mono != 0);
         }
         __builtin_amdgcn_s_waitcnt(0x0F70);
+        tl.first();
         for (uint32_t r = 0; r < 2 * nfs; ++r) {
             const uint32_t m = r >> 1, ch = r & 1u;
-            if (blockIdx.x * SLOTS + m * fstride >= nframes) break;
+            if (fwg + m * fstride >= nframes) break;
             int tid = tid_outer;
             asm volatile("" : "+v"(tid));
-            const uint32_t fraw = blockIdx.x * SLOTS + m * fstride + slot;
+            const uint32_t fraw = fwg + m * fstride + slot;
             const bool active = fraw < nframes;
             const uint32_t f = frame_of(m);
             if constexpr (TRACK) {
@@ -401,28 +429,30 @@
             GLV_SCHED_FENCE();
             FR::template unpack_window<WPRE, WSPLIT>(v, raw, win, tid, ch ^ 1u, a.mono != 0, wp.w);
         }
+        tl.exit(a);
         return;
     }
     if constexpr (IN_MODE == IN_F32_PLANAR && PREFETCH == 1 && LOG_E <= 4) {
         auto row_ptr = [&](uint32_t row) -> const void* { return static_cast<const char*>(a.in) + (size_t) row * ((size_t) N * 4); };
         cf v[E];
         typename FR::RawF raw;
-        if (step_base(0) < a.units) {
+        if (step_base(0) < rend) {
             int tid = tid_outer;
             asm volatile("" : "+v"(tid));
             FR::load_f32_raw(raw, row_ptr(row_of(step_base(0))), tid);
             FR::window_f32_raw(v, raw, win, tid);
         }
         __builtin_amdgcn_s_waitcnt(0x0F70);
+        tl.first();
         for (uint32_t step = 0; step < nsteps; ++step) {
             const uint32_t base = step_base(step);
-            if (base >= a.units) break;
+            if (base >= rend) break;
             int tid = tid_outer;
             asm volatile("" : "+v"(tid));
-            const bool active = base + slot < a.units;
+            const bool active = base + slot < rend;
             const uint32_t row = row_of(base);
             const uint32_t nb = step_base(step + 1);
-            const bool has_next = step + 1 < nsteps && nb < a.units;
+            const bool has_next = step + 1 < nsteps && nb < rend;
             FR::load_f32_raw(raw, row_ptr(row_of(has_next ? nb : base)), tid);
             GLV_SCHED_FENCE();
             BD::template run<0>(v, tw_all, a.tw, xslot, tid, xcount, lds_tw, sy);
@@ -432,17 +462,19 @@
             GLV_SCHED_FENCE();
             FR::window_f32_raw(v, raw, win, tid);
         }
+        tl.exit(a);
         return;
     }
     constexpr bool F32S = IN_MODE == IN_F32_STEREO || IN_MODE == IN_F32_RING || TRACKF;
     constexpr bool RINGF = IN_MODE == IN_F32_RING;
     if constexpr (F32S && PREFETCH == 1 && LOG_E <= 4) {
         if (a.mono == 0) {
-            const uint32_t nframes = a.units / 2;
-            const uint32_t fstride = gridDim.x * SLOTS;
-            const uint32_t nfs = nframes == 0 ? 0 : (nframes - 1) / fstride + 1;
+            const uint32_t nframes = rv.fend;
+            const uint32_t fstride = rv.wgs * SLOTS;
+            const uint32_t fwg = rv.f0 + rv.wg * SLOTS;
+            const uint32_t nfs = nframes <= rv.f0 ? 0 : (nframes - rv.f0 - 1) / fstride + 1;
             auto frame_of = [&](uint32_t m) -> uint32_t {
-                const uint32_t f = blockIdx.x * SLOTS + m * fstride + slot;
+                const uint32_t f = fwg + m * fstride + slot;
                 return f < nframes ? f : nframes - 1;
             };
             auto frame_ptr = [&](uint32_t f) -> const void* { return static_cast<const char*>(a.in) + (size_t) f * ((size_t) N * 8); };
@@ -451,7 +483,7 @@
             size_t trow = 0, trow_next = 0;
             uint32_t tent = 0, tent_next = 0;
             (void) trow; (void) trow_next; (void) frame_ptr; (void) tent; (void) tent_next;
-            if (blockIdx.x * SLOTS < nframes) {
+            if (fwg < nframes) {
                 int tid = tid_outer;
                 asm volatile("" : "+v"(tid));
                 if constexpr (TRACKF) {
@@ -463,12 +495,13 @@
                 FR::window_f32_raw(v, raw, win, tid);
             }
             __builtin_amdgcn_s_waitcnt(0x0F70);
+            tl.first();
             for (uint32_t r = 0; r < 2 * nfs; ++r) {
                 const uint32_t m = r >> 1, ch = r & 1u;
-                if (blockIdx.x * SLOTS + m * fstride >= nframes) break;
+                if (fwg + m * fstride >= nframes) break;
                 int tid = tid_outer;
                 asm volatile("" : "+v"(tid));
-                const bool active = blockIdx.x * SLOTS + m * fstride + slot < nframes;
+                const bool active = fwg + m * fstride + slot < nframes;
                 const uint32_t f = frame_of(m);
                 if constexpr (TRACKF) {
                     const TrackAt w = track_at(frame_of(m + ch), ch ? tent_next : tent);
@@ -486,15 +519,17 @@
                 GLV_SCHED_FENCE();
                 FR::window_f32_raw(v, raw, win, tid);
             }
+            tl.exit(a);
             return;
         }
     }
+    tl.first();
     for (uint32_t step = 0; step < nsteps; ++step) {
         const uint32_t base = step_base(step);
-        if (base >= a.units) break;
+        if (base >= rend) break;
         int tid = tid_outer;
         asm volatile("" : "+v"(tid));
-        const bool active = base + slot < a.units;
+        const bool active = base + slot < rend;
         const uint32_t row = row_of(base);
         cf v[E];
         if constexpr (TRACK) {
@@ -528,6 +563,7 @@
         BD::template run<0>(v, tw_all, a.tw, xslot, tid, xcount, lds_tw, sy);
         finish_row(v, (size_t) row, tid, active);
     }
+    tl.exit(a);
 }
 
 
diff --git a/glava_amd/csrc/glv_round_plan.h b/glava_amd/csrc/glv_round_plan.h
--- /dev/null
+++ b/glava_amd/csrc/glv_round_plan.h
@@ -0,0 +1,83 @@
+#pragma once
+
+#include <stdint.h>
+
+namespace glv {
+
+constexpr int kMaxRounds = 8;
+struct Round { uint32_t wg0, wgs, f0, frames; };
+struct RoundPlan { uint32_t n, pad[3]; Round r[kMaxRounds]; };
+
+enum TaperRule : int { TAPER_EQUAL = 0, TAPER_HALF = 1, TAPER_TWO_THIRDS = 2 };
+
+inline uint32_t plan_workgroups(const RoundPlan& p) { return p.n == 0 ? 0u : p.r[p.n - 1].wg0 + p.r[p.n - 1].wgs; }
+
+inline constexpr uint32_t plan_frame(const Round& r, uint32_t b, uint32_t slots, uint32_t s, uint32_t m) {
+    const uint64_t f = (uint64_t) r.f0 + (uint64_t) (b - r.wg0) * slots + s + (uint64_t) m * ((uint64_t) r.wgs * slots);
+    return f < (uint64_t) r.f0 + r.frames ? (uint32_t) f : ~0u;
+}
+
+inline RoundPlan plan_single(uint32_t frames, uint32_t grid) {
+    RoundPlan p = {};
+    p.n = 1; p.r[0] = Round{0u, grid, 0u, frames};
+    return p;
+}
+
+inline uint32_t plan_equal_grid(uint32_t frames, uint32_t slots, uint32_t cus, uint32_t resident, int max_rounds) {
+    const uint32_t wgs = (frames + slots - 1) / slots, round = cus * resident;
+    if (wgs <= round) return wgs;
+    uint32_t grid = wgs / 8u;
+    if (grid < round) grid = round;
+    if (grid > (uint32_t) max_rounds * round) grid = (uint32_t) max_rounds * round;
+    return grid;
+}
+
+inline RoundPlan plan_rounds(uint32_t frames, uint32_t slots, uint32_t cus, uint32_t resident, int max_rounds, TaperRule rule) {
+    if (max_rounds > kMaxRounds) max_rounds = kMaxRounds;
+    const uint32_t round = cus * resident;
+    const uint64_t per_trip = (uint64_t) round * slots;
+    const uint64_t trips = per_trip ? (frames + per_trip - 1) / per_trip : 0;
+    if (rule == TAPER_EQUAL || max_rounds < 2 || trips < 2 || frames == 0)
+        return plan_single(frames, plan_equal_grid(frames, slots, cus, resident, max_rounds < 1 ? 1 : max_rounds));
+    uint64_t t[kMaxRounds];
+    int n = 0;
+    uint64_t sum = 0;
+    while (n < max_rounds && sum < trips) {
+        uint64_t want = n == 0 ? 1 : (rule == TAPER_HALF ? sum : 2 * sum);
+        if (want > trips - sum) want = trips - sum;
+        t[n++] = want; sum += want;
+    }
+    t[n - 1] += trips - sum;
+    RoundPlan p = {};
+    uint64_t f = 0;
+    uint32_t wg = 0;
+    for (int i = n - 1; i >= 0; --i) {
+        uint64_t fr = t[i] * per_trip;
+        if (fr > frames - f) fr = frames - f;
+        if (fr == 0) break;
+        const uint64_t need = (fr + slots - 1) / slots;
+        Round& r = p.r[p.n++];
+        r.wg0 = wg; r.wgs = (uint32_t) (need < round ? need : round); r.f0 = (uint32_t) f; r.frames = (uint32_t) fr;
+        wg += r.wgs; f += fr;
+    }
+    return p;
+}
+
+inline RoundPlan plan_default(uint32_t frames, uint32_t slots, uint32_t cus, uint32_t resident, int max_rounds, bool taper) {
+    const uint64_t per_trip = (uint64_t) cus * resident * slots;
+    const uint64_t trips = per_trip ? (frames + per_trip - 1) / per_trip : 0;
+    if (!taper || trips / 8u < 2u) return plan_rounds(frames, slots, cus, resident, max_rounds, TAPER_EQUAL);
+    const int rounds = trips / 8u < (uint64_t) max_rounds ? (int) (trips / 8u) : max_rounds;
+    return plan_rounds(frames, slots, cus, resident, rounds, TAPER_TWO_THIRDS);
+}
+
+struct RoundView { uint32_t wg, wgs, f0, fend; };
+inline constexpr RoundView plan_round_of(const RoundPlan& p, uint32_t b, uint32_t grid, uint32_t nframes) {
+    if (p.n == 0) return RoundView{b, grid, 0u, nframes};
+    RoundView v{b - p.r[0].wg0, p.r[0].wgs, p.r[0].f0, p.r[0].f0 + p.r[0].frames};
+    for (int k = 1; k < kMaxRounds; ++k)
+        if ((uint32_t) k < p.n && b >= p.r[k].wg0) v = RoundView{b - p.r[k].wg0, p.r[k].wgs, p.r[k].f0, p.r[k].f0 + p.r[k].frames};
+    return v;
+}
+
+}
diff --git a/glava_amd/csrc/glv_track.cpp b/glava_amd/csrc/glv_track.cpp
--- a/glava_amd/csrc/glv_track.cpp
+++ b/glava_amd/csrc/glv_track.cpp
@@ -162,7 +162,7 @@
         a.out = reinterpret_cast<float*>(work + (size_t) r * 2u * tp.k0 * n * (tp.in16 ? 2u : 4u));
         a.units = (uint32_t) (2u * k_r);
         int variant = 0, grid = 0;
-        launch_plan(b, a.units, glv::IN_S16_STEREO, a.ops, &variant, &grid);
+        launch_plan(b, a.units, glv::IN_S16_STEREO, a.ops, &variant, &grid, &a.plan);
         b->last_grid = grid; b->last_variant = variant;
         const hipError_t e = glv::launch_frame(b->log_nn, glv::IN_S16_STEREO, (int) b->p.log_mode, variant, cls, a, grid, st);
         if (e != hipSuccess) return fail(GLV_ERR_HIP, "kernel launch failed: %s", hipGetErrorString(e));
@@ -178,7 +178,7 @@
     const int hop_mode = tp.f32 ? glv::IN_F32_TRACK : glv::IN_S16_TRACK;
     const int mode = !tp.starts ? hop_mode : tp.f32 ? glv::IN_F32_TRACK_AT : glv::IN_S16_TRACK_AT;
     int variant = 0, grid = 0;
-    launch_plan(b, a.units, hop_mode, a.ops, &variant, &grid);
+    launch_plan(b, a.units, hop_mode, a.ops, &variant, &grid, &a.plan);
     b->last_grid = grid; b->last_variant = variant;
     const hipError_t e = glv::launch_frame(b->log_nn, mode, (int) b->p.log_mode, variant, cls, a, grid, st); ++b->last_launches;
     if (e != hipSuccess) return fail(GLV_ERR_HIP, "kernel launch failed: %s", hipGetErrorString(e));
diff --git a/glava_amd/csrc/glv_tune.hip b/glava_amd/csrc/glv_tune.hip
--- a/glava_amd/csrc/glv_tune.hip
+++ b/glava_amd/csrc/glv_tune.hip
@@ -57,7 +57,30 @@
 }
 }
 
+#if defined(GLV_WG_TIMELINE)
+static uint64_t* g_wg_timeline = nullptr;
+#endif
+
+static glv::RoundPlan g_round_plan = {};
+
 extern "C" {
+int glv_tune_set_rounds(unsigned frames, unsigned slots, unsigned cus, unsigned resident, int max_rounds, int rule) {
+    g_round_plan = glv::RoundPlan{};
+    if (rule < 0) return 0;
+    const glv::RoundPlan p = glv::plan_rounds(frames, slots, cus, resident, max_rounds, (glv::TaperRule) rule);
+    if (p.n <= 1) return 0;
+    g_round_plan = p;
+    return (int) glv::plan_workgroups(p);
+}
+int glv_tune_set_timeline(void* d_buf) {
+#if defined(GLV_WG_TIMELINE)
+    g_wg_timeline = static_cast<uint64_t*>(d_buf);
+    return 0;
+#else
+    (void) d_buf;
+    return -1;
+#endif
+}
 int glv_tune_count(void) { return (int) (sizeof(glv::kVariants) / sizeof(glv::kVariants[0])); }
 const char* glv_tune_describe(int i) { return glv::kVariants[i].desc; }
 int glv_tune_slots(int i) { return glv::kVariants[i].slots; }
@@ -123,6 +146,10 @@
     make_frame_weights(a.wts, a.F, true, 0);
     a.inv_n = 1.0f / (float) N; a.fft_scale = 10.2f; a.one_minus_cutoff = 1.0f - 0.3f;
     a.g = 4.2f * (1.0f / 86.1328125f); a.F_as_float = (float) a.F;
+    a.plan = g_round_plan;
+#if defined(GLV_WG_TIMELINE)
+    a.wg_timeline = g_wg_timeline;
+#endif
     hipStream_t st = (hipStream_t) stream;
     if (grid <= 0) {
         const unsigned slots = (unsigned) kVariants[i].slots;
diff --git a/glava_amd/csrc/glv_wisdom.cpp b/glava_amd/csrc/glv_wisdom.cpp
--- a/glava_amd/csrc/glv_wisdom.cpp
+++ b/glava_amd/csrc/glv_wisdom.cpp
@@ -76,20 +76,21 @@
     return k;
 }
 
-int default_grid(const glv_batch* b, uint32_t units, int variant) {
+bool size_tapers(int log_nn) { return log_nn == 11; }
+glv::RoundPlan default_plan(const glv_batch* b, uint32_t units, int variant, int* grid) {
     const glv::FrameGeometry g = glv::frame_geometry(b->log_nn, variant);
-    const uint32_t wgs = (units + g.rows_per_trip - 1) / g.rows_per_trip;
-    const uint32_t round = (uint32_t) b->num_cus * (uint32_t) g.resident;
-    if (wgs <= round) return (int) wgs;
-    uint32_t grid = wgs / 8u;
-    if (grid < round) grid = round;
-    if (grid > (uint32_t) g.rounds * round) grid = (uint32_t) g.rounds * round;
-    return (int) grid;
+    const uint32_t slots = (uint32_t) g.rows_per_trip / 2u;
+    const uint32_t cus = (uint32_t) (b->grid_cus > 0 ? b->grid_cus : b->num_cus);
+    glv::RoundPlan p = glv::plan_default((units + 1u) / 2u, slots, cus, (uint32_t) g.resident, g.rounds, size_tapers(b->log_nn) || b->grid_cus > 0);
+    *grid = (int) glv::plan_workgroups(p);
+    if (p.n <= 1) p = glv::RoundPlan{};
+    return p;
 }
 }
 namespace glvh __attribute__((visibility("hidden"))) {
-void launch_plan(glv_batch* b, uint32_t units, int in_mode, unsigned ops, int* variant, int* grid) {
+void launch_plan(glv_batch* b, uint32_t units, int in_mode, unsigned ops, int* variant, int* grid, glv::RoundPlan* rounds) {
     int v = 0, g = 0;
+    *rounds = glv::RoundPlan{};
     const uint32_t cls = wisdom_class(b, ops);
     if (b->variant_override < 0 || b->grid_override <= 0) {
         glv_batch::PlanCache& pc = b->plan_cache[in_mode][cls];
@@ -109,7 +110,7 @@
         const int rpt = glv::frame_geometry(b->log_nn, v).rows_per_trip;
         const uint32_t wgs_max = (units + rpt - 1) / rpt;
         if ((uint32_t) g > wgs_max) g = (int) wgs_max;
-    } else g = default_grid(b, units, v);
+    } else *rounds = default_plan(b, units, v, &g);
     *variant = v; *grid = g;
 }
 
```
